# iiscleap/ICL-speech-text-LLM

Measured on AMD Instinct MI355X. Metric: ICL utterances/sec (whole node), SALMONN+Llama2-7B 5-shot VOXCELEB, higher is better.
Workload: dtype bf16

## Files before the change

### icl-speech-text-llm_amd/csrc/attn.hip

```cpp
#include "common.h"
#include <type_traits>

#ifndef ICL_ATTN_V
#define ICL_ATTN_V 1
#endif

namespace {

struct AttnParams {
  const unsigned short* Q;
  const unsigned short* K;
  const unsigned short* V;
  unsigned short* O;
  const int* cu;
  const int* kv_lens;
  const float* rel_bias;
  const float* rel_gate;
  int64_t ldq, ldk, ldv, ldo;
  int64_t kv_seq_stride, kv_head_stride;
  int n_heads, rel_span, n_qblocks;
  float scale_log2e;
};

constexpr float NEG_BIG = -1.0e30f;

__device__ __forceinline__ float max32(const f32x16& a, const f32x16& b) {
  float m = __builtin_fmaxf(a[0], a[1]);
#pragma unroll
  for (int r = 2; r < 16; ++r) m = __builtin_fmaxf(m, a[r]);
#pragma unroll
  for (int r = 0; r < 16; ++r) m = __builtin_fmaxf(m, b[r]);
  return m;
}
constexpr float LOG2E = 1.4426950408889634f;
typedef float f32x2 __attribute__((ext_vector_type(2)));

__device__ __forceinline__ float max_xhalf(float v) {
  const unsigned u = __builtin_bit_cast(unsigned, v);
  const auto r = __builtin_amdgcn_permlane32_swap(u, u, false, false);
  const unsigned lo = r[0], hi = r[1];
  return __builtin_fmaxf(__builtin_bit_cast(float, lo), __builtin_bit_cast(float, hi));
}

template <int D, bool CAUSAL, bool BIAS>
__global__ __launch_bounds__(256, (D == 64 && BIAS) ? 3 : 2) void attn_fwd_kernel(AttnParams p) {
  constexpr int QB = 1;
  constexpr bool P2 = (D == 128);
  constexpr int BQ = 128 * QB;
  constexpr int ROWB = D * 2;
  constexpr int KS = D / 16;
  constexpr int DB = D / 32;
  constexpr int CPR = D / 8;
  constexpr int NCH = 64 * CPR / 256;
  constexpr int RPI = 64 / CPR;
  constexpr int BUF = 2 * 64 * ROWB;
  constexpr int NBUF = D == 64 ? 3 : 2;
  constexpr int AHEAD = NBUF - 1;
  __shared__ __attribute__((aligned(16))) char lds[NBUF * BUF];
  __shared__ float bias_win[BIAS ? 4 * QB * 128 : 1];

  const int tid = threadIdx.x, lane = tid & 63, wave = tid >> 6;
  const int ql = lane & 31, hh = lane >> 5;
  const int n_blocks = gridDim.x;
  const int xcd = blockIdx.x & 7, q8 = n_blocks >> 3, r8 = n_blocks & 7;
  const int item = (xcd < r8 ? xcd * (q8 + 1) : r8 * (q8 + 1) + (xcd - r8) * q8) + (blockIdx.x >> 3);
  const int qblk = (CAUSAL && (ICL_ATTN_V & 2)) ? p.n_qblocks - 1 - item % p.n_qblocks : item % p.n_qblocks;
  const int head = (item / p.n_qblocks) % p.n_heads, seq = item / (p.n_qblocks * p.n_heads);
  const int row0 = p.cu[seq];
  const int len = p.cu[seq + 1] - row0;
  const int qb = qblk * BQ;
  if (qb >= len) return;
  int kvlen = len;
  if (p.kv_lens) kvlen = min(max(p.kv_lens[seq], 1), len);
  const int kv_end = CAUSAL ? min(kvlen, qb + BQ) : kvlen;
  const int n_tiles = (kv_end + 63) >> 6;

  int qw[QB], qpos[QB];
  bf16x8 qf[QB][KS];
  float gate[QB];
  const float* bias_row = nullptr;
#pragma unroll
  for (int qi = 0; qi < QB; ++qi) {
    qw[qi] = qb + (wave * QB + qi) * 32;
    qpos[qi] = qw[qi] + ql;
    const int qrow = min(qpos[qi], len - 1);
    const unsigned short* qp = p.Q + (int64_t)(row0 + qrow) * p.ldq + head * D + hh * 8;
#pragma unroll
    for (int ks = 0; ks < KS; ++ks) qf[qi][ks] = *(const bf16x8*)(qp + ks * 16);
    gate[qi] = 0.f;
    if (BIAS) gate[qi] = p.rel_gate[(int64_t)(row0 + qrow) * p.n_heads + head] * LOG2E;
  }
  if (BIAS) bias_row = p.rel_bias + (int64_t)head * (2 * p.rel_span - 1) + (p.rel_span - 1);

  auto f_k = [](int row) { return D == 64 ? (row >> 1) & 7 : row & 15; };
  auto f_v = [](int row) { return D == 64 ? ((row >> 1) & 1) << 2 : (row & 3) << 2; };
  const int64_t kv_off = p.kv_seq_stride ? (int64_t)seq * p.kv_seq_stride + (int64_t)head * p.kv_head_stride : -1;
  const unsigned short* kbase = kv_off >= 0 ? p.K + kv_off : p.K + (int64_t)row0 * p.ldk + head * D;
  const unsigned short* vbase = kv_off >= 0 ? p.V + kv_off : p.V + (int64_t)row0 * p.ldv + head * D;
  const unsigned short* kptr[NCH];
  const unsigned short* vptr[NCH];
  int srow[NCH], kch[NCH], vch[NCH];
#pragma unroll
  for (int i = 0; i < NCH; ++i) {
    const int j = wave * NCH + i;
    srow[i] = RPI * j + lane / CPR;
    kch[i] = (lane % CPR) ^ f_k(srow[i]);
    vch[i] = (lane % CPR) ^ f_v(srow[i]);
    kptr[i] = kbase + (int64_t)srow[i] * p.ldk + kch[i] * 8;
    vptr[i] = vbase + (int64_t)srow[i] * p.ldv + vch[i] * 8;
  }
  const int64_t kstep = 64 * p.ldk, vstep = 64 * p.ldv;
  typedef const __attribute__((address_space(1))) void* gptr_t;
  typedef __attribute__((address_space(3))) void* lptr_t;
  auto stage_tile = [&](int t, int buf) {
    const int k0 = t * 64;
    char* k_w = lds + buf * BUF + wave * NCH * 1024;
    char* v_w = k_w + 64 * ROWB;
    if (k0 + 64 <= len) {
#pragma unroll
      for (int i = 0; i < NCH; ++i) {
        __builtin_amdgcn_global_load_lds((gptr_t)(kptr[i] + (int64_t)t * kstep), (lptr_t)(k_w + i * 1024), 16, 0, 0);
        __builtin_amdgcn_global_load_lds((gptr_t)(vptr[i] + (int64_t)t * vstep), (lptr_t)(v_w + i * 1024), 16, 0, 0);
      }
    } else {
#pragma unroll
      for (int i = 0; i < NCH; ++i) {
        const int64_t grow = min(k0 + srow[i], len - 1);
        __builtin_amdgcn_global_load_lds((gptr_t)(kbase + grow * p.ldk + kch[i] * 8), (lptr_t)(k_w + i * 1024), 16, 0, 0);
        __builtin_amdgcn_global_load_lds((gptr_t)(vbase + grow * p.ldv + vch[i] * 8), (lptr_t)(v_w + i * 1024), 16, 0, 0);
      }
    }
  };

  f32x16 o_acc[QB][DB];
  float m_run[QB], l_run[QB];
#pragma unroll
  for (int qi = 0; qi < QB; ++qi) {
    m_run[qi] = NEG_BIG;
    l_run[qi] = 0.f;
#pragma unroll
    for (int d = 0; d < DB; ++d)
#pragma unroll
      for (int r = 0; r < 16; ++r) o_acc[qi][d][r] = 0.f;
  }

  int k_off[KS];
#pragma unroll
  for (int ks = 0; ks < KS; ++ks) k_off[ks] = ql * ROWB + (((2 * ks + hh) ^ f_k(ql)) << 4);
  int tr_off[DB];
  {
    const int q = (lane & 15) >> 2;
    const int c2 = ((lane >> 4) & 1) * 2 + ((lane & 3) >> 1);
#pragma unroll
    for (int d = 0; d < DB; ++d)
      tr_off[d] = (4 * hh + q) * ROWB + (((4 * d + c2) ^ f_v(q)) << 4) + (lane & 1) * 8;
  }

  auto wait_oldest_tile = [&]() {
    if constexpr (AHEAD == 1) asm volatile("s_waitcnt vmcnt(0)" ::: "memory");
    else if constexpr (NCH == 2) asm volatile("s_waitcnt vmcnt(4)" ::: "memory");
    else asm volatile("s_waitcnt vmcnt(8)" ::: "memory");
  };
#pragma unroll
  for (int a = 0; a < AHEAD; ++a) stage_tile(min(a, n_tiles - 1), a);
  wait_oldest_tile();
  __syncthreads();
  int cur = 0;

  auto tile = [&](const int t, auto maymask_c, auto last_c) {
    constexpr bool MAYMASK = decltype(maymask_c)::value;
    constexpr bool LAST = decltype(last_c)::value;
    int nxt = cur + AHEAD;
    if (nxt >= NBUF) nxt -= NBUF;
    if constexpr (!LAST) stage_tile(min(t + AHEAD, n_tiles - 1), nxt);
    const int k0 = t * 64;
    const char* k_lds = lds + cur * BUF;
    const char* v_lds = k_lds + 64 * ROWB;
    bool active[QB];
    bool any_active = false;
#pragma unroll
    for (int qi = 0; qi < QB; ++qi) {
      active[qi] = !MAYMASK || !CAUSAL || (k0 <= qw[qi] + 31);
      any_active |= active[qi];
    }
    if (any_active) {
      f32x16 s_acc[QB][2];
#pragma unroll
      for (int qi = 0; qi < QB; ++qi)
#pragma unroll
        for (int kb = 0; kb < 2; ++kb)
#pragma unroll
          for (int r = 0; r < 16; ++r) s_acc[qi][kb][r] = 0.f;
      {
        constexpr int LA = QB == 2 ? 1 : 2;
        bf16x8 kf[LA + 1][2];
        auto read_k = [&](int ks, int slot) {
#pragma unroll
          for (int kb = 0; kb < 2; ++kb) {
            const unsigned a = (unsigned)(uintptr_t)(k_lds + kb * 32 * ROWB + k_off[ks]);
            asm volatile("ds_read_b128 %0, %1" : "=v"(kf[slot][kb]) : "v"(a));
          }
        };
#pragma unroll
        for (int i = 0; i < LA; ++i) read_k(i, i);
#pragma unroll
        for (int ks = 0; ks < KS; ++ks) {
          const int slot = ks % (LA + 1);
          if (ks + LA < KS) read_k(ks + LA, (ks + LA) % (LA + 1));
          const int newer = 2 * (KS - 1 - ks < LA ? KS - 1 - ks : LA);
          if (newer == 4) asm volatile("s_waitcnt lgkmcnt(4)" : "+v"(kf[slot][0]), "+v"(kf[slot][1]));
          else if (newer == 2) asm volatile("s_waitcnt lgkmcnt(2)" : "+v"(kf[slot][0]), "+v"(kf[slot][1]));
          else asm volatile("s_waitcnt lgkmcnt(0)" : "+v"(kf[slot][0]), "+v"(kf[slot][1]));
#pragma unroll
          for (int kb = 0; kb < 2; ++kb)
#pragma unroll
            for (int qi = 0; qi < QB; ++qi)
              if (active[qi])
                s_acc[qi][kb] = __builtin_amdgcn_mfma_f32_32x32x16_bf16(kf[slot][kb], qf[qi][ks], s_acc[qi][kb], 0, 0, 0);
        }
      }
      bf16x8 pf[QB][2][2];
      bf16x8 pl[P2 ? QB : 1][2][2];
#pragma unroll
      for (int qi = 0; qi < QB; ++qi) {
        if (!active[qi]) {
#pragma unroll
          for (int kb = 0; kb < 2; ++kb)
#pragma unroll
            for (int h2 = 0; h2 < 2; ++h2)
#pragma unroll
              for (int e = 0; e < 8; ++e) {
                pf[qi][kb][h2][e] = (__bf16)0.f;
                if (P2) pl[qi][kb][h2][e] = (__bf16)0.f;
              }
          continue;
        }
        const bool need_mask =
            MAYMASK && __builtin_amdgcn_readfirstlane((int)((k0 + 64 > kvlen) || (CAUSAL && (k0 + 63 > qw[qi]))));
        float psum = 0.f, alpha;
        if (!BIAS && !need_mask) {
          float tmax = max32(s_acc[qi][0], s_acc[qi][1]);
          tmax = max_xhalf(tmax) * p.scale_log2e;
          const float m_new = __builtin_fmaxf(m_run[qi], tmax);
          alpha = __builtin_amdgcn_exp2f(m_run[qi] - m_new);
          m_run[qi] = m_new;
          const f32x2 sc2 = {p.scale_log2e, p.scale_log2e}, nm2 = {-m_new, -m_new};
          f32x2 ps2 = {0.f, 0.f};
#pragma unroll
          for (int kb = 0; kb < 2; ++kb)
#pragma unroll
            for (int r = 0; r < 16; r += 2) {
              const f32x2 x = f32x2{s_acc[qi][kb][r], s_acc[qi][kb][r + 1]} * sc2 + nm2;
              const f32x2 e = {__builtin_amdgcn_exp2f(x[0]), __builtin_amdgcn_exp2f(x[1])};
              ps2 += e;
#pragma unroll
              for (int h = 0; h < 2; ++h) {
                pf[qi][kb][r >> 3][(r & 7) + h] = (__bf16)e[h];
                if (P2) pl[qi][kb][r >> 3][(r & 7) + h] = (__bf16)(e[h] - (float)pf[qi][kb][r >> 3][(r & 7) + h]);
              }
            }
          psum = ps2[0] + ps2[1];
        } else {
          float tmax;
          const float* win = nullptr;
          if (BIAS) {
            float* w = bias_win + (wave * QB + qi) * 128;
            const int base_rel = k0 - qw[qi] - 31;
#pragma unroll
            for (int i = 0; i < 2; ++i) {
              const int rel = max(-(p.rel_span - 1), min(p.rel_span - 1, base_rel + lane + 64 * i));
              w[lane + 64 * i] = bias_row[rel];
            }
            __builtin_amdgcn_wave_barrier();
            win = w + (4 * hh - ql + 31);
          }
#pragma unroll
          for (int kb = 0; kb < 2; ++kb) {
#pragma unroll
            for (int r = 0; r < 16; ++r) {
              const int key = k0 + kb * 32 + (r & 3) + 8 * (r >> 2) + 4 * hh;
              float v = s_acc[qi][kb][r] * p.scale_log2e;
              if (BIAS) v = fmaf(gate[qi], win[kb * 32 + (r & 3) + 8 * (r >> 2)], v);
              if (need_mask) {
                const bool ok = (key < kvlen) && (!CAUSAL || key <= qpos[qi]);
                v = ok ? v : NEG_BIG;
              }
              s_acc[qi][kb][r] = v;
            }
          }
          tmax = max_xhalf(max32(s_acc[qi][0], s_acc[qi][1]));
          const float m_new = __builtin_fmaxf(m_run[qi], tmax);
          alpha = __builtin_amdgcn_exp2f(m_run[qi] - m_new);
          m_run[qi] = m_new;
#pragma unroll
          for (int kb = 0; kb < 2; ++kb) {
#pragma unroll
            for (int r = 0; r < 16; ++r) {
              float e = __builtin_amdgcn_exp2f(s_acc[qi][kb][r] - m_new);
              if (need_mask) e = (s_acc[qi][kb][r] <= NEG_BIG * 0.5f) ? 0.f : e;
              psum += e;
              pf[qi][kb][r >> 3][r & 7] = (__bf16)e;
              if (P2) pl[qi][kb][r >> 3][r & 7] = (__bf16)(e - (float)pf[qi][kb][r >> 3][r & 7]);
            }
          }
        }
        l_run[qi] = l_run[qi] * alpha + psum;
        if (__builtin_amdgcn_ballot_w64(alpha != 1.0f) != 0) {
#pragma unroll
          for (int d = 0; d < DB; ++d)
#pragma unroll
            for (int r = 0; r < 16; ++r) o_acc[qi][d][r] *= alpha;
        }
      }
      {
        typedef __attribute__((ext_vector_type(8))) short s16x8;
        s16x4 vr[2][2][2];
        auto read_unit = [&](int u, int slot) {
          const int d = u >> 1, kb = u & 1;
#pragma unroll
          for (int s = 0; s < 2; ++s) {
            const unsigned a = (unsigned)(uintptr_t)(v_lds + (kb * 32 + 16 * s) * ROWB + tr_off[d]);
            asm volatile("ds_read_b64_tr_b16 %0, %1" : "=v"(vr[slot][s][0]) : "v"(a));
            asm volatile("ds_read_b64_tr_b16 %0, %1 offset:%2" : "=v"(vr[slot][s][1]) : "v"(a), "n"(8 * ROWB));
          }
        };
        read_unit(0, 0);
#pragma unroll
        for (int u = 0; u < 2 * DB; ++u) {
          const int slot = u & 1, d = u >> 1, kb = u & 1;
          if (u + 1 < 2 * DB) {
            read_unit(u + 1, slot ^ 1);
            asm volatile("s_waitcnt lgkmcnt(4)" : "+v"(vr[slot][0][0]), "+v"(vr[slot][0][1]), "+v"(vr[slot][1][0]), "+v"(vr[slot][1][1]));
          } else {
            asm volatile("s_waitcnt lgkmcnt(0)" : "+v"(vr[slot][0][0]), "+v"(vr[slot][0][1]), "+v"(vr[slot][1][0]), "+v"(vr[slot][1][1]));
          }
#pragma unroll
          for (int s = 0; s < 2; ++s) {
            const s16x8 both = __builtin_shufflevector(vr[slot][s][0], vr[slot][s][1], 0, 1, 2, 3, 4, 5, 6, 7);
            const bf16x8 vf = __builtin_bit_cast(bf16x8, both);
#pragma unroll
            for (int qi = 0; qi < QB; ++qi)
              if (active[qi]) {
                o_acc[qi][d] = __builtin_amdgcn_mfma_f32_32x32x16_bf16(vf, pf[qi][kb][s], o_acc[qi][d], 0, 0, 0);
                if (P2) o_acc[qi][d] = __builtin_amdgcn_mfma_f32_32x32x16_bf16(vf, pl[qi][kb][s], o_acc[qi][d], 0, 0, 0);
              }
          }
        }
      }
    }
    if constexpr (LAST) asm volatile("s_waitcnt vmcnt(0)" ::: "memory");
    else wait_oldest_tile();
    __builtin_amdgcn_s_barrier();
    cur = cur + 1 == NBUF ? 0 : cur + 1;
  };
  int t = 0;
  if constexpr (ICL_ATTN_V & 1) {
    const int n_staged = max(n_tiles - AHEAD, 0);
    const int n_plain = min(n_staged, CAUSAL ? min(kvlen, qw[0] + 1) >> 6 : kvlen >> 6);
    for (; t < n_plain; ++t) tile(t, std::false_type{}, std::false_type{});
    for (; t < n_staged; ++t) tile(t, std::true_type{}, std::false_type{});
    for (; t < n_tiles; ++t) tile(t, std::true_type{}, std::true_type{});
  } else {
    const int n_plain = min(n_tiles, CAUSAL ? min(kvlen, qw[0] + 1) >> 6 : kvlen >> 6);
    for (; t < n_plain; ++t) tile(t, std::false_type{}, std::false_type{});
    for (; t < n_tiles; ++t) tile(t, std::true_type{}, std::false_type{});
  }
  asm volatile("s_waitcnt vmcnt(0)" ::: "memory");
  __syncthreads();

  float inv[QB];
#pragma unroll
  for (int qi = 0; qi < QB; ++qi) {
    const float l_tot = l_run[qi] + __shfl_xor(l_run[qi], 32, 64);
    inv[qi] = l_tot > 0.f ? 1.f / l_tot : 0.f;
  }
  const bool rows16 = (((uintptr_t)p.O | (uintptr_t)(p.ldo * 2)) & 15) == 0;
  if (rows16) {
    constexpr int PITCH = D * 2 + 16;
    constexpr int LPR = D * 2 / 16, RPI = 64 / LPR;
    char* stg = lds + wave * (QB * 32 * PITCH);
#pragma unroll
    for (int qi = 0; qi < QB; ++qi)
#pragma unroll
      for (int d = 0; d < DB; ++d)
#pragma unroll
        for (int g = 0; g < 4; ++g) {
          const int d0 = d * 32 + 8 * g + 4 * hh;
          *(u32x2*)(stg + (qi * 32 + ql) * PITCH + d0 * 2) =
              u32x2{pack_bf16x2(o_acc[qi][d][4 * g] * inv[qi], o_acc[qi][d][4 * g + 1] * inv[qi]),
                    pack_bf16x2(o_acc[qi][d][4 * g + 2] * inv[qi], o_acc[qi][d][4 * g + 3] * inv[qi])};
        }
    __builtin_amdgcn_wave_barrier();
#pragma unroll
    for (int it = 0; it < QB * 32 / RPI; ++it) {
      const int row = it * RPI + lane / LPR, cc = lane % LPR;
      const int q = qw[row >> 5] + (row & 31);
      const u32x4 v = *(const u32x4*)(stg + row * PITCH + cc * 16);
      if (q < len) *(u32x4*)(p.O + (int64_t)(row0 + q) * p.ldo + head * D + cc * 8) = v;
    }
    return;
  }
#pragma unroll
  for (int qi = 0; qi < QB; ++qi) {
    if (qpos[qi] < len) {
      unsigned short* op = p.O + (int64_t)(row0 + qpos[qi]) * p.ldo + head * D;
#pragma unroll
      for (int d = 0; d < DB; ++d) {
#pragma unroll
        for (int g = 0; g < 4; ++g) {
          const int d0 = d * 32 + 8 * g + 4 * hh;
          u32x2 pk = {pack_bf16x2(o_acc[qi][d][4 * g] * inv[qi], o_acc[qi][d][4 * g + 1] * inv[qi]),
                      pack_bf16x2(o_acc[qi][d][4 * g + 2] * inv[qi], o_acc[qi][d][4 * g + 3] * inv[qi])};
          *(u32x2*)(op + d0) = pk;
        }
      }
    }
  }
}


constexpr int IL64_NW = 4;
template <bool CAUSAL, int NW>
__global__ __launch_bounds__(64 * NW, CAUSAL ? 1 : 2) void attn_fwd_il64_kernel(AttnParams p) {
  constexpr int D = 64, QB = 2, BQ = 32 * NW * QB, ROWB = D * 2, KS = D / 16, DB = D / 32, CPR = D / 8;
  constexpr int NCH = 64 * CPR / (64 * NW), RPI = 64 / CPR, BUF = 2 * 64 * ROWB, NBUF = 3;
  constexpr int EPI = NW * QB * 32 * (D * 2 + 16);
  static_assert(NW == 4 && NCH == 2, "the counted waits below (vmcnt(4) = one tile of 2 K + 2 V LDS-DMA per wave in flight) are for 4 waves");
  static_assert(EPI <= NBUF * BUF, "the epilogue staging must fit inside the K / V ring it reuses");
  __shared__ __attribute__((aligned(16))) char lds[NBUF * BUF];

  const int tid = threadIdx.x, lane = tid & 63, wave = tid >> 6;
  const int ql = lane & 31, hh = lane >> 5;
  const int n_blocks = gridDim.x;
  const int xcd = blockIdx.x & 7, q8 = n_blocks >> 3, r8 = n_blocks & 7;
  const int item = (xcd < r8 ? xcd * (q8 + 1) : r8 * (q8 + 1) + (xcd - r8) * q8) + (blockIdx.x >> 3);
  const int qblk = item % p.n_qblocks;
  const int head = (item / p.n_qblocks) % p.n_heads, seq = item / (p.n_qblocks * p.n_heads);
  const int row0 = p.cu[seq];
  const int len = p.cu[seq + 1] - row0;
  const int qb = qblk * BQ;
  if (qb >= len) return;
  int kvlen = len;
  if (p.kv_lens) kvlen = min(max(p.kv_lens[seq], 1), len);
  const int kv_end = CAUSAL ? min(kvlen, qb + BQ) : kvlen;
  const int n_tiles = (kv_end + 63) >> 6;

  int qw[QB], qpos[QB];
  bf16x8 qf[QB][KS];
#pragma unroll
  for (int qi = 0; qi < QB; ++qi) {
    qw[qi] = qb + (wave * QB + qi) * 32;
    qpos[qi] = qw[qi] + ql;
    const int qrow = min(qpos[qi], len - 1);
    const unsigned short* qp = p.Q + (int64_t)(row0 + qrow) * p.ldq + head * D + hh * 8;
#pragma unroll
    for (int ks = 0; ks < KS; ++ks) qf[qi][ks] = *(const bf16x8*)(qp + ks * 16);
  }

  auto f_k = [](int row) { return (row >> 1) & 7; };
  auto f_v = [](int row) { return ((row >> 1) & 1) << 2; };
  const int64_t kv_off = p.kv_seq_stride ? (int64_t)seq * p.kv_seq_stride + (int64_t)head * p.kv_head_stride : -1;
  const unsigned short* kbase = kv_off >= 0 ? p.K + kv_off : p.K + (int64_t)row0 * p.ldk + head * D;
  const unsigned short* vbase = kv_off >= 0 ? p.V + kv_off : p.V + (int64_t)row0 * p.ldv + head * D;
  const unsigned short* kptr[NCH];
  const unsigned short* vptr[NCH];
  int srow[NCH], kch[NCH], vch[NCH];
#pragma unroll
  for (int i = 0; i < NCH; ++i) {
    const int j = wave * NCH + i;
    srow[i] = RPI * j + lane / CPR;
    kch[i] = (lane % CPR) ^ f_k(srow[i]);
    vch[i] = (lane % CPR) ^ f_v(srow[i]);
    kptr[i] = kbase + (int64_t)srow[i] * p.ldk + kch[i] * 8;
    vptr[i] = vbase + (int64_t)srow[i] * p.ldv + vch[i] * 8;
  }
  const int64_t kstep = 64 * p.ldk, vstep = 64 * p.ldv;
  typedef const __attribute__((address_space(1))) void* gptr_t;
  typedef __attribute__((address_space(3))) void* lptr_t;
  auto stage_tile = [&](int t, int buf) {
    const int k0 = t * 64;
    char* k_w = lds + buf * BUF + wave * NCH * 1024;
    char* v_w = k_w + 64 * ROWB;
    if (k0 + 64 <= len) {
#pragma unroll
      for (int i = 0; i < NCH; ++i) {
        __builtin_amdgcn_global_load_lds((gptr_t)(kptr[i] + (int64_t)t * kstep), (lptr_t)(k_w + i * 1024), 16, 0, 0);
        __builtin_amdgcn_global_load_lds((gptr_t)(vptr[i] + (int64_t)t * vstep), (lptr_t)(v_w + i * 1024), 16, 0, 0);
      }
    } else {
#pragma unroll
      for (int i = 0; i < NCH; ++i) {
        const int64_t grow = min(k0 + srow[i], len - 1);
        __builtin_amdgcn_global_load_lds((gptr_t)(kbase + grow * p.ldk + kch[i] * 8), (lptr_t)(k_w + i * 1024), 16, 0, 0);
        __builtin_amdgcn_global_load_lds((gptr_t)(vbase + grow * p.ldv + vch[i] * 8), (lptr_t)(v_w + i * 1024), 16, 0, 0);
      }
    }
  };

  f32x16 o_acc[QB][DB];
  float m_run[QB], l_run[QB];
#pragma unroll
  for (int qi = 0; qi < QB; ++qi) {
    m_run[qi] = NEG_BIG;
    l_run[qi] = 0.f;
#pragma unroll
    for (int d = 0; d < DB; ++d)
#pragma unroll
      for (int r = 0; r < 16; ++r) o_acc[qi][d][r] = 0.f;
  }
  int k_off[KS];
#pragma unroll
  for (int ks = 0; ks < KS; ++ks) k_off[ks] = ql * ROWB + (((2 * ks + hh) ^ f_k(ql)) << 4);
  int tr_off[DB];
  {
    const int q = (lane & 15) >> 2;
    const int c2 = ((lane >> 4) & 1) * 2 + ((lane & 3) >> 1);
#pragma unroll
    for (int d = 0; d < DB; ++d) tr_off[d] = (4 * hh + q) * ROWB + (((4 * d + c2) ^ f_v(q)) << 4) + (lane & 1) * 8;
  }

  auto sm_head = [&](const int qi, f32x16 (&s)[2], const int k0, auto maymask_c) -> bool {
    constexpr bool MAYMASK = decltype(maymask_c)::value;
    const bool need_mask =
        MAYMASK && __builtin_amdgcn_readfirstlane((int)((k0 + 64 > kvlen) || (CAUSAL && (k0 + 63 > qw[qi]))));
    float tmax;
    if (!need_mask) {
      tmax = max_xhalf(max32(s[0], s[1])) * p.scale_log2e;
    } else {
#pragma unroll
      for (int kb = 0; kb < 2; ++kb)
#pragma unroll
        for (int r = 0; r < 16; ++r) {
          const int key = k0 + kb * 32 + (r & 3) + 8 * (r >> 2) + 4 * hh;
          const bool ok = (key < kvlen) && (!CAUSAL || key <= qpos[qi]);
          s[kb][r] = ok ? s[kb][r] * p.scale_log2e : NEG_BIG;
        }
      tmax = max_xhalf(max32(s[0], s[1]));
    }
    const float m_new = __builtin_fmaxf(m_run[qi], tmax);
    const float alpha = __builtin_amdgcn_exp2f(m_run[qi] - m_new);
    m_run[qi] = m_new;
    l_run[qi] *= alpha;
    if (__builtin_amdgcn_ballot_w64(alpha != 1.0f) != 0) {
#pragma unroll
      for (int d = 0; d < DB; ++d)
#pragma unroll
        for (int r = 0; r < 16; ++r) o_acc[qi][d][r] *= alpha;
    }
    return need_mask;
  };
  auto sm_tail = [&](const int qi, f32x16 (&s)[2], const bool need_mask, bf16x8 (&pf)[2][2]) {
    float psum = 0.f;
    const float m = m_run[qi];
    if (!need_mask) {
#pragma unroll
      for (int kb = 0; kb < 2; ++kb)
#pragma unroll
        for (int r = 0; r < 16; ++r) {
          const float e = __builtin_amdgcn_exp2f(fmaf(s[kb][r], p.scale_log2e, -m));
          psum += e;
          pf[kb][r >> 3][r & 7] = (__bf16)e;
        }
    } else {
#pragma unroll
      for (int kb = 0; kb < 2; ++kb)
#pragma unroll
        for (int r = 0; r < 16; ++r) {
          float e = __builtin_amdgcn_exp2f(s[kb][r] - m);
          e = (s[kb][r] <= NEG_BIG * 0.5f) ? 0.f : e;
          psum += e;
          pf[kb][r >> 3][r & 7] = (__bf16)e;
        }
    }
    l_run[qi] += psum;
  };

  stage_tile(0, 0);
  stage_tile(min(1, n_tiles - 1), 1);
  asm volatile("s_waitcnt vmcnt(4)" ::: "memory");
  __syncthreads();
  int cur = 0;

  auto tile = [&](const int t, auto maymask_c) {
    int nxt = cur + 2;
    if (nxt >= NBUF) nxt -= NBUF;
    stage_tile(min(t + 2, n_tiles - 1), nxt);
    const int k0 = t * 64;
    const char* k_lds = lds + cur * BUF;
    const char* v_lds = k_lds + 64 * ROWB;
    bf16x8 kf[KS][2];
#pragma unroll
    for (int ks = 0; ks < KS; ++ks)
#pragma unroll
      for (int kb = 0; kb < 2; ++kb) {
        const unsigned a = (unsigned)(uintptr_t)(k_lds + kb * 32 * ROWB + k_off[ks]);
        asm volatile("ds_read_b128 %0, %1" : "=v"(kf[ks][kb]) : "v"(a));
      }
    f32x16 s0[2], s1[2];
#pragma unroll
    for (int kb = 0; kb < 2; ++kb)
#pragma unroll
      for (int r = 0; r < 16; ++r) s0[kb][r] = s1[kb][r] = 0.f;
#pragma unroll
    for (int ks = 0; ks < KS; ++ks) {
      if (ks == 0) asm volatile("s_waitcnt lgkmcnt(6)" : "+v"(kf[0][0]), "+v"(kf[0][1]));
      if (ks == 1) asm volatile("s_waitcnt lgkmcnt(4)" : "+v"(kf[1][0]), "+v"(kf[1][1]));
      if (ks == 2) asm volatile("s_waitcnt lgkmcnt(2)" : "+v"(kf[2][0]), "+v"(kf[2][1]));
      if (ks == 3) asm volatile("s_waitcnt lgkmcnt(0)" : "+v"(kf[3][0]), "+v"(kf[3][1]));
#pragma unroll
      for (int kb = 0; kb < 2; ++kb) s0[kb] = __builtin_amdgcn_mfma_f32_32x32x16_bf16(kf[ks][kb], qf[0][ks], s0[kb], 0, 0, 0);
    }
    const bool nm0 = sm_head(0, s0, k0, maymask_c);
#pragma unroll
    for (int ks = 0; ks < KS; ++ks)
#pragma unroll
      for (int kb = 0; kb < 2; ++kb) s1[kb] = __builtin_amdgcn_mfma_f32_32x32x16_bf16(kf[ks][kb], qf[1][ks], s1[kb], 0, 0, 0);
    bf16x8 pf0[2][2], pf1[2][2];
    sm_tail(0, s0, nm0, pf0);
    asm volatile("" : "+v"(pf0[0][0]), "+v"(pf0[0][1]), "+v"(pf0[1][0]), "+v"(pf0[1][1]));
    typedef __attribute__((ext_vector_type(8))) short s16x8;
    s16x4 vr[2][2][DB][2];
#pragma unroll
    for (int kb = 0; kb < 2; ++kb)
#pragma unroll
      for (int s = 0; s < 2; ++s)
#pragma unroll
        for (int d = 0; d < DB; ++d) {
          const unsigned a = (unsigned)(uintptr_t)(v_lds + (kb * 32 + 16 * s) * ROWB + tr_off[d]);
          asm volatile("ds_read_b64_tr_b16 %0, %1" : "=v"(vr[kb][s][d][0]) : "v"(a));
          asm volatile("ds_read_b64_tr_b16 %0, %1 offset:%2" : "=v"(vr[kb][s][d][1]) : "v"(a), "n"(8 * ROWB));
        }
    const bool nm1 = sm_head(1, s1, k0, maymask_c);
    bf16x8 vf[2][2][DB];
#pragma unroll
    for (int kb = 0; kb < 2; ++kb)
#pragma unroll
      for (int s = 0; s < 2; ++s) {
        if (kb == 0 && s == 0) asm volatile("s_waitcnt lgkmcnt(12)" : "+v"(vr[0][0][0][0]), "+v"(vr[0][0][0][1]), "+v"(vr[0][0][1][0]), "+v"(vr[0][0][1][1]));
        if (kb == 0 && s == 1) asm volatile("s_waitcnt lgkmcnt(8)" : "+v"(vr[0][1][0][0]), "+v"(vr[0][1][0][1]), "+v"(vr[0][1][1][0]), "+v"(vr[0][1][1][1]));
        if (kb == 1 && s == 0) asm volatile("s_waitcnt lgkmcnt(4)" : "+v"(vr[1][0][0][0]), "+v"(vr[1][0][0][1]), "+v"(vr[1][0][1][0]), "+v"(vr[1][0][1][1]));
        if (kb == 1 && s == 1) asm volatile("s_waitcnt lgkmcnt(0)" : "+v"(vr[1][1][0][0]), "+v"(vr[1][1][0][1]), "+v"(vr[1][1][1][0]), "+v"(vr[1][1][1][1]));
#pragma unroll
        for (int d = 0; d < DB; ++d) {
          const s16x8 both = __builtin_shufflevector(vr[kb][s][d][0], vr[kb][s][d][1], 0, 1, 2, 3, 4, 5, 6, 7);
          vf[kb][s][d] = __builtin_bit_cast(bf16x8, both);
          o_acc[0][d] = __builtin_amdgcn_mfma_f32_32x32x16_bf16(vf[kb][s][d], pf0[kb][s], o_acc[0][d], 0, 0, 0);
        }
      }
    sm_tail(1, s1, nm1, pf1);
#pragma unroll
    for (int kb = 0; kb < 2; ++kb)
#pragma unroll
      for (int s = 0; s < 2; ++s)
#pragma unroll
        for (int d = 0; d < DB; ++d)
          o_acc[1][d] = __builtin_amdgcn_mfma_f32_32x32x16_bf16(vf[kb][s][d], pf1[kb][s], o_acc[1][d], 0, 0, 0);
    asm volatile("s_waitcnt vmcnt(4)" ::: "memory");
    __builtin_amdgcn_s_barrier();
    cur = cur + 1 == NBUF ? 0 : cur + 1;
  };
  int t = 0;
  {
    const int n_plain = min(n_tiles, CAUSAL ? min(kvlen, qw[0] + 1) >> 6 : kvlen >> 6);
    for (; t < n_plain; ++t) tile(t, std::false_type{});
  }
  for (; t < n_tiles; ++t) tile(t, std::true_type{});
  asm volatile("s_waitcnt vmcnt(0)" ::: "memory");
  __syncthreads();

  float inv[QB];
#pragma unroll
  for (int qi = 0; qi < QB; ++qi) {
    const float l_tot = l_run[qi] + __shfl_xor(l_run[qi], 32, 64);
    inv[qi] = l_tot > 0.f ? 1.f / l_tot : 0.f;
  }
  const bool rows16 = (((uintptr_t)p.O | (uintptr_t)(p.ldo * 2)) & 15) == 0;
  if (rows16) {
    constexpr int PITCH = D * 2 + 16;
    constexpr int LPR = D * 2 / 16, RPS = 64 / LPR;
    char* stg = lds + wave * (QB * 32 * PITCH);
#pragma unroll
    for (int qi = 0; qi < QB; ++qi)
#pragma unroll
      for (int d = 0; d < DB; ++d)
#pragma unroll
        for (int g = 0; g < 4; ++g) {
          const int d0 = d * 32 + 8 * g + 4 * hh;
          *(u32x2*)(stg + (qi * 32 + ql) * PITCH + d0 * 2) =
              u32x2{pack_bf16x2(o_acc[qi][d][4 * g] * inv[qi], o_acc[qi][d][4 * g + 1] * inv[qi]),
                    pack_bf16x2(o_acc[qi][d][4 * g + 2] * inv[qi], o_acc[qi][d][4 * g + 3] * inv[qi])};
        }
    __builtin_amdgcn_wave_barrier();
#pragma unroll
    for (int it = 0; it < QB * 32 / RPS; ++it) {
      const int row = it * RPS + lane / LPR, cc = lane % LPR;
      const int q = qw[row >> 5] + (row & 31);
      const u32x4 v = *(const u32x4*)(stg + row * PITCH + cc * 16);
      if (q < len) *(u32x4*)(p.O + (int64_t)(row0 + q) * p.ldo + head * D + cc * 8) = v;
    }
    return;
  }
#pragma unroll
  for (int qi = 0; qi < QB; ++qi) {
    if (qpos[qi] < len) {
      unsigned short* op = p.O + (int64_t)(row0 + qpos[qi]) * p.ldo + head * D;
#pragma unroll
      for (int d = 0; d < DB; ++d)
#pragma unroll
        for (int g = 0; g < 4; ++g) {
          const int d0 = d * 32 + 8 * g + 4 * hh;
          *(u32x2*)(op + d0) = u32x2{pack_bf16x2(o_acc[qi][d][4 * g] * inv[qi], o_acc[qi][d][4 * g + 1] * inv[qi]),
                                     pack_bf16x2(o_acc[qi][d][4 * g + 2] * inv[qi], o_acc[qi][d][4 * g + 3] * inv[qi])};
        }
    }
  }
}

template <int D>
int launch_attn(const AttnParams& p, const icl_attn_args* a, hipStream_t stream) {
  const int bq = (D == 64 && !a->rel_bias) ? IL64_NW * 64 : 128;
  dim3 grid(((a->max_seqlen + bq - 1) / bq) * a->n_heads * a->n_seqs, 1, 1);
  const bool bias = a->rel_bias != nullptr;
  if (D == 64 && !bias) {
    if (a->causal) hipLaunchKernelGGL((attn_fwd_il64_kernel<true, IL64_NW>), grid, dim3(64 * IL64_NW), 0, stream, p);
    else hipLaunchKernelGGL((attn_fwd_il64_kernel<false, IL64_NW>), grid, dim3(64 * IL64_NW), 0, stream, p);
    ICL_CHECK_LAUNCH("icl_attn_fwd_bf16");
    return ICL_OK;
  }
  if (a->causal) {
    if (bias)
      hipLaunchKernelGGL((attn_fwd_kernel<D, true, true>), grid, dim3(256), 0, stream, p);
    else
      hipLaunchKernelGGL((attn_fwd_kernel<D, true, false>), grid, dim3(256), 0, stream, p);
  } else {
    if (bias)
      hipLaunchKernelGGL((attn_fwd_kernel<D, false, true>), grid, dim3(256), 0, stream, p);
    else
      hipLaunchKernelGGL((attn_fwd_kernel<D, false, false>), grid, dim3(256), 0, stream, p);
  }
  ICL_CHECK_LAUNCH("icl_attn_fwd_bf16");
  return ICL_OK;
}

}

extern "C" int icl_attn_fwd_bf16(const icl_attn_args* a, void* stream) {
  ICL_CHECK_ARG(a != nullptr, "icl_attn_fwd_bf16: args is NULL");
  ICL_CHECK_ARG(a->Q && a->K && a->V && a->O && a->cu_seqlens, "icl_attn_fwd_bf16: NULL pointer");
  ICL_CHECK_ARG(a->head_dim == 64 || a->head_dim == 128, "icl_attn_fwd_bf16: head_dim=%d (only 64 and 128)", a->head_dim);
  ICL_CHECK_ARG(a->n_seqs > 0 && a->n_seqs <= 65535 && a->n_heads > 0 && a->n_heads <= 65535 && a->max_seqlen > 0,
                "icl_attn_fwd_bf16: bad n_seqs/n_heads/max_seqlen");
  ICL_CHECK_ARG(a->ldq % 8 == 0 && a->ldk % 8 == 0 && a->ldv % 8 == 0 && a->ldo % 4 == 0,
                "icl_attn_fwd_bf16: leading dimensions must be multiples of 8 (ldo: 4)");
  ICL_CHECK_ARG(((uintptr_t)a->Q & 15) == 0 && ((uintptr_t)a->K & 15) == 0 && ((uintptr_t)a->V & 15) == 0 &&
                    ((uintptr_t)a->O & 7) == 0,
                "icl_attn_fwd_bf16: Q/K/V must be 16-byte and O 8-byte aligned");
  ICL_CHECK_ARG((a->rel_bias == nullptr) == (a->rel_gate == nullptr), "icl_attn_fwd_bf16: rel_bias and rel_gate go together");
  if (a->rel_bias) ICL_CHECK_ARG(a->rel_span >= 1, "icl_attn_fwd_bf16: rel_span must be >= 1");
  AttnParams p;
  p.Q = (const unsigned short*)a->Q;
  p.K = (const unsigned short*)a->K;
  p.V = (const unsigned short*)a->V;
  p.O = (unsigned short*)a->O;
  p.cu = a->cu_seqlens;
  p.kv_lens = a->kv_lens;
  p.rel_bias = a->rel_bias;
  p.rel_gate = a->rel_gate;
  p.ldq = a->ldq; p.ldk = a->ldk; p.ldv = a->ldv; p.ldo = a->ldo;
  ICL_CHECK_ARG((a->kv_seq_stride == 0) == (a->kv_head_stride == 0) && a->kv_seq_stride >= 0 && a->kv_head_stride >= 0 &&
                    a->kv_seq_stride % 8 == 0 && a->kv_head_stride % 8 == 0,
                "icl_attn_fwd_bf16: kv_seq_stride / kv_head_stride must both be 0 or both positive multiples of 8");
  p.kv_seq_stride = a->kv_seq_stride; p.kv_head_stride = a->kv_head_stride;
  p.n_heads = a->n_heads;
  p.rel_span = a->rel_span;
  const int bq = (a->head_dim == 64 && !a->rel_bias) ? IL64_NW * 64 : 128;
  p.n_qblocks = (a->max_seqlen + bq - 1) / bq;
  p.scale_log2e = a->scale * LOG2E;
  return a->head_dim == 64 ? launch_attn<64>(p, a, (hipStream_t)stream) : launch_attn<128>(p, a, (hipStream_t)stream);
}
```

### icl-speech-text-llm_amd/csrc/beats.hip

```cpp
#include "common.h"

namespace {

__device__ __forceinline__ int audio_of(const int* cu, int n_audio, int row, int pad) {
  int lo = 0, hi = n_audio - 1;
  while (lo < hi) {
    const int mid = (lo + hi + 1) >> 1;
    if (cu[mid] + pad * mid <= row) lo = mid;
    else hi = mid - 1;
  }
  return lo;
}

__global__ __launch_bounds__(256) void beats_patchify_kernel(const float* fbank, int max_frames, const int* cu,
                                                              int n_audio, int total_rows, unsigned short* out) {
  const int row0 = blockIdx.x * 8;
  const int row = row0 + (threadIdx.x >> 5);
  if (row >= total_rows) return;
  int a = audio_of(cu, n_audio, row0, 0);
  while (a + 1 < n_audio && cu[a + 1] <= row) ++a;
  const int local = row - cu[a];
  const int tp = local >> 3, fp = local & 7;
  const int l = threadIdx.x & 31, i = l >> 1, j0 = (l & 1) * 8;
  const float* src = fbank + ((int64_t)a * max_frames + tp * 16 + i) * 128 + fp * 16 + j0;
  const f32x4 v0 = *(const f32x4*)src, v1 = *(const f32x4*)(src + 4);
  *(u32x4*)(out + (int64_t)row * 256 + l * 8) =
      u32x4{pack_bf16x2(v0[0], v0[1]), pack_bf16x2(v0[2], v0[3]), pack_bf16x2(v1[0], v1[1]), pack_bf16x2(v1[2], v1[3])};
}

__global__ __launch_bounds__(256) void beats_posconv_pack_kernel(float* x, const int* cu, const int* valid,
                                                                  int n_audio, int C, int G, unsigned short* xg) {
  const int lanes_per_row = C >> 3, rows_per_block = 256 / lanes_per_row;
  const int sub = threadIdx.x / lanes_per_row;
  if (sub >= rows_per_block) return;
  const int total = cu[n_audio] + 128 * n_audio;
  const int prow0 = blockIdx.x * rows_per_block, prow = prow0 + sub;
  if (prow >= total) return;
  int a = audio_of(cu, n_audio, prow0, 128);
  while (a + 1 < n_audio && cu[a + 1] + 128 * (a + 1) <= prow) ++a;
  const int r = prow - (cu[a] + 128 * a);
  const int T = cu[a + 1] - cu[a];
  const int t = r - 64;
  const bool in_range = (t >= 0) && (t < T);
  const bool live = in_range && (t < valid[a]);
  const int cpg = C / G;
  const int c = (threadIdx.x - sub * lanes_per_row) * 8;
  f32x4 v0 = {0.f, 0.f, 0.f, 0.f}, v1 = v0;
  if (in_range) {
    float* px = x + ((int64_t)cu[a] + t) * C + c;
    if (live) {
      v0 = *(const f32x4*)px;
      v1 = *(const f32x4*)(px + 4);
    } else {
      *(f32x4*)px = v0;
      *(f32x4*)(px + 4) = v0;
    }
  }
  const int g = c / cpg, ci = c - g * cpg;
  const int64_t base = ((int64_t)cu[a] + 128 * (int64_t)a) * C;
  *(u32x4*)(xg + base + ((int64_t)g * (T + 128) + r) * cpg + ci) =
      u32x4{pack_bf16x2(v0[0], v0[1]), pack_bf16x2(v0[2], v0[3]), pack_bf16x2(v1[0], v1[1]), pack_bf16x2(v1[2], v1[3])};
}

__global__ __launch_bounds__(256) void gather_rows_kernel(const float* src, int64_t lds_, const int* idx, float* out,
                                                           int64_t ldo, int N) {
  const int64_t r = blockIdx.x;
  const float* s = src + (int64_t)idx[r] * lds_;
  float* d = out + r * ldo;
  for (int c = threadIdx.x * 4; c < N; c += blockDim.x * 4) *(f32x4*)(d + c) = *(const f32x4*)(s + c);
}

}

extern "C" int icl_beats_patchify(const float* fbank, int32_t max_frames, const int32_t* cu_rows, int32_t n_audio,
                                  int32_t total_rows, void* out, void* stream) {
  ICL_CHECK_ARG(fbank && cu_rows && out && n_audio > 0 && total_rows > 0, "icl_beats_patchify: bad arguments");
  ICL_CHECK_ARG(((uintptr_t)fbank & 15) == 0 && ((uintptr_t)out & 15) == 0, "icl_beats_patchify: misaligned pointer");
  hipLaunchKernelGGL(beats_patchify_kernel, dim3((total_rows + 7) / 8), dim3(256), 0, (hipStream_t)stream, fbank, max_frames,
                     cu_rows, n_audio, total_rows, (unsigned short*)out);
  ICL_CHECK_LAUNCH("icl_beats_patchify");
  return ICL_OK;
}

extern "C" int icl_beats_posconv_pack(float* x, const int32_t* cu_rows, const int32_t* valid_rows, int32_t n_audio,
                                      int32_t total_rows, int32_t channels, int32_t groups, void* xg, void* stream) {
  ICL_CHECK_ARG(x && cu_rows && valid_rows && xg && n_audio > 0 && total_rows > 0, "icl_beats_posconv_pack: bad arguments");
  ICL_CHECK_ARG(groups > 0 && channels % groups == 0 && (channels / groups) % 8 == 0,
                "icl_beats_posconv_pack: channels/groups must be a multiple of 8 (got %d/%d)", channels, groups);
  ICL_CHECK_ARG(channels % 8 == 0 && channels <= 2048 && ((uintptr_t)x & 15) == 0 && ((uintptr_t)xg & 15) == 0,
                "icl_beats_posconv_pack: channels must be a multiple of 8 (<= 2048), pointers 16-byte aligned");
  const int rows_per_block = 256 / (channels / 8);
  hipLaunchKernelGGL(beats_posconv_pack_kernel, dim3((total_rows + 128 * n_audio + rows_per_block - 1) / rows_per_block), dim3(256),
                     0, (hipStream_t)stream, x, cu_rows, valid_rows, n_audio, channels, groups, (unsigned short*)xg);
  ICL_CHECK_LAUNCH("icl_beats_posconv_pack");
  return ICL_OK;
}

extern "C" int icl_gather_rows_f32(const float* src, int64_t ld_src, const int32_t* idx, float* out, int64_t ld_out,
                                   int32_t rows, int32_t N, void* stream) {
  ICL_CHECK_ARG(src && idx && out && rows > 0 && N > 0 && N % 4 == 0 && ld_src % 4 == 0 && ld_out % 4 == 0,
                "icl_gather_rows_f32: bad arguments");
  ICL_CHECK_ARG(((uintptr_t)src & 15) == 0 && ((uintptr_t)out & 15) == 0, "icl_gather_rows_f32: misaligned");
  hipLaunchKernelGGL(gather_rows_kernel, dim3(rows), dim3(256), 0, (hipStream_t)stream, src, ld_src, idx, out, ld_out, N);
  ICL_CHECK_LAUNCH("icl_gather_rows_f32");
  return ICL_OK;
}
```

### icl-speech-text-llm_amd/csrc/gemm.hip

```cpp
#include "gemm_common.h"
#include <vector>

using namespace iclg;

namespace {


#define TILE_STAGES_DEEP(BM_, BN_) (((BM_) + (BN_)) <= 128 ? 4 : 3)

template <int WAVES_M, int WAVES_N, int MI, int NI, int NST>
__global__ __launch_bounds__(256) void gemm_bf16_kernel(GemmParams p) {
  constexpr int BM = WAVES_M * MI * 16, BN = WAVES_N * NI * 16;
  constexpr int A_BYTES = BM * 128, W_BYTES = BN * 128, BUF = A_BYTES + W_BYTES;
  constexpr int A_INSTR = BM / 32, W_INSTR = BN / 32;
  constexpr int G_STAGE = A_INSTR + W_INSTR;
  static_assert(WAVES_M * WAVES_N == 4, "4 waves per block");
  extern __shared__ __attribute__((aligned(16))) char smem[];

  const int tid = threadIdx.x, lane = tid & 63;
  const int wave = __builtin_amdgcn_readfirstlane(tid >> 6);
  const int wm = wave / WAVES_N, wn = wave % WAVES_N;

  int tm, tn;
  block_to_tile(p, blockIdx.x, tm, tn);
// ... 664 lines not shown
    for (int u = 0; u < U; ++u) {
      if (j + u >= j1) break;
      const int s = 2 * (j + u);
#pragma unroll
      for (int h = 0; h < 2; ++h) {
        if (h == 0 ? s < s0 : s + 1 >= s1) continue;
#pragma unroll
        for (int t = 0; t < NT; ++t) {
          const bf16x8 wf = fp8x8_scaled_bf16(wq[u][t][2 * h], wq[u][t][2 * h + 1], sc[t]);
#pragma unroll
          for (int b = 0; b < MB; ++b) acc[t][b] = __builtin_amdgcn_mfma_f32_16x16x32_bf16(wf, af[u][h][b], acc[t][b], 0, 0, 0);
        }
      }
    }
  }
#pragma unroll
  for (int t = 0; t < NT; ++t)
#pragma unroll
    for (int b = 0; b < MB; ++b) *(f32x4*)&red[wave][t][b][lane * 4] = acc[t][b];
  __syncthreads();
  for (int f = wave; f < NT * MB; f += 8) {
    const int t = f / MB, b = f - t * MB;
    f32x4 v = *(const f32x4*)&red[0][t][b][lane * 4];
#pragma unroll
    for (int w = 1; w < 8; ++w) v = v + *(const f32x4*)&red[w][t][b][lane * 4];
    if (!(p.epi & ICL_EPI_SWIGLU)) epi_store4(p, 0, b * 16 + fr, n0 + t * 16 + fq * 4, v);
    else *(f32x4*)&red[0][t][b][lane * 4] = v;
  }
  if (p.epi & ICL_EPI_SWIGLU) {
    if constexpr (NT == 2) {
      __syncthreads();
      for (int b = wave; b < MB; b += 8) {
        const f32x4 g = *(const f32x4*)&red[0][0][b][lane * 4], u = *(const f32x4*)&red[0][1][b][lane * 4];
        epi_store_swiglu(p, 0, b * 16 + fr, n0, fq * 4, g, u);
      }
    }
  }
}

template <int MB, int NT, int U>
int launch_skinny_fp8w(GemmParams& p, const float* wscale, hipStream_t stream) {
  const int blocks = (p.N + 16 * NT - 1) / (16 * NT);
  hipLaunchKernelGGL((gemm_skinny_fp8w_kernel<MB, NT, U>), dim3(blocks), dim3(512), 0, stream, p, wscale);
  ICL_CHECK_LAUNCH("icl_gemm_fp8w");
  return ICL_OK;
}


template <int DEPTH, int MT>
int launch_m128(GemmParams& p, hipStream_t stream) {
  constexpr int BN = 128, SMEM = (DEPTH + 1) * MT * 16 * 128;
  auto kern = gemm_m128_kernel<DEPTH, MT>;
  static bool attr_set = false;
  if (!attr_set) {
    hipError_t e = hipFuncSetAttribute((const void*)kern, hipFuncAttributeMaxDynamicSharedMemorySize, SMEM);
    if (e != hipSuccess) {
      icl_set_error("icl_gemm_bf16: hipFuncSetAttribute(%d) failed: %s", SMEM, hipGetErrorString(e));
      return ICL_ELAUNCH;
    }
    attr_set = true;
  }
  hipLaunchKernelGGL(kern, dim3((p.N + BN - 1) / BN, 1, p.split_k), dim3(512), SMEM, stream, p);
  ICL_CHECK_LAUNCH("icl_gemm_bf16(m128)");
  return ICL_OK;
}

template <int WAVES_M, int WAVES_N, int MI, int NI, int NST>
int launch_tile_n(GemmParams& p, dim3 grid, hipStream_t stream) {
  constexpr int BM = WAVES_M * MI * 16, BN = WAVES_N * NI * 16;
  constexpr int SMEM = (BM + BN) * 128 * NST;
  auto kern = gemm_bf16_kernel<WAVES_M, WAVES_N, MI, NI, NST>;
  static bool attr_set = false;
  if (!attr_set) {
    hipError_t e = hipFuncSetAttribute((const void*)kern, hipFuncAttributeMaxDynamicSharedMemorySize, SMEM);
    if (e != hipSuccess) {
      icl_set_error("icl_gemm_bf16: hipFuncSetAttribute(%d) failed: %s", SMEM, hipGetErrorString(e));
      return ICL_ELAUNCH;
    }
    attr_set = true;
  }
  hipLaunchKernelGGL(kern, grid, dim3(256), SMEM, stream, p);
  ICL_CHECK_LAUNCH("icl_gemm_bf16");
  return ICL_OK;
}

template <int WAVES_M, int WAVES_N, int MI, int NI>
int launch_tile(GemmParams& p, int batch, hipStream_t stream) {
  constexpr int BM = WAVES_M * MI * 16, BN = WAVES_N * NI * 16;
  constexpr int DEEP = TILE_STAGES_DEEP(BM, BN);
  p.tiles_m = (p.M + BM - 1) / BM;
  p.tiles_n = (p.N + BN - 1) / BN;
  dim3 grid(p.tiles_m * p.tiles_n, 1, p.split_k > 1 ? p.split_k : batch);
  static int n_cu = 0;
  if (n_cu <= 0) {
    n_cu = icl_device_cu_count();
    if (n_cu <= 0) n_cu = 256;
  }
  const int64_t blocks = (int64_t)grid.x * grid.z;
  const int per_cu = (160 * 1024) / ((BM + BN) * 128 * DEEP);
  if (blocks <= (int64_t)n_cu * per_cu) return launch_tile_n<WAVES_M, WAVES_N, MI, NI, DEEP>(p, grid, stream);
  return launch_tile_n<WAVES_M, WAVES_N, MI, NI, 2>(p, grid, stream);
}

}


extern "C" int icl_gemm_select_tile(int32_t M, int32_t N, int32_t K, int32_t batch, int32_t split_k) {
  const int64_t t128 = (int64_t)((M + 127) / 128) * ((N + 127) / 128) * batch;
  if (split_k > 1 || M <= 64 || t128 < 256) return 2;
  if (N <= 64) return 2;
  if (N <= 128) return 1;
  static int ncu = 0;
  if (ncu <= 0) {
    ncu = icl_device_cu_count();
    if (ncu <= 0) ncu = 256;
  }
  const int64_t t256 = (int64_t)((M + 255) / 256) * ((N + 255) / 256) * batch;
  const int64_t rounds = (t256 + ncu - 1) / ncu;
  const double eff = (double)t256 / (double)(rounds * ncu);
  if (K >= 768 && eff >= 0.6) return 3;
  return 1;
}

struct NormFuse {
  const float* gamma;
  float eps;
  unsigned short* xn;
  int64_t ldx;
};

static int gemm_impl(const icl_gemm_args* a, void* stream_, const RopeFuse* rope, const NormFuse* norm = nullptr,
                     const float* wscale = nullptr) {
  hipStream_t stream = (hipStream_t)stream_;
  ICL_CHECK_ARG(a != nullptr, "icl_gemm_bf16: args is NULL");
  ICL_CHECK_ARG(a->A && a->W && a->C, "icl_gemm_bf16: A/W/C must be non-NULL");
  ICL_CHECK_ARG(a->M > 0 && a->N > 0 && a->K > 0, "icl_gemm_bf16: M,N,K must be > 0 (got %d,%d,%d)",
                a->M, a->N, a->K);
  ICL_CHECK_ARG(a->K % 64 == 0, "icl_gemm_bf16: K=%d must be a multiple of 64", a->K);
  ICL_CHECK_ARG(a->lda % 8 == 0 && a->ldw % 8 == 0,
                "icl_gemm_bf16: lda=%lld / ldw=%lld must be multiples of 8", (long long)a->lda,
                (long long)a->ldw);
  ICL_CHECK_ARG(((uintptr_t)a->A & 15) == 0 && ((uintptr_t)a->W & 15) == 0,
                "icl_gemm_bf16: A and W must be 16-byte aligned");
  ICL_CHECK_ARG(a->ldw >= a->K, "icl_gemm_bf16: ldw=%lld < K=%d", (long long)a->ldw, a->K);
  ICL_CHECK_ARG(a->batch >= 1 && a->batch <= 65535, "icl_gemm_bf16: batch=%d out of range", a->batch);
  ICL_CHECK_ARG(a->split_k >= 1 && a->split_k <= 64, "icl_gemm_bf16: split_k=%d out of range", a->split_k);
  ICL_CHECK_ARG(a->out_dtype == ICL_BF16 || a->out_dtype == ICL_F32, "icl_gemm_bf16: bad out_dtype %d",
                a->out_dtype);
  ICL_CHECK_ARG(a->res_dtype == ICL_BF16 || a->res_dtype == ICL_F32, "icl_gemm_bf16: bad res_dtype %d",
                a->res_dtype);
  ICL_CHECK_ARG((a->epilogue & ~15) == 0, "icl_gemm_bf16: unknown epilogue bits 0x%x", a->epilogue);
  const bool swiglu = a->epilogue & ICL_EPI_SWIGLU;
  if (swiglu) {
    ICL_CHECK_ARG(a->N % 32 == 0, "icl_gemm_bf16: SWIGLU needs N %% 32 == 0 (N=%d)", a->N);
    ICL_CHECK_ARG((a->epilogue & (ICL_EPI_GELU | ICL_EPI_RESIDUAL)) == 0,
                  "icl_gemm_bf16: SWIGLU cannot be combined with GELU/RESIDUAL");
    ICL_CHECK_ARG(a->ldc % 4 == 0, "icl_gemm_bf16: SWIGLU needs ldc %% 4 == 0");
  }
  if (a->epilogue & ICL_EPI_BIAS) ICL_CHECK_ARG(a->bias, "icl_gemm_bf16: EPI_BIAS without bias");
  if (a->epilogue & ICL_EPI_RESIDUAL) ICL_CHECK_ARG(a->R, "icl_gemm_bf16: EPI_RESIDUAL without R");
  const int nout = swiglu ? a->N / 2 : a->N;
  ICL_CHECK_ARG(a->ldc >= nout, "icl_gemm_bf16: ldc=%lld < %d output columns", (long long)a->ldc, nout);
  if (a->split_k > 1) {
    ICL_CHECK_ARG(a->batch == 1, "icl_gemm_bf16: split_k > 1 requires batch == 1");
    ICL_CHECK_ARG(a->workspace, "icl_gemm_bf16: split_k > 1 requires a workspace");
    ICL_CHECK_ARG(a->split_k <= a->K / 64, "icl_gemm_bf16: split_k=%d > K/64=%d", a->split_k, a->K / 64);
  }
  const int cal = a->out_dtype == ICL_BF16 ? 8 : 16;
  ICL_CHECK_ARG(((uintptr_t)a->C % cal) == 0, "icl_gemm_bf16: C must be %d-byte aligned", cal);
  if (a->R) {
    const int ral = a->res_dtype == ICL_BF16 ? 8 : 16;
    ICL_CHECK_ARG(((uintptr_t)a->R % ral) == 0, "icl_gemm_bf16: R must be %d-byte aligned", ral);
  }

  GemmParams p;
  p.A = (const __bf16*)a->A;
  p.W = (const __bf16*)a->W;
  p.C = a->C;
  p.bias = a->bias;
  p.R = a->R;
  p.ws = a->workspace;
  p.lda = a->lda; p.ldw = a->ldw; p.ldc = a->ldc; p.ldr = a->ldr;
  p.sA = a->strideA; p.sC = a->strideC; p.sR = a->strideR;
  p.M = a->M; p.N = a->N; p.K = a->K;
  p.epi = a->epilogue; p.out_dtype = a->out_dtype; p.res_dtype = a->res_dtype;
  p.split_k = a->split_k;
  p.tiles_m = p.tiles_n = 0;
  p.group_m = p.xcd_sync = 0;

  if (wscale) {
    ICL_CHECK_ARG(a->M <= 64 && a->batch == 1 && !rope, "icl_gemm_fp8w: needs M <= 64 and batch == 1 (M=%d batch=%d)", a->M, a->batch);
    p.split_k = 1;
    const bool sw = a->epilogue & ICL_EPI_SWIGLU;
    const int mb = (a->M + 15) / 16;
    if (sw) return mb <= 1 ? launch_skinny_fp8w<1, 2, 4>(p, wscale, stream) : mb == 2 ? launch_skinny_fp8w<2, 2, 2>(p, wscale, stream)
                           : launch_skinny_fp8w<4, 2, 1>(p, wscale, stream);
    return mb <= 1 ? launch_skinny_fp8w<1, 1, 8>(p, wscale, stream) : mb == 2 ? launch_skinny_fp8w<2, 1, 4>(p, wscale, stream)
                   : launch_skinny_fp8w<4, 1, 2>(p, wscale, stream);
  }
  int tile = a->tile;
  if (tile == 0) tile = icl_gemm_select_tile(a->M, a->N, a->K, a->batch, a->split_k);
  if (tile == 3 && a->K < 128) tile = 1;
  if (rope) {
    ICL_CHECK_ARG(tile == 3, "icl_gemm_rope_kv_bf16: only the 256x256 tile fuses RoPE (this problem resolves to tile %d; "
                             "use icl_gemm_bf16 + icl_rope_kv_bf16)", tile);
    ICL_CHECK_ARG(a->split_k == 1, "icl_gemm_rope_kv_bf16: split_k must be 1");
    return launch_tile256(p, 1, stream, rope);
  }
  int rc;
  if (tile == 1)
    rc = launch_tile<2, 2, 4, 4>(p, a->batch, stream);
  else if (tile == 2)
    rc = launch_tile<2, 2, 2, 2>(p, a->batch, stream);
  else if (tile == 3) {
    ICL_CHECK_ARG(a->split_k == 1 || (a->split_k <= a->K / 128 && a->N % 4 == 0),
                  "icl_gemm_bf16: split_k=%d on the 256x256 tile needs K / split_k >= 128 and N %% 4 == 0 (K=%d N=%d)", a->split_k, a->K, a->N);
    rc = launch_tile256(p, a->batch, stream);
  } else if (tile == 4 || tile == 6) {
    ICL_CHECK_ARG(a->M <= 64 && a->batch == 1, "icl_gemm_bf16: the skinny kernel needs M <= 64 and batch == 1");
    p.split_k = 1;
    const bool sw = a->epilogue & ICL_EPI_SWIGLU, pk = tile == 6;
    const int mb = (a->M + 15) / 16;
    if (sw) rc = mb <= 1 ? launch_skinny<1, 2, 4>(p, stream, pk) : mb == 2 ? launch_skinny<2, 2, 2>(p, stream, pk) : launch_skinny<4, 2, 2>(p, stream, pk);
    else    rc = mb <= 1 ? launch_skinny<1, 1, 8>(p, stream, pk) : mb == 2 ? launch_skinny<2, 1, 4>(p, stream, pk) : launch_skinny<4, 1, 2>(p, stream, pk);
    return rc;
  } else if (tile == 5) {
    ICL_CHECK_ARG(a->M <= 256 && a->batch == 1, "icl_gemm_bf16: the decode tile needs M <= 256 and batch == 1");
    rc = a->M <= 64 ? launch_m128<3, 4>(p, stream) : a->M <= 128 ? launch_m128<3, 8>(p, stream) : launch_m128<3, 16>(p, stream);
  } else {
    icl_set_error("icl_gemm_bf16: unsupported tile id %d", tile);
    return ICL_EINVAL;
  }
  if (rc != ICL_OK) return rc;
  if (a->split_k > 1 && norm) {
    if (a->N <= 4096) hipLaunchKernelGGL(splitk_reduce_rmsnorm_kernel<4>, dim3(a->M), dim3(256), 0, stream, p, norm->gamma, norm->eps, norm->xn, norm->ldx);
    else              hipLaunchKernelGGL(splitk_reduce_rmsnorm_kernel<8>, dim3(a->M), dim3(256), 0, stream, p, norm->gamma, norm->eps, norm->xn, norm->ldx);
    ICL_CHECK_LAUNCH("icl_gemm_rmsnorm_bf16(split-K reduce + RMSNorm)");
  } else if (a->split_k > 1) {
    const int64_t total = (int64_t)a->M * nout;
    int blocks = (int)((total + 255) / 256);
    if (blocks > 2048) blocks = 2048;
    hipLaunchKernelGGL(gemm_splitk_reduce_kernel, dim3(blocks), dim3(256), 0, stream, p);
    ICL_CHECK_LAUNCH("icl_gemm_bf16(split-K reduce)");
  }
  return ICL_OK;
}

extern "C" int icl_rmsnorm(const void* x, int64_t ldx, const float* gamma, void* y, int64_t ldy, int32_t M, int32_t N, float eps,
                           int32_t in_dtype, int32_t out_dtype, void* stream);

static int gemm_rmsnorm_impl(const icl_gemm_args* a, const float* wscale, const float* gamma, float eps, void* xn, int64_t ld_xn,
                             void* stream) {
  ICL_CHECK_ARG(a != nullptr && gamma && xn, "icl_gemm_rmsnorm_bf16: NULL pointer");
  ICL_CHECK_ARG(a->batch == 1 && a->out_dtype == ICL_F32 && (a->epilogue & ~ICL_EPI_RESIDUAL) == 0 &&
                    (!(a->epilogue & ICL_EPI_RESIDUAL) || a->res_dtype == ICL_F32),
                "icl_gemm_rmsnorm_bf16: batch 1, f32 output, residual-only epilogue with an f32 residual");
  ICL_CHECK_ARG(a->N % 4 == 0 && a->N <= 8192 && a->ldc % 4 == 0 && a->ldr % 4 == 0 && ld_xn % 4 == 0 && ld_xn >= a->N,
                "icl_gemm_rmsnorm_bf16: N=%d must be a multiple of 4 and <= 8192, leading dimensions multiples of 4", a->N);
  ICL_CHECK_ARG(((uintptr_t)gamma & 15) == 0 && ((uintptr_t)xn & 7) == 0 && ((uintptr_t)a->C & 15) == 0 &&
                    (!a->R || ((uintptr_t)a->R & 15) == 0), "icl_gemm_rmsnorm_bf16: misaligned pointer");
  if (a->split_k > 1 && a->tile != 4 && a->tile != 6 && !wscale) {
    const NormFuse nf{gamma, eps, (unsigned short*)xn, ld_xn};
    return gemm_impl(a, stream, nullptr, &nf);
  }
  const int rc = gemm_impl(a, stream, nullptr, nullptr, wscale);
  if (rc != ICL_OK) return rc;
#ifndef ICL_SMALL_M_BLOCKNORM
#define ICL_SMALL_M_BLOCKNORM 1
#endif
  if (ICL_SMALL_M_BLOCKNORM && a->M <= 64 && a->ldc == a->N) {
    GemmParams q{};
    q.ws = (float*)a->C; q.C = a->C; q.R = nullptr; q.ldc = a->ldc; q.ldr = 0; q.M = a->M; q.N = a->N; q.split_k = 1; q.epi = 0;
    if (a->N <= 4096) hipLaunchKernelGGL(splitk_reduce_rmsnorm_kernel<4>, dim3(a->M), dim3(256), 0, (hipStream_t)stream, q, gamma, eps, (unsigned short*)xn, ld_xn);
    else              hipLaunchKernelGGL(splitk_reduce_rmsnorm_kernel<8>, dim3(a->M), dim3(256), 0, (hipStream_t)stream, q, gamma, eps, (unsigned short*)xn, ld_xn);
    ICL_CHECK_LAUNCH("icl_gemm_rmsnorm_bf16(row-per-block RMSNorm)");
    return ICL_OK;
  }
  return icl_rmsnorm(a->C, a->ldc, gamma, xn, ld_xn, a->M, a->N, eps, ICL_F32, ICL_BF16, stream);
}

extern "C" int icl_gemm_rmsnorm_bf16(const icl_gemm_args* a, const float* gamma, float eps, void* xn, int64_t ld_xn, void* stream) {
  return gemm_rmsnorm_impl(a, nullptr, gamma, eps, xn, ld_xn, stream);
}

extern "C" int icl_gemm_bf16(const icl_gemm_args* a, void* stream) { return gemm_impl(a, stream, nullptr); }

extern "C" int icl_gemm_fp8w(const icl_gemm_args* a, const float* w_scale, void* stream) {
  ICL_CHECK_ARG(w_scale, "icl_gemm_fp8w: w_scale is NULL");
  return gemm_impl(a, stream, nullptr, nullptr, w_scale);
}

extern "C" int icl_gemm_rmsnorm_fp8w(const icl_gemm_args* a, const float* w_scale, const float* gamma, float eps, void* xn,
                                     int64_t ld_xn, void* stream) {
  ICL_CHECK_ARG(w_scale, "icl_gemm_rmsnorm_fp8w: w_scale is NULL");
  return gemm_rmsnorm_impl(a, w_scale, gamma, eps, xn, ld_xn, stream);
}

extern "C" int icl_gemm_rope_kv_bf16(const icl_gemm_args* a, int64_t k_off, int64_t v_off, const float* cosT,
                                     const float* sinT, const int32_t* pos, const int32_t* seq_ids, void* kcache,
                                     void* vcache, int32_t n_heads, int32_t head_dim, int32_t max_len, int32_t kv_rows_to_c,
                                     void* stream) {
  ICL_CHECK_ARG(a != nullptr && cosT && sinT && pos, "icl_gemm_rope_kv_bf16: NULL pointer");
  ICL_CHECK_ARG(head_dim == 128, "icl_gemm_rope_kv_bf16: head_dim=%d (the fused epilogue is built for 128)", head_dim);
  ICL_CHECK_ARG(n_heads > 0 && k_off == (int64_t)n_heads * 128 && v_off == 2 * k_off && a->N == 3 * k_off && k_off % 256 == 0,
                "icl_gemm_rope_kv_bf16: need q|k|v blocks of n_heads*128 columns each, a multiple of 256 (N=%d k_off=%lld v_off=%lld)",
                a->N, (long long)k_off, (long long)v_off);
  ICL_CHECK_ARG(a->batch == 1 && a->out_dtype == ICL_BF16 && (a->epilogue & ~ICL_EPI_BIAS) == 0,
                "icl_gemm_rope_kv_bf16: batch 1, bf16 output, bias-only epilogue");
  ICL_CHECK_ARG(a->C && ((uintptr_t)a->C & 15) == 0 && a->ldc % 8 == 0, "icl_gemm_rope_kv_bf16: C must be 16-byte aligned, ldc %% 8 == 0");
  ICL_CHECK_ARG(!a->bias || ((uintptr_t)a->bias & 15) == 0, "icl_gemm_rope_kv_bf16: bias must be 16-byte aligned");
  ICL_CHECK_ARG(((uintptr_t)cosT & 15) == 0 && ((uintptr_t)sinT & 15) == 0, "icl_gemm_rope_kv_bf16: cos/sin misaligned");
  ICL_CHECK_ARG((kcache == nullptr) == (vcache == nullptr), "icl_gemm_rope_kv_bf16: kcache and vcache must both be set or both NULL");
  if (kcache) {
    ICL_CHECK_ARG(seq_ids && max_len > 0, "icl_gemm_rope_kv_bf16: cache append needs seq_ids and max_len");
    ICL_CHECK_ARG(((uintptr_t)kcache & 15) == 0 && ((uintptr_t)vcache & 15) == 0, "icl_gemm_rope_kv_bf16: cache misaligned");
  }
  ICL_CHECK_ARG(kv_rows_to_c || kcache, "icl_gemm_rope_kv_bf16: kv_rows_to_c = 0 needs a cache to hold k / v");
  RopeFuse rf;
  rf.kv_rows_to_c = kv_rows_to_c;
  rf.cosT = cosT; rf.sinT = sinT; rf.pos = pos; rf.seq_ids = seq_ids;
  rf.kc = (unsigned short*)kcache; rf.vc = (unsigned short*)vcache;
  rf.k_off = (int)k_off; rf.v_off = (int)v_off; rf.H = n_heads; rf.max_len = max_len;
  return gemm_impl(a, stream, &rf);
}

extern "C" int icl_pack_decode_weights(const void* W, int64_t ldw, int32_t N, int32_t K, void* out, void* stream) {
  ICL_CHECK_ARG(W && out && N > 0 && K > 0, "icl_pack_decode_weights: bad arguments");
  ICL_CHECK_ARG(K % 64 == 0 && ldw % 8 == 0 && ldw >= K, "icl_pack_decode_weights: K=%d must be a multiple of 64, ldw=%lld a multiple of 8", K, (long long)ldw);
  ICL_CHECK_ARG(((uintptr_t)W & 15) == 0 && ((uintptr_t)out & 15) == 0, "icl_pack_decode_weights: misaligned pointer");
  const int64_t pieces = (int64_t)((N + 15) >> 4) * (K >> 5) * 64;
  const int blocks = (int)std::min<int64_t>((pieces + 255) / 256, 65535);
  hipLaunchKernelGGL(pack_decode_w_kernel, dim3(blocks), dim3(256), 0, (hipStream_t)stream, (const unsigned short*)W, ldw, N, K, (u32x4*)out);
  ICL_CHECK_LAUNCH("icl_pack_decode_weights");
  return ICL_OK;
}

extern "C" int icl_pack_fp8_weights(const void* W, int64_t ldw, int32_t N, int32_t K, void* q, float* scales, void* w_deq,
                                    int64_t ld_deq, void* stream) {
  ICL_CHECK_ARG(W && q && scales && w_deq && N > 0 && K > 0, "icl_pack_fp8_weights: bad arguments");
  ICL_CHECK_ARG(K % 64 == 0 && ldw % 8 == 0 && ldw >= K && ld_deq % 8 == 0 && ld_deq >= K,
                "icl_pack_fp8_weights: K=%d must be a multiple of 64, ldw=%lld / ld_deq=%lld multiples of 8 and >= K", K, (long long)ldw,
                (long long)ld_deq);
  ICL_CHECK_ARG((((uintptr_t)W | (uintptr_t)q | (uintptr_t)w_deq) & 15) == 0, "icl_pack_fp8_weights: misaligned pointer");
  ICL_CHECK_ARG(w_deq == W ? ld_deq == ldw : true, "icl_pack_fp8_weights: in place needs ld_deq == ldw");
  const int tiles = (N + 15) >> 4;
  hipStream_t s = (hipStream_t)stream;
  hipLaunchKernelGGL(pack_fp8_w_kernel, dim3(tiles), dim3(256), 0, s, (const unsigned short*)W, ldw, N, K, (u32x4*)q, scales,
                     (unsigned short*)w_deq, ld_deq);
  ICL_CHECK_LAUNCH("icl_pack_fp8_weights");
  std::vector<float> sc_host(N);
  hipError_t e = hipMemcpyAsync(sc_host.data(), scales, sizeof(float) * (size_t)N, hipMemcpyDeviceToHost, s);
  if (e == hipSuccess) e = hipStreamSynchronize(s);
  if (e != hipSuccess) {
    icl_set_error("icl_pack_fp8_weights: %s", hipGetErrorString(e));
    return ICL_ELAUNCH;
  }
  for (int n = 0; n < N; ++n)
    ICL_CHECK_ARG(sc_host[n] == sc_host[n], "icl_pack_fp8_weights: row %d holds a non-finite value", n);
  return ICL_OK;
}
```

### icl-speech-text-llm_amd/runtime/binding.py

```python
from __future__ import annotations

import ctypes
import os
from ctypes import POINTER, Structure, c_char_p, c_float, c_int, c_int32, c_int64, c_void_p

import torch

_HERE = os.path.dirname(os.path.abspath(__file__))
LIB_PATH = os.path.normpath(os.path.join(_HERE, "..", "lib", "libicl_hip.so"))

ICL_BF16, ICL_F32 = 0, 1
EPI_BIAS, EPI_GELU, EPI_RESIDUAL, EPI_SWIGLU = 1, 2, 4, 8
ABI_VERSION = 6
SAMPLE_TOP_K_MAX = 1024


GEMM_PROFILE = None


class IclError(RuntimeError):
    """Raised when a libicl_hip entry point returns a negative code."""


class GemmArgs(Structure):
    _fields_ = [
        ("A", c_void_p), ("W", c_void_p), ("C", c_void_p), ("bias", c_void_p), ("R", c_void_p),
        ("workspace", c_void_p),
        ("lda", c_int64), ("ldw", c_int64), ("ldc", c_int64), ("ldr", c_int64),
        ("strideA", c_int64), ("strideC", c_int64), ("strideR", c_int64),
        ("M", c_int32), ("N", c_int32), ("K", c_int32), ("batch", c_int32), ("epilogue", c_int32),
        ("out_dtype", c_int32), ("res_dtype", c_int32), ("split_k", c_int32), ("tile", c_int32),
    ]


class AttnArgs(Structure):
    _fields_ = [
        ("Q", c_void_p), ("K", c_void_p), ("V", c_void_p), ("O", c_void_p),
        ("cu_seqlens", c_void_p), ("kv_lens", c_void_p), ("rel_bias", c_void_p), ("rel_gate", c_void_p),
        ("ldq", c_int64), ("ldk", c_int64), ("ldv", c_int64), ("ldo", c_int64),
        ("n_seqs", c_int32), ("max_seqlen", c_int32), ("n_heads", c_int32), ("head_dim", c_int32),
        ("causal", c_int32), ("rel_span", c_int32), ("scale", c_float), ("reserved", c_int32),
        ("kv_seq_stride", c_int64), ("kv_head_stride", c_int64),
    ]


_SIGNATURES = {
    "icl_abi_version": (c_int, []),
    "icl_last_error": (c_char_p, []),
    "icl_device_cu_count": (c_int, []),
    "icl_gemm_bf16": (c_int, [POINTER(GemmArgs), c_void_p]),
    "icl_gemm_rmsnorm_bf16": (c_int, [POINTER(GemmArgs), c_void_p, c_float, c_void_p, c_int64, c_void_p]),
    "icl_gemm_select_tile": (c_int, [c_int32, c_int32, c_int32, c_int32, c_int32]),
    "icl_attn_fwd_bf16": (c_int, [POINTER(AttnArgs), c_void_p]),
    "icl_attn_decode_bf16": (c_int, [c_void_p, c_int64, c_void_p, c_void_p, c_void_p, c_int64, c_void_p,
                                     c_int32, c_int32, c_int32, c_int32, c_float, c_void_p]),
    "icl_attn_decode_rope_bf16": (c_int, [c_void_p, c_int64, c_int64, c_int64, c_void_p, c_void_p, c_void_p, c_void_p, c_void_p,
                                          c_void_p, c_void_p, c_int64, c_void_p, c_int32, c_int32, c_int32, c_int32, c_float,
                                          c_void_p]),
    "icl_layernorm": (c_int, [c_void_p, c_int64, c_void_p, c_float, c_void_p, c_void_p, c_void_p, c_int64,
                              c_void_p, c_int64, c_int32, c_int32, c_float, c_int32, c_int32, c_void_p]),
    "icl_rmsnorm": (c_int, [c_void_p, c_int64, c_void_p, c_void_p, c_int64, c_int32, c_int32, c_float,
                            c_int32, c_int32, c_void_p]),
    "icl_rope_kv_bf16": (c_int, [c_void_p, c_int64, c_int64, c_int64, c_void_p, c_void_p, c_void_p, c_void_p,
                                 c_void_p, c_void_p, c_int32, c_int32, c_int32, c_int32, c_void_p]),
    "icl_gemm_rope_kv_bf16": (c_int, [POINTER(GemmArgs), c_int64, c_int64, c_void_p, c_void_p, c_void_p, c_void_p,
                                      c_void_p, c_void_p, c_int32, c_int32, c_int32, c_int32, c_void_p]),
    "icl_pack_decode_weights": (c_int, [c_void_p, c_int64, c_int32, c_int32, c_void_p, c_void_p]),
    "icl_pack_fp8_weights": (c_int, [c_void_p, c_int64, c_int32, c_int32, c_void_p, c_void_p, c_void_p, c_int64, c_void_p]),
    "icl_gemm_fp8w": (c_int, [POINTER(GemmArgs), c_void_p, c_void_p]),
    "icl_gemm_rmsnorm_fp8w": (c_int, [POINTER(GemmArgs), c_void_p, c_void_p, c_float, c_void_p, c_int64, c_void_p]),
    "icl_embed_gather_interleave": (c_int, [c_void_p, c_void_p, c_void_p, c_void_p, c_int32, c_int32,
                                            c_int32, c_int32, c_void_p]),
    "icl_argmax_eos": (c_int, [c_void_p, c_int64, c_int32, c_int32, c_int32, c_int32, c_int32, c_void_p, c_void_p,
                               c_int32, c_int32, c_void_p, c_void_p]),
    "icl_argmax_fsm": (c_int, [c_void_p, c_int64, c_int32, c_int32, c_void_p, c_void_p, c_void_p, c_void_p, c_int32, c_int32,
                               c_void_p, c_int32, c_int32, c_int32, c_int32, c_void_p, c_void_p, c_int32, c_int32, c_void_p,
                               c_void_p, c_void_p]),
    "icl_sample_eos": (c_int, [c_void_p, c_int64, c_int32, c_int32, c_void_p, c_int64, c_void_p, c_int32, c_int32,
                               c_float, c_float, c_int32, c_float, c_void_p, c_int32, c_int32, c_int32, c_void_p, c_void_p,
                               c_int32, c_int32, c_void_p, c_void_p, c_void_p, c_void_p, c_int32, c_void_p]),
    "icl_beam_step": (c_int, [c_void_p, c_int64, c_int32, c_int32, c_int32, c_int32, c_int32, c_int32, c_int32, c_int32, c_float, c_float,
                              c_void_p, c_void_p, c_void_p, c_void_p, c_void_p, c_void_p, c_void_p, c_void_p, c_void_p, c_void_p]),
    "icl_kv_copy_spans_bf16": (c_int, [c_void_p, c_void_p, c_int64, c_int64, c_int64, c_int64, c_int64, c_int64, c_void_p,
                                       c_void_p, c_void_p, c_void_p, c_void_p, c_int32, c_int32, c_int32, c_int32, c_int32,
                                       c_int32, c_int32, c_int32, c_int32, c_void_p]),
    "icl_kv_copy_spans_fp8": (c_int, [c_void_p, c_void_p, c_void_p, c_void_p] + [c_int64] * 12 +
                              [c_void_p, c_void_p, c_void_p, c_void_p, c_void_p] + [c_int32] * 9 + [c_void_p]),
    "icl_kv_append_fp8": (c_int, [c_void_p, c_int64, c_int64, c_int64, c_void_p, c_void_p, c_void_p, c_void_p, c_void_p,
                                  c_void_p, c_int32, c_int32, c_int32, c_int32, c_void_p]),
    "icl_rope_kv_fp8": (c_int, [c_void_p, c_int64, c_int64, c_int64, c_void_p, c_void_p, c_void_p, c_void_p, c_void_p,
                                c_void_p, c_void_p, c_void_p, c_int32, c_int32, c_int32, c_int32, c_void_p]),
    "icl_attn_decode_bf16_epl16": (c_int, [c_void_p, c_int64, c_void_p, c_void_p, c_void_p, c_int64, c_void_p,
                                           c_int32, c_int32, c_int32, c_int32, c_float, c_void_p]),
    "icl_attn_decode_fp8": (c_int, [c_void_p, c_int64, c_void_p, c_void_p, c_void_p, c_void_p, c_void_p, c_int64, c_void_p,
                                    c_int32, c_int32, c_int32, c_int32, c_float, c_void_p]),
    "icl_attn_decode_rope_fp8": (c_int, [c_void_p, c_int64, c_int64, c_int64, c_void_p, c_void_p, c_void_p, c_void_p, c_void_p,
                                         c_void_p, c_void_p, c_void_p, c_void_p, c_int64, c_void_p, c_int32, c_int32, c_int32,
                                         c_int32, c_float, c_void_p]),
    "icl_logmel_whisper": (c_int, [c_void_p, c_int64, c_void_p, c_void_p, c_int32, c_int32, c_void_p,
                                   c_void_p, c_int64, c_void_p, c_void_p]),
    "icl_spec_to_xt": (c_int, [c_void_p, c_int32, c_int32, c_void_p, c_int64, c_void_p]),
    "icl_fbank_kaldi": (c_int, [c_void_p, c_int64, c_void_p, c_void_p, c_int32, c_int32, c_float, c_float,
                                c_void_p, c_void_p]),
    "icl_qformer_window_xattn": (c_int, [c_void_p, c_int64, c_void_p, c_int64, c_int64, c_void_p, c_int64,
                                         c_int32, c_int32, c_int32, c_int32, c_int32, c_float, c_void_p]),
    "icl_beats_gate": (c_int, [c_void_p, c_int64, c_void_p, c_void_p, c_void_p, c_void_p, c_int32, c_int32,
                               c_void_p]),
    "icl_axpby_cast": (c_int, [c_void_p, c_int64, c_int32, c_void_p, c_int64, c_int32, c_float, c_void_p,
                               c_int64, c_int32, c_int32, c_int32, c_void_p]),
    "icl_lora_down_bf16": (c_int, [c_void_p, c_int64, c_int32, c_void_p, c_int64, c_int32, c_float, c_int32,
                                   c_void_p]),
    "icl_beats_patchify": (c_int, [c_void_p, c_int32, c_void_p, c_int32, c_int32, c_void_p, c_void_p]),
    "icl_beats_posconv_pack": (c_int, [c_void_p, c_void_p, c_void_p, c_int32, c_int32, c_int32, c_int32, c_void_p,
                                       c_void_p]),
    "icl_gather_rows_f32": (c_int, [c_void_p, c_int64, c_void_p, c_void_p, c_int64, c_int32, c_int32, c_void_p]),
    "icl_cross_entropy": (c_int, [c_void_p, c_int64, c_void_p, c_int32, c_int32, c_void_p, c_void_p, c_void_p]),
}

EXPORTED_SYMBOLS = tuple(_SIGNATURES)

_lib = None


def load_library() -> ctypes.CDLL:
    global _lib
    if _lib is not None:
        return _lib
    path = os.environ.get("ICL_LIB_PATH") or LIB_PATH
    if not os.path.exists(path):
        raise ImportError(
            f"{path} not found: build it with `python -c 'import __graft_entry__ as g; g.build()'` "
            "(or `make -C icl-speech-text-llm_amd/csrc`). There is no CPU fallback for the HIP path.")
    lib = ctypes.CDLL(path)
    for name, (res, args) in _SIGNATURES.items():
        fn = getattr(lib, name)
        fn.restype = res
        fn.argtypes = args
    ver = lib.icl_abi_version()
    if ver != ABI_VERSION:
        raise ImportError(f"libicl_hip ABI version {ver} != binding version {ABI_VERSION}")
    _lib = lib
    return lib


def _check(rc: int, what: str) -> None:
    if rc != 0:
        msg = load_library().icl_last_error()
        raise IclError(f"{what} failed (code {rc}): {msg.decode() if msg else '?'}")


def _eos_pair(eos_id):
    if isinstance(eos_id, (tuple, list)):
        ids = [int(e) for e in eos_id]
        if not 1 <= len(ids) <= 2:
            raise ValueError(f"one or two EOS ids are supported, not {ids}")
        return ids[0], (ids[1] if len(ids) == 2 and ids[1] != ids[0] else -1)
    return int(eos_id), -1


def _stream() -> int:
    return torch.cuda.current_stream().cuda_stream


def _ptr(t):
    return 0 if t is None else t.data_ptr()


def _dt(t: torch.Tensor) -> int:
    if t.dtype == torch.bfloat16:
        return ICL_BF16
    if t.dtype == torch.float32:
        return ICL_F32
    raise TypeError(f"unsupported dtype {t.dtype}")


def _require_gpu(*tensors):
    for t in tensors:
        if t is not None and not t.is_cuda:
            raise IclError("libicl_hip operands must live on the GPU (no CPU fallback in the product path)")


def gemm(a: torch.Tensor, w: torch.Tensor, out: torch.Tensor, *, bias=None, residual=None, gelu=False,
         swiglu=False, split_k: int = 1, workspace=None, tile: int = 0, M=None, K=None, lda=None,
         batch: int = 1, stride_a: int = 0, stride_c: int = 0, stride_r: int = 0, rope=None, N=None, w_scale=None) -> torch.Tensor:
    _require_gpu(a, w, out, bias, residual, workspace)
    lib = load_library()
    g = GemmArgs()
    _require_gpu(w_scale)
    N = w.shape[0] if N is None else N
    g.A, g.W, g.C = a.data_ptr(), w.data_ptr(), out.data_ptr()
    g.bias, g.R, g.workspace = _ptr(bias), _ptr(residual), _ptr(workspace)
    g.lda = a.stride(-2) if lda is None else lda
    g.ldw = w.stride(0) if w_scale is None else w.shape[1]
    g.ldc = out.stride(-2)
    g.ldr = residual.stride(-2) if residual is not None else 0
    g.strideA, g.strideC, g.strideR = stride_a, stride_c, stride_r
    g.M = a.shape[-2] if M is None else M
    g.N = N
    g.K = w.shape[1] if K is None else K
    g.batch = batch
    epi = 0
    if bias is not None:
        assert bias.dtype == torch.float32
        epi |= EPI_BIAS
    if gelu:
        epi |= EPI_GELU
    if residual is not None:
        epi |= EPI_RESIDUAL
    if swiglu:
        epi |= EPI_SWIGLU
    g.epilogue = epi
    g.out_dtype = _dt(out)
    g.res_dtype = _dt(residual) if residual is not None else ICL_F32
    g.split_k = split_k
    if w_scale is not None:
        assert w.dtype == torch.uint8 and w_scale.dtype == torch.float32 and rope is None
        tile = "fp8w"
    elif tile == 0:
        tile = lib.icl_gemm_select_tile(g.M, N, g.K, batch, split_k)
    g.tile = tile if w_scale is None else 0
    if split_k > 1 and workspace is not None:
        assert workspace.dtype == torch.float32 and workspace.numel() >= split_k * g.M * N
    if rope is not None:
        k_off, v_off, cos, sin, pos, seq_ids, kcache, vcache, n_heads, head_dim, max_len = rope[:11]
        kv_rows_to_c = int(rope[11]) if len(rope) > 11 else 1
        _require_gpu(cos, sin, pos, seq_ids, kcache, vcache)

        def launch():
            _check(lib.icl_gemm_rope_kv_bf16(ctypes.byref(g), k_off, v_off, cos.data_ptr(), sin.data_ptr(), pos.data_ptr(),
                                             _ptr(seq_ids), _ptr(kcache), _ptr(vcache), n_heads, head_dim, max_len,
                                             kv_rows_to_c, _stream()), "icl_gemm_rope_kv_bf16")
    elif w_scale is not None:
        def launch():
            _check(lib.icl_gemm_fp8w(ctypes.byref(g), w_scale.data_ptr(), _stream()), "icl_gemm_fp8w")
    else:
        def launch():
            _check(lib.icl_gemm_bf16(ctypes.byref(g), _stream()), "icl_gemm_bf16")
    if GEMM_PROFILE is not None:
        e0, e1 = torch.cuda.Event(enable_timing=True), torch.cuda.Event(enable_timing=True)
        e0.record()
        launch()
        e1.record()
        GEMM_PROFILE.append((tile, split_k, 2.0 * g.M * N * g.K * batch, e0, e1, (g.M, N, g.K, batch)))
        return out
    launch()
    return out


def gemm_rmsnorm(a: torch.Tensor, w: torch.Tensor, out: torch.Tensor, gamma: torch.Tensor, eps: float, xn: torch.Tensor, *,
                 residual=None, split_k: int = 1, workspace=None, tile: int = 0, N=None, K=None, w_scale=None) -> torch.Tensor:
    _require_gpu(a, w, out, gamma, xn, residual, workspace, w_scale)
    lib = load_library()
    g = GemmArgs()
    N = w.shape[0] if N is None else N
    g.A, g.W, g.C = a.data_ptr(), w.data_ptr(), out.data_ptr()
    g.bias, g.R, g.workspace = 0, _ptr(residual), _ptr(workspace)
    g.lda, g.ldw, g.ldc = a.stride(-2), (w.stride(0) if w_scale is None else w.shape[1]), out.stride(-2)
    g.ldr = residual.stride(-2) if residual is not None else 0
    g.strideA = g.strideC = g.strideR = 0
    g.M, g.N, g.K, g.batch = a.shape[-2], N, (w.shape[1] if K is None else K), 1
    g.epilogue = EPI_RESIDUAL if residual is not None else 0
    g.out_dtype, g.res_dtype, g.split_k = _dt(out), ICL_F32, split_k
    assert out.dtype == torch.float32 and xn.dtype == torch.bfloat16 and gamma.dtype == torch.float32
    if w_scale is not None:
        assert w.dtype == torch.uint8 and w_scale.dtype == torch.float32
        g.tile = 0
        _check(lib.icl_gemm_rmsnorm_fp8w(ctypes.byref(g), w_scale.data_ptr(), gamma.data_ptr(), eps, xn.data_ptr(), xn.stride(0),
                                         _stream()), "icl_gemm_rmsnorm_fp8w")
        return out
    g.tile = tile if tile else lib.icl_gemm_select_tile(g.M, N, g.K, 1, split_k)
    if split_k > 1 and workspace is not None:
        assert workspace.dtype == torch.float32 and workspace.numel() >= split_k * g.M * N
    _check(lib.icl_gemm_rmsnorm_bf16(ctypes.byref(g), gamma.data_ptr(), eps, xn.data_ptr(), xn.stride(0), _stream()),
           "icl_gemm_rmsnorm_bf16")
    return out


def pack_decode_weights(w: torch.Tensor, K=None) -> torch.Tensor:
    _require_gpu(w)
    assert w.dtype == torch.bfloat16 and w.dim() == 2
    N, K = w.shape[0], (w.shape[1] if K is None else K)
    out = torch.empty((N + 15) // 16 * 16, K, dtype=torch.bfloat16, device=w.device)
    _check(load_library().icl_pack_decode_weights(w.data_ptr(), w.stride(0), N, K, out.data_ptr(), _stream()),
           "icl_pack_decode_weights")
    return out


def pack_fp8_weights(w: torch.Tensor, K=None, out=None):
    _require_gpu(w, out)
    assert w.dtype == torch.bfloat16 and w.dim() == 2
    N, K = w.shape[0], (w.shape[1] if K is None else K)
    q = torch.empty((N + 15) // 16 * 16, K, dtype=torch.uint8, device=w.device)
    scales = torch.empty(N, dtype=torch.float32, device=w.device)
    if out is None:
        out = torch.empty(N, K, dtype=torch.bfloat16, device=w.device)
    assert out.dtype == torch.bfloat16 and out.shape[0] == N and out.shape[1] >= K and out.stride(1) == 1
    _check(load_library().icl_pack_fp8_weights(w.data_ptr(), w.stride(0), N, K, q.data_ptr(), scales.data_ptr(), out.data_ptr(),
                                               out.stride(0), _stream()), "icl_pack_fp8_weights")
    return q, scales, out


def rope_fusable(M: int, n_heads: int, head_dim: int, K: int) -> bool:
    hd = n_heads * head_dim
    return (head_dim == 128 and hd % 256 == 0 and K >= 128 and
            load_library().icl_gemm_select_tile(M, 3 * hd, K, 1, 1) == 3)


def attn_fwd(q, k, v, out, cu_seqlens, max_seqlen: int, n_heads: int, head_dim: int, scale: float, *,
             causal=False, kv_lens=None, rel_bias=None, rel_gate=None, rel_span: int = 0, kv_cache_max_len: int = 0):
    _require_gpu(q, k, v, out, cu_seqlens, kv_lens, rel_bias, rel_gate)
    lib = load_library()
    a = AttnArgs()
    a.Q, a.K, a.V, a.O = q.data_ptr(), k.data_ptr(), v.data_ptr(), out.data_ptr()
    a.cu_seqlens, a.kv_lens = cu_seqlens.data_ptr(), _ptr(kv_lens)
    a.rel_bias, a.rel_gate = _ptr(rel_bias), _ptr(rel_gate)
    a.ldq, a.ldk, a.ldv, a.ldo = q.stride(0), k.stride(0), v.stride(0), out.stride(0)
    a.reserved = 0
    if kv_cache_max_len > 0:
        a.ldk = a.ldv = head_dim
        a.kv_seq_stride, a.kv_head_stride = n_heads * kv_cache_max_len * head_dim, kv_cache_max_len * head_dim
    else:
        a.kv_seq_stride = a.kv_head_stride = 0
    a.n_seqs = cu_seqlens.numel() - 1
    a.max_seqlen, a.n_heads, a.head_dim = max_seqlen, n_heads, head_dim
    a.causal, a.rel_span, a.scale = int(causal), rel_span, scale
    assert cu_seqlens.dtype == torch.int32
    _check(lib.icl_attn_fwd_bf16(ctypes.byref(a), _stream()), "icl_attn_fwd_bf16")
    return out


def attn_decode(q, kcache, vcache, out, lens, n_heads: int, head_dim: int, max_len: int, scale: float):
    _require_gpu(q, kcache, vcache, out, lens)
    assert lens.dtype == torch.int32
    _check(load_library().icl_attn_decode_bf16(q.data_ptr(), q.stride(0), kcache.data_ptr(), vcache.data_ptr(),
                                               out.data_ptr(), out.stride(0), lens.data_ptr(), q.shape[0],
                                               n_heads, head_dim, max_len, scale, _stream()),
           "icl_attn_decode_bf16")
    return out


def attn_decode_rope(qkv, k_off: int, v_off: int, cos, sin, pos, seq_ids, kcache, vcache, out, lens, n_heads: int,
                     head_dim: int, max_len: int, scale: float):
    _require_gpu(qkv, cos, sin, pos, seq_ids, kcache, vcache, out, lens)
    assert lens.dtype == torch.int32 and pos.dtype == torch.int32 and qkv.dtype == torch.bfloat16
    _check(load_library().icl_attn_decode_rope_bf16(qkv.data_ptr(), qkv.stride(0), k_off, v_off, cos.data_ptr(), sin.data_ptr(),
                                                    pos.data_ptr(), _ptr(seq_ids), kcache.data_ptr(), vcache.data_ptr(),
                                                    out.data_ptr(), out.stride(0), lens.data_ptr(), qkv.shape[0], n_heads,
                                                    head_dim, max_len, scale, _stream()), "icl_attn_decode_rope_bf16")
    return out


def _fp8_cache(kq, vq, ks, vs):
    assert kq.dtype == torch.uint8 and vq.dtype == torch.uint8 and ks.dtype == torch.float32 and vs.dtype == torch.float32


def attn_decode_bf16_epl16(q, kcache, vcache, out, lens, n_heads: int, head_dim: int, max_len: int, scale: float):
    _require_gpu(q, kcache, vcache, out, lens)
    assert lens.dtype == torch.int32
    _check(load_library().icl_attn_decode_bf16_epl16(q.data_ptr(), q.stride(0), kcache.data_ptr(), vcache.data_ptr(),
                                                     out.data_ptr(), out.stride(0), lens.data_ptr(), q.shape[0], n_heads, head_dim,
                                                     max_len, scale, _stream()), "icl_attn_decode_bf16_epl16")
    return out


def attn_decode_fp8(q, kq, vq, ks, vs, out, lens, n_heads: int, head_dim: int, max_len: int, scale: float):
    _require_gpu(q, kq, vq, ks, vs, out, lens)
    _fp8_cache(kq, vq, ks, vs)
    assert lens.dtype == torch.int32
    _check(load_library().icl_attn_decode_fp8(q.data_ptr(), q.stride(0), kq.data_ptr(), vq.data_ptr(), ks.data_ptr(), vs.data_ptr(),
                                              out.data_ptr(), out.stride(0), lens.data_ptr(), q.shape[0], n_heads, head_dim,
                                              max_len, scale, _stream()), "icl_attn_decode_fp8")
    return out


def attn_decode_rope_fp8(qkv, k_off: int, v_off: int, cos, sin, pos, seq_ids, kq, vq, ks, vs, out, lens, n_heads: int,
                         head_dim: int, max_len: int, scale: float):
    _require_gpu(qkv, cos, sin, pos, seq_ids, kq, vq, ks, vs, out, lens)
    _fp8_cache(kq, vq, ks, vs)
    assert lens.dtype == torch.int32 and pos.dtype == torch.int32 and qkv.dtype == torch.bfloat16
    _check(load_library().icl_attn_decode_rope_fp8(qkv.data_ptr(), qkv.stride(0), k_off, v_off, cos.data_ptr(), sin.data_ptr(),
                                                   pos.data_ptr(), _ptr(seq_ids), kq.data_ptr(), vq.data_ptr(), ks.data_ptr(),
                                                   vs.data_ptr(), out.data_ptr(), out.stride(0), lens.data_ptr(), qkv.shape[0],
                                                   n_heads, head_dim, max_len, scale, _stream()), "icl_attn_decode_rope_fp8")
    return out


def rope_kv_fp8(qkv, k_off: int, v_off: int, cos, sin, pos, seq_ids, kq, vq, ks, vs, n_heads: int, head_dim: int,
                max_len: int, M=None):
    _require_gpu(qkv, cos, sin, pos, seq_ids, kq, vq, ks, vs)
    _fp8_cache(kq, vq, ks, vs)
    M = qkv.shape[0] if M is None else M
    _check(load_library().icl_rope_kv_fp8(qkv.data_ptr(), qkv.stride(0), k_off, v_off, cos.data_ptr(), sin.data_ptr(),
                                          pos.data_ptr(), seq_ids.data_ptr(), kq.data_ptr(), vq.data_ptr(), ks.data_ptr(),
                                          vs.data_ptr(), M, n_heads, head_dim, max_len, _stream()), "icl_rope_kv_fp8")


def kv_append_fp8(qkv, k_off: int, v_off: int, pos, seq_ids, kq, vq, ks, vs, n_heads: int, head_dim: int, max_len: int, M=None):
    _require_gpu(qkv, pos, seq_ids, kq, vq, ks, vs)
    _fp8_cache(kq, vq, ks, vs)
    M = qkv.shape[0] if M is None else M
    _check(load_library().icl_kv_append_fp8(qkv.data_ptr(), qkv.stride(0), k_off, v_off, pos.data_ptr(), seq_ids.data_ptr(),
                                            kq.data_ptr(), vq.data_ptr(), ks.data_ptr(), vs.data_ptr(), M, n_heads, head_dim,
                                            max_len, _stream()), "icl_kv_append_fp8")


def layernorm(x, gamma, beta, out, eps: float, *, res=None, alpha: float = 1.0, out2=None, M=None, N=None):
    _require_gpu(x, gamma, beta, out, res, out2)
    M = x.shape[0] if M is None else M
    N = x.shape[1] if N is None else N
    if res is not None:
        assert res.dtype == x.dtype and res.stride(0) == x.stride(0)
    _check(load_library().icl_layernorm(x.data_ptr(), x.stride(0), _ptr(res), alpha, gamma.data_ptr(),
                                        beta.data_ptr(), out.data_ptr(), out.stride(0), _ptr(out2),
                                        out2.stride(0) if out2 is not None else 0, M, N, eps, _dt(x), _dt(out),
                                        _stream()), "icl_layernorm")
    return out


def rmsnorm(x, gamma, out, eps: float, *, M=None, N=None):
    _require_gpu(x, gamma, out)
    M = x.shape[0] if M is None else M
    N = x.shape[1] if N is None else N
    _check(load_library().icl_rmsnorm(x.data_ptr(), x.stride(0), gamma.data_ptr(), out.data_ptr(), out.stride(0),
                                      M, N, eps, _dt(x), _dt(out), _stream()), "icl_rmsnorm")
    return out


def rope_kv(qkv, k_off: int, v_off: int, cos, sin, pos, seq_ids, kcache, vcache, n_heads: int, head_dim: int,
            max_len: int, M=None):
    _require_gpu(qkv, cos, sin, pos, seq_ids, kcache, vcache)
    M = qkv.shape[0] if M is None else M
    _check(load_library().icl_rope_kv_bf16(qkv.data_ptr(), qkv.stride(0), k_off, v_off, cos.data_ptr(),
                                           sin.data_ptr(), pos.data_ptr(), _ptr(seq_ids), _ptr(kcache),
                                           _ptr(vcache), M, n_heads, head_dim, max_len, _stream()),
           "icl_rope_kv_bf16")


def embed_gather_interleave(src_idx, table, speech, out):
    _require_gpu(src_idx, table, speech, out)
    assert src_idx.dtype == torch.int32 and table.dtype == torch.bfloat16 and out.dtype == torch.float32
    _check(load_library().icl_embed_gather_interleave(src_idx.data_ptr(), table.data_ptr(), _ptr(speech),
                                                      out.data_ptr(), src_idx.numel(), table.shape[1],
                                                      table.shape[0], 0 if speech is None else speech.shape[0],
                                                      _stream()), "icl_embed_gather_interleave")
    return out


def argmax_eos(logits, eos_id, pad_id: int, finished, out_tokens, step: int, next_ids, V=None):
    _require_gpu(logits, finished, out_tokens, next_ids)
    e1, e2 = _eos_pair(eos_id)
    _check(load_library().icl_argmax_eos(logits.data_ptr(), logits.stride(0), logits.shape[0],
                                         logits.shape[1] if V is None else V, e1, e2, pad_id, finished.data_ptr(),
                                         out_tokens.data_ptr(), out_tokens.stride(0), step, next_ids.data_ptr(),
                                         _stream()), "icl_argmax_eos")


def argmax_fsm(logits, tables, state, steps_left: int, eos_id, pad_id: int, finished, out_tokens, step: int, next_ids,
               out_logprob=None, V=None):
    _require_gpu(logits, tables.state_off, tables.edge_tok, tables.edge_next, tables.state_dist, state, finished, out_tokens,
                 next_ids, out_logprob)
    V = logits.shape[1] if V is None else V
    if tables.vocab > V:
        raise ValueError(f"automaton built for a vocabulary of {tables.vocab} ids used on logits of {V}")
    assert logits.dtype == torch.float32 and state.dtype == torch.int32 and state.numel() == logits.shape[0]
    assert out_logprob is None or (out_logprob.dtype == torch.float32 and out_logprob.stride(0) == out_tokens.stride(0))
    e1, e2 = _eos_pair(eos_id)
    _check(load_library().icl_argmax_fsm(logits.data_ptr(), logits.stride(0), logits.shape[0], V, tables.state_off.data_ptr(),
                                         tables.edge_tok.data_ptr(), tables.edge_next.data_ptr(), tables.state_dist.data_ptr(),
                                         tables.n_states, tables.n_edges, state.data_ptr(), steps_left, e1, e2, pad_id,
                                         finished.data_ptr(), out_tokens.data_ptr(), out_tokens.stride(0), step,
                                         next_ids.data_ptr(), _ptr(out_logprob), _stream()), "icl_argmax_fsm")


def sample_eos(logits, work, uniforms, eos_id, pad_id: int, finished, out_tokens, step: int, next_ids, *,
               temperature: float = 1.0, top_k: int = 50, top_p: float = 1.0, repetition_penalty: float = 1.0, V=None,
               debug=None):
    _require_gpu(logits, work, uniforms, finished, out_tokens, next_ids)
    assert logits.dtype == torch.float32 and work.dtype == torch.float32 and uniforms.dtype == torch.float32
    V = logits.shape[1] if V is None else V
    e1, e2 = _eos_pair(eos_id)
    dbg = (None, None, None, 0)
    if debug is not None:
        _require_gpu(*debug)
        dbg = (debug[0].data_ptr(), debug[1].data_ptr(), debug[2].data_ptr(), debug[0].shape[1])
    _check(load_library().icl_sample_eos(logits.data_ptr(), logits.stride(0), logits.shape[0], V, work.data_ptr(),
                                         work.stride(0), out_tokens.data_ptr(), out_tokens.stride(0), step,
                                         repetition_penalty, temperature, top_k, top_p, uniforms.data_ptr(), e1, e2, pad_id,
                                         finished.data_ptr(), out_tokens.data_ptr(), out_tokens.stride(0), step,
                                         next_ids.data_ptr(), dbg[0], dbg[1], dbg[2], dbg[3], _stream()), "icl_sample_eos")


class BeamState:

    def __init__(self, get, B: int, K: int, T: int, pad_id: int):
        f32, i32 = torch.float32, torch.int32
        self.B, self.K, self.T = B, K, T
        self.run_score, self.fin_score = get("gen_beam_run_score", (B, K), f32), get("gen_beam_fin_score", (B, K), f32)
        self.run_seq, self.fin_seq = get("gen_beam_run_seq", (B, K, T), i32), get("gen_beam_fin_seq", (B, K, T), i32)
        self.fin_len, self.fin_flag = get("gen_beam_fin_len", (B, K), i32), get("gen_beam_fin_flag", (B, K), i32)
        self.unsat = get("gen_beam_unsat", (B,), i32)
        self.next_ids, self.parent = get("gen_beam_next", (B * K,), i32), get("gen_beam_parent", (B * K,), i32)
        self.run_score.fill_(-1.0e9)
        self.run_score[:, 0] = 0.0
        self.fin_score.fill_(-1.0e9)
        self.run_seq.fill_(pad_id)
        self.fin_seq.fill_(pad_id)
        self.fin_len.zero_()
        self.fin_flag.zero_()
        self.unsat.fill_(1)


def beam_step(logits, state: BeamState, step: int, eos_id, length_penalty: float, V=None, repetition_penalty: float = 1.0):
    _require_gpu(logits, state.run_score)
    assert logits.dtype == torch.float32 and logits.stride(1) == 1
    rows = logits.shape[0] // state.B
    assert rows * state.B == logits.shape[0] and rows in (1, state.K)
    e1, e2 = _eos_pair(eos_id)
    _check(load_library().icl_beam_step(logits.data_ptr(), logits.stride(0), rows, state.B,
                                        logits.shape[1] if V is None else V, state.K, state.T, step, e1, e2,
                                        float(length_penalty), float(repetition_penalty), state.run_score.data_ptr(),
                                        state.run_seq.data_ptr(),
                                        state.fin_score.data_ptr(), state.fin_seq.data_ptr(), state.fin_len.data_ptr(),
                                        state.fin_flag.data_ptr(), state.unsat.data_ptr(), state.next_ids.data_ptr(),
                                        state.parent.data_ptr(), _stream()), "icl_beam_step")


def kv_copy_spans(src, dst, n_rows: int, *, src_seq=None, src_t0=None, dst_seq=None, dst_t0=None, n_t=None, n_fixed: int = 0,
                  src_scale=None, dst_scale=None):
    _require_gpu(src, dst, src_seq, src_t0, dst_seq, dst_t0, n_t, src_scale, dst_scale)
    fp8 = src.dtype == torch.uint8
    assert src.dtype == dst.dtype and src.dtype in (torch.bfloat16, torch.uint8) and src.dim() == 5 and dst.dim() == 5
    assert src.stride(4) == 1 and dst.stride(4) == 1 and src.stride(3) == src.shape[4] and dst.stride(3) == dst.shape[4]
    assert src.shape[0] == dst.shape[0] and src.shape[2] == dst.shape[2] and src.shape[4] == dst.shape[4]
    for t in (src_seq, src_t0, dst_seq, dst_t0, n_t):
        assert t is None or (t.dtype == torch.int32 and t.numel() >= n_rows)
    ids = (_ptr(src_seq), _ptr(src_t0), _ptr(dst_seq), _ptr(dst_t0), _ptr(n_t), n_fixed, n_rows, src.shape[0], src.shape[2],
           src.shape[4], src.shape[1], dst.shape[1], src.shape[3], dst.shape[3], _stream())
    if fp8:
        assert src_scale is not None and dst_scale is not None and src_scale.dtype == torch.float32 and dst_scale.dtype == torch.float32
        assert tuple(src_scale.shape) == tuple(src.shape[:4]) and tuple(dst_scale.shape) == tuple(dst.shape[:4])
        assert src_scale.stride(3) == 1 and dst_scale.stride(3) == 1
        _check(load_library().icl_kv_copy_spans_fp8(src.data_ptr(), src_scale.data_ptr(), dst.data_ptr(), dst_scale.data_ptr(),
                                                    src.stride(0), src.stride(1), src.stride(2), dst.stride(0), dst.stride(1),
                                                    dst.stride(2), src_scale.stride(0), src_scale.stride(1), src_scale.stride(2),
                                                    dst_scale.stride(0), dst_scale.stride(1), dst_scale.stride(2), *ids),
               "icl_kv_copy_spans_fp8")
        return
    assert src_scale is None and dst_scale is None
    _check(load_library().icl_kv_copy_spans_bf16(src.data_ptr(), dst.data_ptr(), src.stride(0), src.stride(1), src.stride(2),
                                                 dst.stride(0), dst.stride(1), dst.stride(2), *ids), "icl_kv_copy_spans_bf16")


def logmel_whisper(wav, wav_lens, mel_filters, n_mel: int, spec, xt, workspace):
    _require_gpu(wav, wav_lens, mel_filters, spec, xt, workspace)
    assert wav.dtype == torch.float32 and mel_filters.dtype == torch.float64 and wav_lens.dtype == torch.int32
    _check(load_library().icl_logmel_whisper(wav.data_ptr(), wav.stride(0), wav_lens.data_ptr(),
                                             mel_filters.data_ptr(), n_mel, wav.shape[0], _ptr(spec), _ptr(xt),
                                             xt.stride(-2) if xt is not None else 0, workspace.data_ptr(),
                                             _stream()), "icl_logmel_whisper")


def spec_to_xt(spec, xt):
    _require_gpu(spec, xt)
    assert spec.dtype == torch.float32 and spec.is_contiguous()
    _check(load_library().icl_spec_to_xt(spec.data_ptr(), spec.shape[1], spec.shape[0], xt.data_ptr(),
                                         xt.stride(-2), _stream()), "icl_spec_to_xt")


def fbank_kaldi(wav, wav_lens, mel_banks, max_frames: int, mean: float, std: float, out):
    _require_gpu(wav, wav_lens, mel_banks, out)
    assert wav.dtype == torch.float32 and mel_banks.dtype == torch.float64 and wav_lens.dtype == torch.int32
    _check(load_library().icl_fbank_kaldi(wav.data_ptr(), wav.stride(0), wav_lens.data_ptr(), mel_banks.data_ptr(),
                                          wav.shape[0], max_frames, mean, std, out.data_ptr(), _stream()),
           "icl_fbank_kaldi")


def qformer_window_xattn(q, kv, v_off: int, out, n_audio: int, win_per_audio: int, win: int, rows_per_audio: int,
                         n_heads: int, scale: float):
    _require_gpu(q, kv, out)
    _check(load_library().icl_qformer_window_xattn(q.data_ptr(), q.stride(0), kv.data_ptr(), kv.stride(0), v_off,
                                                   out.data_ptr(), out.stride(0), n_audio, win_per_audio, win,
                                                   rows_per_audio, n_heads, scale, _stream()),
           "icl_qformer_window_xattn")


def beats_gate(qkv, grep_w, grep_b, grep_a, gate, n_heads: int, M=None):
    _require_gpu(qkv, grep_w, grep_b, grep_a, gate)
    M = qkv.shape[0] if M is None else M
    _check(load_library().icl_beats_gate(qkv.data_ptr(), qkv.stride(0), grep_w.data_ptr(), grep_b.data_ptr(),
                                         grep_a.data_ptr(), gate.data_ptr(), M, n_heads, _stream()),
           "icl_beats_gate")


def axpby_cast(x, out, alpha: float = 1.0, add=None):
    _require_gpu(x, out, add)
    M, N = x.shape
    _check(load_library().icl_axpby_cast(x.data_ptr(), x.stride(0), _dt(x), _ptr(add),
                                         add.stride(0) if add is not None else 0,
                                         _dt(add) if add is not None else ICL_F32, alpha, out.data_ptr(),
                                         out.stride(0), _dt(out), M, N, _stream()), "icl_axpby_cast")
    return out


def lora_down(x, K0: int, a, r_total: int, scale: float, M=None):
    _require_gpu(x, a)
    M = x.shape[0] if M is None else M
    _check(load_library().icl_lora_down_bf16(x.data_ptr(), x.stride(0), K0, a.data_ptr(), a.stride(0), r_total,
                                             scale, M, _stream()), "icl_lora_down_bf16")


def device_cu_count() -> int:
    return load_library().icl_device_cu_count()


def beats_patchify(fbank, cu_rows, total_rows: int, out):
    _require_gpu(fbank, cu_rows, out)
    _check(load_library().icl_beats_patchify(fbank.data_ptr(), fbank.shape[1], cu_rows.data_ptr(), fbank.shape[0],
                                             total_rows, out.data_ptr(), _stream()), "icl_beats_patchify")


def beats_posconv_pack(x, cu_rows, valid_rows, n_audio: int, total_rows: int, groups: int, xg):
    _require_gpu(x, cu_rows, valid_rows, xg)
    _check(load_library().icl_beats_posconv_pack(x.data_ptr(), cu_rows.data_ptr(), valid_rows.data_ptr(), n_audio,
                                                 total_rows, x.shape[1], groups, xg.data_ptr(), _stream()),
           "icl_beats_posconv_pack")


def gather_rows(src, idx, out, N=None):
    _require_gpu(src, idx, out)
    assert src.dtype == torch.float32 and out.dtype == torch.float32 and idx.dtype == torch.int32
    _check(load_library().icl_gather_rows_f32(src.data_ptr(), src.stride(0), idx.data_ptr(), out.data_ptr(),
                                              out.stride(0), idx.numel(), src.shape[1] if N is None else N,
                                              _stream()), "icl_gather_rows_f32")
    return out


def cross_entropy(logits, labels, row_loss, mean_loss, V=None):
    _require_gpu(logits, labels, row_loss, mean_loss)
    assert logits.dtype == torch.float32 and labels.dtype == torch.int32
    _check(load_library().icl_cross_entropy(logits.data_ptr(), logits.stride(0), labels.data_ptr(), labels.numel(),
                                            logits.shape[1] if V is None else V, row_loss.data_ptr(),
                                            mean_loss.data_ptr(), _stream()), "icl_cross_entropy")
    return mean_loss
```

### icl-speech-text-llm_amd/runtime/engines.py

```python
from __future__ import annotations

import os
from dataclasses import dataclass

from typing import Dict, List, Optional, Sequence, Tuple

import torch

from . import binding as B
from .packing import PackedBeats, PackedLlama, PackedQFormer, PackedWhisper

BF16, F32, I32 = torch.bfloat16, torch.float32, torch.int32


class Workspace:

    GRAPH_VISIBLE = ("dc_", "gen_", "kv_")

    def __init__(self, device):
        self.device = torch.device(device)
        self._bufs: Dict[tuple, list] = {}
        self.generation = 0

    def get(self, name: str, shape: Sequence[int], dtype, zero: bool = False) -> torch.Tensor:
# ... 65 lines not shown
        w, c = self.w, self.w.cfg
        n, d, T = xt.shape[0], c.d_model, c.n_ctx
        M = n * T
        x2 = ws.get("wh_x2", (n, 3002, d), BF16, zero=True)
        h = ws.get("wh_h", (M, d), F32)
        xn = ws.get("wh_xn", (M, d), BF16)
        qkv = ws.get("wh_qkv", (M, 3 * d), BF16)
        att = ws.get("wh_att", (M, d), BF16)
        ff = ws.get("wh_ff", (M, c.ffn), BF16)
        out = ws.get("wh_out", (M, d), F32)
        cu = ws.get("wh_cu", (n + 1,), I32)
        cu.copy_(torch.arange(0, M + 1, T, dtype=I32), non_blocking=True)
        B.gemm(xt, w.conv1_w, x2[:, 1:], bias=w.conv1_b, gelu=True, M=3000, K=384, lda=128, batch=n,
               stride_a=3002 * 128, stride_c=3002 * d)
        B.gemm(x2, w.conv2_w, h, bias=w.conv2_b, gelu=True, residual=w.pos, M=T, K=3 * d, lda=2 * d, batch=n,
               stride_a=3002 * d, stride_c=T * d, stride_r=0)
        D = d // c.n_heads
        for L in w.layers:
            B.layernorm(h, L.ln1_g, L.ln1_b, xn, 1e-5)
            B.gemm(xn, L.wqkv, qkv, bias=L.bqkv)
            B.attn_fwd(qkv[:, :d], qkv[:, d:2 * d], qkv[:, 2 * d:], att, cu, T, c.n_heads, D, D ** -0.5, kv_lens=kv_lens)
            B.gemm(att, L.wo, h, bias=L.bo, residual=h)
            B.layernorm(h, L.ln2_g, L.ln2_b, xn, 1e-5)
            B.gemm(xn, L.w1, ff, bias=L.b1, gelu=True)
            B.gemm(ff, L.w2, h, bias=L.b2, residual=h)
        if not final_ln:
            return h
        B.layernorm(h, w.lnf_g, w.lnf_b, out, 1e-5)
        return out


class QwenAudioTowerHIP:

    def __init__(self, enc: WhisperEncoderHIP, proj_w: torch.Tensor, proj_b: torch.Tensor, llm_hidden: int):
        self.enc, self.proj_w, self.proj_b, self.llm_hidden = enc, proj_w, proj_b, llm_hidden

    @staticmethod
    def output_lengths(mel_len: int):
        feat = (mel_len - 1) // 2 + 1
        return feat, (feat - 2) // 2 + 1

    def forward(self, ws: Workspace, xt: torch.Tensor, mel_lens: List[int]) -> Tuple[torch.Tensor, List[int]]:
        w, c = self.enc.w, self.enc.w.cfg
        n, d, T = xt.shape[0], c.d_model, c.n_ctx
        lens = [self.output_lengths(int(m)) for m in mel_lens]
        kv = _i32([max(1, f) for f, _ in lens], xt.device)
        h = self.enc.forward(ws, xt, kv_lens=kv, final_ln=False)
        P = n * (T // 2)
        pooled = ws.get("qa_pool", (P, d), F32)
        even, odd = h.view(P, 2 * d)[:, :d], h.view(P, 2 * d)[:, d:]
        B.axpby_cast(odd, pooled, alpha=0.5)
        B.axpby_cast(even, pooled, alpha=0.5, add=pooled)
        pb = ws.get("qa_pool_bf", (P, d), BF16)
        B.layernorm(pooled, w.lnf_g, w.lnf_b, pb, 1e-5)
        out = ws.get("qa_out", (P, self.llm_hidden), F32)
        B.gemm(pb, self.proj_w, out, bias=self.proj_b)
        return out, [o for _, o in lens]


class BeatsHIP:
    def __init__(self, w: PackedBeats, device):
        from .audio_tables import kaldi_mel_banks
        self.w = w
        self.banks = torch.from_numpy(kaldi_mel_banks()).to(device)

    @staticmethod
    def frames(n_samples: int) -> int:
        return 0 if n_samples < 400 else 1 + (n_samples - 400) // 160

    @classmethod
    def tokens(cls, n_samples: int) -> int:
        return (cls.frames(n_samples) // 16) * 8

    def forward(self, ws: Workspace, wav: torch.Tensor, padded_lens: List[int], valid_lens: List[int]):
        w, c = self.w, self.w.cfg
        dev = wav.device
        n, d = wav.shape[0], c.d_model
        nf = [self.frames(L) for L in padded_lens]
        T = [(f // 16) * 8 for f in nf]
        assert min(T) > 0, "audio shorter than one BEATs patch (16 frames)"
        assert max(T) <= w.rel_span or w.rel_span > c.max_distance, "audio longer than the packed relative-position span"
        cu_h = [0]
        for t in T:
            cu_h.append(cu_h[-1] + t)
        M = cu_h[-1]
        valid_T = []
        for a in range(n):
            vf = self._valid_units(valid_lens[a], padded_lens[a], nf[a])
            valid_T.append(max(1, self._valid_units(vf, nf[a], T[a])))
        max_frames = max(nf)
        fb = ws.get("be_fbank", (n, max_frames, 128), F32)
        B.fbank_kaldi(wav, _i32(padded_lens, dev), self.banks, max_frames, c.fbank_mean, c.fbank_std, fb)
        cu = _i32(cu_h, dev)
        valid = _i32(valid_T, dev)
        patches = ws.get("be_patches", (M, 256), BF16)
        B.beats_patchify(fb, cu, M, patches)
        e = ws.get("be_e", (M, c.embed), F32)
        eb = ws.get("be_eb", (M, c.embed), BF16)
        B.gemm(patches, w.patch_w, e)
        B.layernorm(e, w.ln0_g, w.ln0_b, eb, 1e-5)
        x = ws.get("be_x", (M, d), F32)
        B.gemm(eb, w.proj_w, x, bias=w.proj_b)
        G, cpg = c.conv_groups, d // c.conv_groups
        xg = ws.get("be_xg", ((M + 128 * n) * d,), BF16)
        B.beats_posconv_pack(x, cu, valid, n, M, G, xg)
        y = ws.get("be_y", (M, d), F32)
        uniform = all(t == T[0] for t in T)
        for g in range(G):
            wg, bg = w.posconv_w[g], w.posconv_b[g * cpg:(g + 1) * cpg]
            if uniform:
                a_view = xg[g * (T[0] + 128) * cpg:]
                B.gemm(a_view, wg, y[:, g * cpg:], bias=bg, gelu=True, residual=x[:, g * cpg:], M=T[0], K=128 * cpg,
                       lda=cpg, batch=n, stride_a=(T[0] + 128) * d, stride_c=T[0] * d, stride_r=T[0] * d)
            else:
                for a in range(n):
                    base = (cu_h[a] + 128 * a) * d + g * (T[a] + 128) * cpg
                    B.gemm(xg[base:], wg, y[cu_h[a]:cu_h[a + 1], g * cpg:], bias=bg, gelu=True,
                           residual=x[cu_h[a]:cu_h[a + 1], g * cpg:], M=T[a], K=128 * cpg, lda=cpg)
        xb = ws.get("be_xb", (M, d), BF16)
        B.layernorm(y, w.enc_ln_g, w.enc_ln_b, x, 1e-5, out2=xb)
        qkv = ws.get("be_qkv", (M, 3 * d), BF16)
        att = ws.get("be_att", (M, d), BF16)
        o = ws.get("be_o", (M, d), F32)
        ff = ws.get("be_ff", (M, c.ffn), BF16)
        gate = ws.get("be_gate", (M, c.n_heads), F32)
        alpha = c.deep_norm_alpha
        for L in w.layers:
            B.gemm(xb, L.wqkv, qkv, bias=L.bqkv)
            B.beats_gate(qkv, L.extra["grep_w"], L.extra["grep_b"], L.extra["grep_a"], gate, c.n_heads)
            B.attn_fwd(qkv[:, :d], qkv[:, d:2 * d], qkv[:, 2 * d:], att, cu, max(T), c.n_heads, 64, 0.125,
                       kv_lens=valid, rel_bias=w.rel_table, rel_gate=gate, rel_span=w.rel_span)
            B.gemm(att, L.wo, o, bias=L.bo)
            B.layernorm(o, L.ln1_g, L.ln1_b, x, 1e-5, res=x, alpha=alpha, out2=xb)
            B.gemm(xb, L.w1, ff, bias=L.b1, gelu=True)
            B.gemm(ff, L.w2, o, bias=L.b2)
            B.layernorm(o, L.ln2_g, L.ln2_b, x, 1e-5, res=x, alpha=alpha, out2=xb)
        return x, cu_h, T

    @staticmethod
    def _valid_units(valid_in: int, total_in: int, n_units: int) -> int:
        if n_units == 0:
            return 0
        per = total_in // n_units
        if per == 0:
            return n_units
        return min(n_units, -(-valid_in // per)) if valid_in > 0 else 0


class SpeechQFormerHIP:
    def __init__(self, w: PackedQFormer, whisper_d: int, beats_d: int, llm_hidden: int):
        self.w, self.whisper_d, self.beats_d, self.llm_hidden = w, whisper_d, beats_d, llm_hidden
        c = w.cfg
        self.win = round(1500 * c.second_per_window / 30.0)
        self.stride = round(1500 * c.second_stride / 30.0)
        assert self.win == self.stride, "HIP path implements non-overlapping windows (kernel == stride, SURVEY.md A8)"

    def n_windows(self, T: int = 1500) -> int:
        return (T - self.win) // self.stride + 1

    def forward(self, ws: Workspace, speech: torch.Tensor, n: int, audio: Optional[torch.Tensor] = None,
                audio_cu: Optional[List[int]] = None) -> torch.Tensor:
        T0 = 1500
        frames = [T0] * n if audio is None else [max(T0, audio_cu[a + 1] - audio_cu[a]) for a in range(n)]
        self.last_windows = [self.n_windows(f) for f in frames]
        if all(f == T0 for f in frames):
            return self._run(ws, speech, n, audio, audio_cu, T0)
        Wmax = max(self.last_windows)
        full = ws.get("qf_out_ragged", (n, Wmax, self.llm_hidden), F32)
        full.zero_()
        a0 = 0
        while a0 < n:
            a1 = a0 + 1
            while a1 < n and frames[a1] == frames[a0]:
                a1 += 1
            cu = [x - audio_cu[a0] for x in audio_cu[a0:a1 + 1]]
            out = self._run(ws, speech[a0 * T0:a1 * T0], a1 - a0, audio[audio_cu[a0]:audio_cu[a1]], cu, frames[a0])
            nw = self.n_windows(frames[a0])
            full[a0:a1, :nw].copy_(out.view(a1 - a0, nw, self.llm_hidden))
            a0 = a1
        return full.view(n * Wmax, self.llm_hidden)

    def _run(self, ws: Workspace, speech: torch.Tensor, n: int, audio: Optional[torch.Tensor], audio_cu: Optional[List[int]],
             T: int) -> torch.Tensor:
        w, c = self.w, self.w.cfg
        dw, db, hq = self.whisper_d, self.beats_d, c.hidden
        C = dw + (db if audio is not None else 0)
        assert C == c.enc_width, f"Q-Former encoder width {c.enc_width} != {C}"
        cat = ws.get("qf_cat", (n * T, C), BF16)
        if T == 1500:
            B.layernorm(speech, w.ln_speech_g, w.ln_speech_b, cat, 1e-5, N=dw)
        else:
            cat.zero_()
            for a in range(n):
                B.layernorm(speech[a * 1500:(a + 1) * 1500], w.ln_speech_g, w.ln_speech_b, cat[a * T:a * T + 1500], 1e-5, N=dw)
        if audio is not None:
            if T == 1500:
                cat[:, dw:].zero_()
            for a in range(n):
                ta = audio_cu[a + 1] - audio_cu[a]
                assert ta <= T
                B.layernorm(audio[audio_cu[a]:audio_cu[a] + ta], w.ln_audio_g, w.ln_audio_b,
                            cat[a * T:a * T + ta, dw:], 1e-5, N=db)
        nw = self.n_windows(T)
        W = n * nw
        h = ws.get("qf_h", (W, hq), F32)
        hb = ws.get("qf_hb", (W, hq), BF16)
        t32 = ws.get("qf_t32", (W, hq), F32)
        tb = ws.get("qf_tb", (W, hq), BF16)
        q = ws.get("qf_q", (W, hq), BF16)
        kv = ws.get("qf_kv", (n * T, 2 * hq), BF16)
        ff = ws.get("qf_ff", (W, c.ffn), BF16)
        q0 = ws.get("qf_q0", (1, hq), F32)
        B.layernorm(w.query, w.emb_ln_g, w.emb_ln_b, q0, c.ln_eps)
        B.axpby_cast(q0.expand(W, hq), h)
        B.axpby_cast(q0.expand(W, hq), hb)
        for L in w.layers:
            B.gemm(hb, L.sa_wv, tb, bias=L.sa_bv)
            B.gemm(tb, L.sa_wo, t32, bias=L.sa_bo, residual=h)
            B.layernorm(t32, L.sa_ln_g, L.sa_ln_b, h, c.ln_eps, out2=hb)
            B.gemm(hb, L.ca_wq, q, bias=L.ca_bq)
            B.gemm(cat, L.ca_wkv, kv, bias=L.ca_bkv)
            B.qformer_window_xattn(q, kv, hq, tb, n, nw, self.win, T, c.n_heads, 0.125)
            B.gemm(tb, L.ca_wo, t32, bias=L.ca_bo, residual=h)
            B.layernorm(t32, L.ca_ln_g, L.ca_ln_b, h, c.ln_eps, out2=hb)
            B.gemm(hb, L.w1, ff, bias=L.b1, gelu=True)
            B.gemm(ff, L.w2, t32, bias=L.b2, residual=h)
            B.layernorm(t32, L.ff_ln_g, L.ff_ln_b, h, c.ln_eps, out2=hb)
        out = ws.get("qf_out", (W, self.llm_hidden), F32)
        B.gemm(hb, w.proj_w, out, bias=w.proj_b)
        return out


DECODE_SITES = ("qkv", "o", "gu", "down")


@dataclass(frozen=True)
class GemmLaunch:
    tile: object
    split_k: int
    weight: str
    N: int
    K: int
    fused_norm: bool = False


@dataclass(frozen=True)
class DecodePlan:
    Bn: int
    sites: Dict[str, GemmLaunch]
    workspace: int


def lm_head_tile(R: int) -> int:
    return 4 if R <= 8 else 0


def t256_split(N: int, K: int, n_cu: int) -> int:
    tiles = (N + 255) // 256
    split = min(K // 512, int(0.8 * n_cu) // tiles)
    return split if split >= 2 and tiles * split >= 0.45 * n_cu else 0


def decode_plan(Bn: int, cfg, k_aug: int, n_cu: int, weight_dtype: str = "bf16", decode_packed: bool = True,
                decode_t256: Sequence[str] = DECODE_SITES, fuse_norms: bool = True) -> DecodePlan:
    hd, I = cfg.hidden, cfg.ffn
    shapes = dict(qkv=(3 * hd, k_aug), o=(hd, hd), gu=(2 * I, hd), down=(hd, I))

    def sk(N, K):
        tiles = ((N + 63) // 64) * ((Bn + 63) // 64)
        s = max(1, min(K // 512, (2 * n_cu + tiles - 1) // tiles))
        return min(s, 16)

    def sk5(N, K):
        return max(1, min(n_cu // ((N + 127) // 128), K // 512))
    plan = {}
    for name, (N, K) in shapes.items():
        if Bn <= 8 and weight_dtype == "fp8":
            tile, split, weight = "fp8w", 1, "fp8"
        elif Bn <= 256 and decode_packed:
            if Bn <= 8:
                tile, split, weight = 6, 1, "packed"
            else:
                tile, split, weight = 5, sk5(N, K), "packed"
                s256 = t256_split(N, K, n_cu) if Bn > 128 and name in decode_t256 else 0
                if s256:
                    tile, split, weight = 3, s256, "row"
        elif Bn <= 8:
            tile, split, weight = 4, 1, "row"
        else:
            tile, split, weight = 2, sk(N, K), "row"
        plan[name] = GemmLaunch(tile, split, weight, N, K, fused_norm=fuse_norms and name in ("o", "down"))
    plan["lm_head"] = GemmLaunch(lm_head_tile(Bn), 1, "row", cfg.vocab, hd)
    nsplit = max(p.split_k for p in plan.values())
    return DecodePlan(Bn, plan, nsplit * Bn * max(3 * hd, 2 * I) if nsplit > 1 else 0)


class LlamaHIP:
    decode_packed_weights = True
    fuse_decode_norms = True
    fuse_decode_rope = os.environ.get("ICL_FUSE_DECODE_ROPE", "1") != "0"

    decode_t256 = tuple(x for x in os.environ.get("ICL_DECODE_T256", "qkv,o,gu,down").split(",") if x)

    def _t256_split(self, N: int, K: int) -> int:
        return t256_split(N, K, self.n_cu)

    def decode_plan(self, Bn: int) -> DecodePlan:
        return decode_plan(Bn, self.w.cfg, self.w.k_aug, self.n_cu, self.weight_dtype, self.decode_packed_weights,
                           self.decode_t256, self.fuse_decode_norms)

    def __init__(self, w: PackedLlama, device, decode_packed: Optional[bool] = None, pack_now: bool = True,
                 weight_dtype: str = "bf16"):
        if weight_dtype not in ("bf16", "fp8"):
            raise ValueError(f"weight_dtype must be 'bf16' or 'fp8', not {weight_dtype!r}")
        self.w = w
        self.device = torch.device(device)
        self.n_cu = max(B.device_cu_count(), 1)
        self.weight_dtype = weight_dtype
        if decode_packed is not None:
            self.decode_packed_weights = bool(decode_packed)
        if weight_dtype == "fp8":
            self._quantize_fp8()
        elif self.decode_packed_weights and pack_now:
            self.ensure_decode_packed()

    def _quantize_fp8(self):
        c = self.w.cfg
        for L in self.w.layers:
            packs = []
            for name, K in (("wqkv", self.w.k_aug), ("wo", c.hidden), ("wgu", c.hidden), ("wdown", c.ffn)):
                q, s, wd = B.pack_fp8_weights(getattr(L, name), K=K)
                setattr(L, name, wd)
                packs.append((q, s))
            L.fp8 = tuple(packs)
            L.decode_packed = None

    def ensure_decode_packed(self):
        c = self.w.cfg
        for L in self.w.layers:
            if getattr(L, "decode_packed", None) is None:
                L.decode_packed = (B.pack_decode_weights(L.wqkv, K=self.w.k_aug), B.pack_decode_weights(L.wo, K=c.hidden),
                                   B.pack_decode_weights(L.wgu, K=c.hidden), B.pack_decode_weights(L.wdown, K=c.ffn))

    def embed(self, ws: Workspace, src_idx: torch.Tensor, speech: Optional[torch.Tensor], name: str = "ll_h") -> torch.Tensor:
        h = ws.get(name, (src_idx.numel(), self.w.cfg.hidden), F32)
        B.embed_gather_interleave(src_idx, self.w.embed, speech, h)
        return h

    def _layer(self, ws: Workspace, L, h, M: int, tag: str, attn_fn, pos, seq_ids, kc, vc, max_len: int,
               split: Optional[DecodePlan] = None, kv_rows_to_c: bool = True, xn_ready: bool = False, next_norm=None,
               attn_does_rope: bool = False, rope_fn=None):
        c, w = self.w.cfg, self.w
        hd, I, D, H = c.hidden, c.ffn, c.head_dim, c.n_heads
        xn = ws.get(tag + "xn", (M, w.k_aug), BF16, zero=True)
        qkv = ws.get(tag + "qkv", (M, 3 * hd), BF16)
        att = ws.get(tag + "att", (M, hd), BF16)
        act = ws.get(tag + "act", (M, I), BF16)
        site = split.sites if split is not None else {}
        ps = {k: site[k] if k in site else GemmLaunch(0, 1, "row", 0, 0) for k in DECODE_SITES}

        def tile_of(name):
            return ps[name].tile

        def weight_of(name, idx, row_major):
            if ps[name].weight == "fp8":
                return L.fp8[idx][0]
            return L.decode_packed[idx] if ps[name].weight == "packed" else row_major

        def scale_of(name, idx):
            return L.fp8[idx][1] if ps[name].weight == "fp8" else None
        sk = {k: p.split_k for k, p in ps.items()}
        wsk = ws.get(tag + "splitk", (split.workspace,), F32) if split is not None and split.workspace else None
        if not xn_ready:
            B.rmsnorm(h, L.rms1, xn, c.rms_eps, N=hd)
        if L.lora_a is not None:
            r2 = L.lora_a.shape[0]
            if split is not None and M > 64:
                B.lora_down(xn, hd, L.lora_a, r2, 1.0, M=M)
            else:
                B.gemm(xn, L.lora_a, xn[:, hd:hd + r2], K=hd, tile=4 if split is not None else 2)
        if split is None and B.rope_fusable(M, H, D, L.wqkv.shape[1]):
            B.gemm(xn, L.wqkv, qkv, bias=L.bqkv, tile=3,
                   rope=(hd, 2 * hd, w.rope_cos, w.rope_sin, pos, seq_ids, kc, vc, H, D, max_len, kv_rows_to_c))
        else:
            B.gemm(xn, weight_of("qkv", 0, L.wqkv), qkv, bias=L.bqkv, split_k=sk.get("qkv", 1),
                   workspace=wsk, tile=tile_of("qkv"), N=3 * hd, K=w.k_aug, w_scale=scale_of("qkv", 0))
            if rope_fn is not None:
                rope_fn(qkv)
            elif not attn_does_rope:
                B.rope_kv(qkv, hd, 2 * hd, w.rope_cos, w.rope_sin, pos, seq_ids, kc, vc, H, D, max_len, M=M)
        attn_fn(qkv, att)
        if ps["o"].fused_norm:
            B.gemm_rmsnorm(att, weight_of("o", 1, L.wo), h, L.rms2, c.rms_eps, xn, residual=h, split_k=sk.get("o", 1),
                           workspace=wsk, tile=tile_of("o"), N=hd, K=hd, w_scale=scale_of("o", 1))
        else:
            B.gemm(att, weight_of("o", 1, L.wo), h, residual=h, split_k=sk.get("o", 1), workspace=wsk, tile=tile_of("o"),
                   N=hd, K=hd, w_scale=scale_of("o", 1))
            B.rmsnorm(h, L.rms2, xn, c.rms_eps, N=hd)
        B.gemm(xn, weight_of("gu", 2, L.wgu), act, swiglu=True, K=hd, split_k=sk.get("gu", 1), workspace=wsk,
               tile=tile_of("gu"), N=2 * I, w_scale=scale_of("gu", 2))
        if ps["down"].fused_norm and next_norm is not None:
            B.gemm_rmsnorm(act, weight_of("down", 3, L.wdown), h, next_norm[0], c.rms_eps, next_norm[1], residual=h,
                           split_k=sk.get("down", 1), workspace=wsk, tile=tile_of("down"), N=hd, K=I, w_scale=scale_of("down", 3))
            return True
        B.gemm(act, weight_of("down", 3, L.wdown), h, residual=h, split_k=sk.get("down", 1), workspace=wsk,
               tile=tile_of("down"), N=hd, K=I, w_scale=scale_of("down", 3))
        return False

    def prefill(self, ws: Workspace, h: torch.Tensor, seq_lens: List[int], cache: Optional["KVCache"] = None) -> torch.Tensor:
        c = self.w.cfg
        dev = h.device
        M = sum(seq_lens)
        cu_h = [0]
        for s in seq_lens:
            cu_h.append(cu_h[-1] + s)
        assert max(seq_lens) <= c.max_pos
        pos = _i32([p for s in seq_lens for p in range(s)], dev)
        sid = _i32([b for b, s in enumerate(seq_lens) for _ in range(s)], dev)
        cu = _i32(cu_h, dev)
        maxS = max(seq_lens)
        H, D, hd = c.n_heads, c.head_dim, c.hidden

        fp8 = cache is not None and cache.dtype == "fp8"
        kv_from_cache = cache is not None and not fp8 and B.rope_fusable(M, H, D, self.w.k_aug)

        def attn(qkv, att):
            B.attn_fwd(qkv[:, :hd], qkv[:, hd:2 * hd], qkv[:, 2 * hd:], att, cu, maxS, H, D, D ** -0.5, causal=True)

        for i, L in enumerate(self.w.layers):
            kc = cache.k[i] if cache is not None else None
            vc = cache.v[i] if cache is not None else None
            fn = attn
            if fp8:
                def fn(qkv, att, i=i):
                    B.kv_append_fp8(qkv, hd, 2 * hd, pos, sid, cache.k[i], cache.v[i], cache.ks[i], cache.vs[i], H, D, cache.max_len,
                                    M=M)
                    attn(qkv, att)
                self._layer(ws, L, h, M, "pf_", fn, pos, sid, None, None, 0)
                continue
            if kv_from_cache:
                def fn(qkv, att, kc=kc, vc=vc):
                    B.attn_fwd(qkv[:, :hd], kc, vc, att, cu, maxS, H, D, D ** -0.5, causal=True, kv_cache_max_len=cache.max_len)
            self._layer(ws, L, h, M, "pf_", fn, pos, sid, kc, vc, cache.max_len if cache is not None else 0,
                        kv_rows_to_c=not kv_from_cache)
        return h

    def logits(self, ws: Workspace, h_rows: torch.Tensor, name: str = "ll_logits", xn_ready: bool = False) -> torch.Tensor:
        c = self.w.cfg
        R = h_rows.shape[0]
        xn = ws.get(name + "_xn", (R, c.hidden), BF16)
        out = ws.get(name, (R, c.vocab), F32)
        if not xn_ready:
            B.rmsnorm(h_rows, self.w.norm, xn, c.rms_eps)
        B.gemm(xn, self.w.lm_head, out, tile=lm_head_tile(R))
        return out

    def decode_step(self, ws: Workspace, cache: "KVCache", next_ids: torch.Tensor, pos: torch.Tensor,
                    lens: torch.Tensor, sid: torch.Tensor) -> torch.Tensor:
        c = self.w.cfg
        Bn = next_ids.numel()
        h = self.embed(ws, next_ids, None, name="dc_h")
        H, D = c.n_heads, c.head_dim
        split = self.decode_plan(Bn)
        if any(p.weight == "packed" for p in split.sites.values()):
            self.ensure_decode_packed()

        layers = self.w.layers
        xn_next = ws.get("dc_xn", (Bn, self.w.k_aug), BF16, zero=True)
        xn_final = ws.get("dc_logits_xn", (Bn, c.hidden), BF16)
        ready = False
        fp8 = cache.dtype == "fp8"
        for i, L in enumerate(layers):
            kc, vc = cache.k[i], cache.v[i]
            ks, vs = (cache.ks[i], cache.vs[i]) if fp8 else (None, None)

            fuse_rope = self.fuse_decode_rope and Bn > 8
            rope_fn = None
            if fp8 and fuse_rope:
                def attn(qkv, att, kc=kc, vc=vc, ks=ks, vs=vs):
                    B.attn_decode_rope_fp8(qkv, c.hidden, 2 * c.hidden, self.w.rope_cos, self.w.rope_sin, pos, sid, kc, vc, ks, vs,
                                           att, lens, H, D, cache.max_len, D ** -0.5)
            elif fp8:
                def rope_fn(qkv, ks=ks, vs=vs, kc=kc, vc=vc):
                    B.rope_kv_fp8(qkv, c.hidden, 2 * c.hidden, self.w.rope_cos, self.w.rope_sin, pos, sid, kc, vc, ks, vs, H, D,
                                  cache.max_len, M=Bn)

                def attn(qkv, att, kc=kc, vc=vc, ks=ks, vs=vs):
                    B.attn_decode_fp8(qkv[:, :c.hidden], kc, vc, ks, vs, att, lens, H, D, cache.max_len, D ** -0.5)
            elif fuse_rope:
                def attn(qkv, att, kc=kc, vc=vc):
                    B.attn_decode_rope(qkv, c.hidden, 2 * c.hidden, self.w.rope_cos, self.w.rope_sin, pos, sid, kc, vc, att, lens,
                                       H, D, cache.max_len, D ** -0.5)
            else:
                def attn(qkv, att, kc=kc, vc=vc):
                    B.attn_decode(qkv[:, :c.hidden], kc, vc, att, lens, H, D, cache.max_len, D ** -0.5)

            nxt = (layers[i + 1].rms1, xn_next) if i + 1 < len(layers) else (self.w.norm, xn_final)
            ready = self._layer(ws, L, h, Bn, "dc_", attn, pos, sid, kc, vc, cache.max_len, split=split, xn_ready=ready,
                                next_norm=nxt, attn_does_rope=fuse_rope, rope_fn=rope_fn)
        return self.logits(ws, h, name="dc_logits", xn_ready=ready)


KV_DTYPES = ("bf16", "fp8")


def check_kv_dtype(value: str) -> str:
    if value not in KV_DTYPES:
        raise ValueError(f"llm_kv_dtype must be one of {KV_DTYPES}, not {value!r}")
    return value


class KVCache:

    def __init__(self, cfg, n_seqs: int, max_len: int, ws: Workspace, dtype: str = "bf16"):
        self.n_seqs, self.max_len, self.dtype = n_seqs, max_len, check_kv_dtype(dtype)
        shape = (cfg.n_layers, n_seqs, cfg.n_heads, max_len, cfg.head_dim)
        if dtype == "fp8":
            self.k = ws.get("kv_k8", shape, torch.uint8)
            self.v = ws.get("kv_v8", shape, torch.uint8)
            self.ks = ws.get("kv_ks", shape[:4], F32)
            self.vs = ws.get("kv_vs", shape[:4], F32)
        else:
            self.k = ws.get("kv_k", shape, BF16)
            self.v = ws.get("kv_v", shape, BF16)
            self.ks = self.vs = None

    def planes(self):
        return ((self.k, self.ks), (self.v, self.vs))

    def rows(self, b0: int, b1: int) -> "KVCache":
        sub = object.__new__(KVCache)
        sub.n_seqs, sub.max_len, sub.dtype = b1 - b0, self.max_len, self.dtype
        sub.k, sub.v = self.k[:, b0:b1], self.v[:, b0:b1]
        sub.ks, sub.vs = (self.ks[:, b0:b1], self.vs[:, b0:b1]) if self.ks is not None else (None, None)
        return sub
```

### icl-speech-text-llm_amd/runtime/salmonn.py

```python
from __future__ import annotations

import os

from dataclasses import dataclass
from typing import Dict, List, Optional, Sequence, Tuple, Union

import torch

from . import binding as B
from .config import SalmonnCfg
from .engines import (BF16, F32, I32, BeatsHIP, KVCache, LlamaHIP, LogMel, SpeechQFormerHIP, WhisperEncoderHIP, Workspace, _i32,
                      check_kv_dtype)
from .packing import normalize_keys, pack_beats, pack_llama, pack_qformer, pack_whisper

Segment = Union[Sequence[int], Tuple[str, int, int]]


def speech_segment(first_row: int, n_rows: int) -> Tuple[str, int, int]:
    return ("speech", first_row, n_rows)


@dataclass
class GenerateResult:
    tokens: torch.Tensor
    first_logits: Optional[torch.Tensor] = None
    step_logits: Optional[torch.Tensor] = None
    dropped: Tuple[int, ...] = ()
    token_logprobs: Optional[torch.Tensor] = None


class CausalLMRuntimeMixin:

    use_graphs = True
    kv_dtype = "bf16"

    def _gather_indices(self, prompts: Sequence[Sequence[Segment]], n_speech_rows: int) -> Tuple[List[int], List[int]]:
        V = self.lm_cfg.vocab
        flat: List[int] = []
        lens: List[int] = []
        for segs in prompts:
            before = len(flat)
            for seg in segs:
                if isinstance(seg, tuple) and len(seg) == 3 and seg[0] == "speech":
                    _, first, cnt = seg
                    if first < 0 or first + cnt > n_speech_rows:
                        raise ValueError(f"speech segment [{first},{first + cnt}) outside {n_speech_rows} speech rows")
                    flat.extend(-(r + 1) for r in range(first, first + cnt))
                else:
                    for t in seg:
                        t = int(t)
                        if not 0 <= t < V:
                            raise ValueError(f"token id {t} outside the vocabulary [0,{V})")
                        flat.append(t)
            if len(flat) == before:
                raise ValueError("empty prompt")
            lens.append(len(flat) - before)
        return flat, lens

    @staticmethod
    def _prompt_lengths(prompts: Sequence[Sequence[Segment]]) -> List[int]:
        return [sum(seg[2] if (isinstance(seg, tuple) and len(seg) == 3 and seg[0] == "speech") else len(seg) for seg in segs)
                for segs in prompts]

    def embed_prompts(self, prompts, speech: Optional[torch.Tensor], name: str = "ll_h"):
        rows = 0 if speech is None else speech.shape[0] * (speech.shape[1] if speech.dim() == 3 else 1)
        sp2 = None if speech is None else speech.reshape(rows, self.lm_cfg.hidden).contiguous()
        flat, lens = self._gather_indices(prompts, rows)
        h = self.llama.embed(self.ws, _i32(flat, self.device), sp2, name=name)
        return h, lens

    def forward_logits(self, prompts, speech: Optional[torch.Tensor]) -> Tuple[torch.Tensor, List[int]]:
        h, lens = self.embed_prompts(prompts, speech, name="fw_h")
        self.llama.prefill(self.ws, h, lens, cache=None)
        return self.llama.logits(self.ws, h, name="fw_logits"), lens

    def cross_entropy(self, logits: torch.Tensor, shifted_labels: torch.Tensor) -> torch.Tensor:
        M = logits.shape[0]
        rows = self.ws.get("ce_rows", (M,), F32)
        mean = self.ws.get("ce_mean", (1,), F32)
        B.cross_entropy(logits, shifted_labels.to(device=self.device, dtype=I32), rows, mean)
        return mean

    MAX_GRAPHS = 16

    def _cache(self, n_seqs: int, max_len: int) -> KVCache:
        return KVCache(self.lm_cfg, n_seqs, max_len, self.ws, dtype=self.kv_dtype)

    prefill_chunk = int(os.environ.get("ICL_PREFILL_CHUNK", "128"))

    def _graph_lookup(self, gkey):
        gen = self.ws.generation
        if self._graph_gen != gen:
            self._graphs.clear()
            self._graph_warm.clear()
            self._graph_gen = gen
        return self._graphs.get(gkey), gkey in self._graph_warm

    def generate(self, prompts, speech: Optional[torch.Tensor], max_new_tokens: int = 10, eos_id: Optional[int] = None,
                 pad_id: Optional[int] = None, suppress_eos: bool = False, want_first_logits: bool = False,
                 cache_len_multiple: int = 64, do_sample: bool = False, temperature: float = 1.0, top_p: float = 1.0,
                 top_k: int = 50, repetition_penalty: float = 1.0, generator: Optional[torch.Generator] = None,
                 sample_debug=None, want_step_logits: bool = False, overlong: str = "raise", num_beams: int = 1,
                 length_penalty: float = 1.0, beam_debug: Optional[dict] = None, constraint=None) -> GenerateResult:
        c, ws, dev = self.lm_cfg, self.ws, self.device
        if overlong not in ("raise", "drop"):
            raise ValueError(f"overlong must be 'raise' or 'drop', not {overlong!r}")
        if constraint is not None:
            constraint = self._check_constraint(constraint, len(prompts), max_new_tokens, eos_id, do_sample, repetition_penalty,
                                                num_beams, suppress_eos)
        limit = c.max_pos // cache_len_multiple * cache_len_multiple
        plens = self._prompt_lengths(prompts)
        bad = [b for b, n in enumerate(plens) if n + max_new_tokens > limit]
        if bad and (overlong == "raise" or len(bad) == len(plens)):
            raise ValueError(f"prompt + new tokens of row(s) {bad} ({[plens[b] + max_new_tokens for b in bad]} positions) "
                             f"exceed max_pos {c.max_pos}")
        if bad:
            keep = [b for b in range(len(plens)) if b not in set(bad)]
            sub = self.generate([prompts[b] for b in keep], speech, max_new_tokens=max_new_tokens, eos_id=eos_id, pad_id=pad_id,
                                suppress_eos=suppress_eos, want_first_logits=want_first_logits,
                                cache_len_multiple=cache_len_multiple, do_sample=do_sample, temperature=temperature, top_p=top_p,
                                top_k=top_k, repetition_penalty=repetition_penalty, generator=generator,
                                sample_debug=sample_debug, want_step_logits=want_step_logits, num_beams=num_beams,
                                length_penalty=length_penalty,
                                constraint=None if constraint is None else (constraint[0], [constraint[1][b] for b in keep]))
            n, kidx = len(plens), torch.tensor(keep)
            toks = torch.full((n, sub.tokens.shape[1]), c.pad_id if pad_id is None else pad_id, dtype=torch.int64)
            toks[kidx] = sub.tokens
            first = steps = None
            if sub.first_logits is not None:
                first = torch.full((n, sub.first_logits.shape[1]), float("nan"), dtype=F32, device=dev)
                first[kidx.to(dev)] = sub.first_logits
            if sub.step_logits is not None:
                steps = torch.full((sub.step_logits.shape[0], n, sub.step_logits.shape[2]), float("nan"), dtype=F32, device=dev)
                steps[:, kidx.to(dev)] = sub.step_logits
            lps = None
            if sub.token_logprobs is not None:
                lps = torch.full((n, sub.token_logprobs.shape[1]), float("nan"), dtype=F32)
                lps[kidx] = sub.token_logprobs
            return GenerateResult(tokens=toks, first_logits=first, step_logits=steps, dropped=tuple(bad), token_logprobs=lps)
        eos = c.eos_id if eos_id is None else eos_id
        eos = tuple(int(e) for e in eos) if isinstance(eos, (tuple, list)) else int(eos)
        pad = c.pad_id if pad_id is None else pad_id
        if suppress_eos:
            eos = -1
        assert max_new_tokens >= 1
        if num_beams != 1:
            if num_beams < 1:
                raise ValueError(f"num_beams must be >= 1, not {num_beams}")
            if do_sample or want_step_logits:
                raise NotImplementedError("beam search runs without sampling (HF's beam-sample mode) and without a per-step logits trace")
            if num_beams > 8 or max_new_tokens > 64:
                raise ValueError(f"beam search supports num_beams <= 8 and max_new_tokens <= 64 (got {num_beams}, {max_new_tokens})")
            return self._generate_beam(prompts, speech, max_new_tokens, eos, pad, num_beams, float(length_penalty),
                                       want_first_logits, cache_len_multiple, debug=beam_debug,
                                       repetition_penalty=float(repetition_penalty))
        h, lens = self.embed_prompts(prompts, speech)
        Bn = len(lens)
        need = max(lens) + max_new_tokens
        max_len = -(-need // cache_len_multiple) * cache_len_multiple
        assert max_len <= c.max_pos, f"prompt + new tokens ({need}) exceeds max_pos {c.max_pos}"
        cache = self._cache(Bn, max_len)
        marks = getattr(self, "phase_marks", None)
        if marks is not None:
            marks["prefill_start"].record()
        if Bn <= self.prefill_chunk:
            self.llama.prefill(ws, h, lens, cache)
        else:
            r0 = 0
            for b0 in range(0, Bn, self.prefill_chunk):
                b1 = min(Bn, b0 + self.prefill_chunk)
                r1 = r0 + sum(lens[b0:b1])
                self.llama.prefill(ws, h[r0:r1], lens[b0:b1], cache.rows(b0, b1))
                r0 = r1
        cu_last = []
        acc = 0
        for s in lens:
            acc += s
            cu_last.append(acc - 1)
        last = ws.get("gen_last", (Bn, c.hidden), F32)
        B.gather_rows(h, _i32(cu_last, dev), last)
        logits = self.llama.logits(ws, last, name="gen_logits")
        first = logits.clone() if want_first_logits else None
        trace = ws.get("gen_logits_trace", (max_new_tokens, Bn, c.vocab), F32) if want_step_logits else None
        if trace is not None:
            trace[0].copy_(logits)
        if marks is not None:
            marks["prefill_end"].record()
        finished = ws.get("gen_finished", (Bn,), I32)
        finished.zero_()
        toks = ws.get("gen_tokens", (Bn, max_new_tokens), I32)
        nxt = ws.get("gen_next", (Bn,), I32)
        sampled = do_sample or repetition_penalty != 1.0
        lps = None
        if constraint is not None:
            tables = constraint[0].upload(dev)
            fsm_state = ws.get("gen_fsm_state", (Bn,), I32)
            fsm_state.copy_(torch.tensor(constraint[1], dtype=I32), non_blocking=True)
            lps = ws.get("gen_token_logprobs", (Bn, max_new_tokens), F32)
            knobs = ("fsm", tables.uid)

            def tail(lg, step):
                B.argmax_fsm(lg, tables, fsm_state, max_new_tokens - step, eos, pad, finished, toks, step, nxt, out_logprob=lps,
                             V=c.vocab)
        elif sampled:
            top_k = c.vocab if not top_k else min(int(top_k), c.vocab)
            if top_k < 1 or B.SAMPLE_TOP_K_MAX < top_k < c.vocab:
                raise ValueError(f"top_k={top_k}: the sampling kernel supports 1..{B.SAMPLE_TOP_K_MAX}, or 0 / None / >= vocabulary "
                                 f"({c.vocab}) for no top-k filter")
            if (do_sample and not (0.0 < float(top_p) <= 1.0 and float(temperature) > 0.0)) or not float(repetition_penalty) > 0.0:
                raise ValueError(f"sampling knobs out of range: temperature={temperature} (> 0), top_p={top_p} (0 < p <= 1), "
                                 f"repetition_penalty={repetition_penalty} (> 0)")
            knobs = ((float(temperature), top_k, float(top_p)) if do_sample else (1.0, 1, 1.0)) + (float(repetition_penalty),)
            uni = ws.get("gen_uniform", (max_new_tokens, Bn), F32)
            if do_sample and generator is not None and generator.device.type != uni.device.type:
                uni.copy_(torch.rand(uni.shape, generator=generator))
            elif do_sample:
                uni.uniform_(0.0, 1.0, generator=generator)
            else:
                uni.zero_()
            work = ws.get("gen_sample_work", (Bn, logits.shape[1]), F32)

            def tail(lg, step):
                B.sample_eos(lg, work, uni[step], eos, pad, finished, toks, step, nxt, temperature=knobs[0], top_k=knobs[1],
                             top_p=knobs[2], repetition_penalty=knobs[3], V=c.vocab,
                             debug=sample_debug if step == 0 else None)
        else:
            knobs = None

            def tail(lg, step):
                B.argmax_eos(lg, eos, pad, finished, toks, step, nxt, V=c.vocab)
        tail(logits, 0)
        if max_new_tokens > 1:
            steps = max_new_tokens - 1
            pos_all = ws.get("gen_pos", (steps, Bn), I32)
            len_all = ws.get("gen_len", (steps, Bn), I32)
            sid = ws.get("gen_sid", (Bn,), I32)
            pos_all.copy_(torch.tensor([[s + t for s in lens] for t in range(steps)], dtype=I32), non_blocking=True)
            len_all.copy_(torch.tensor([[s + t + 1 for s in lens] for t in range(steps)], dtype=I32), non_blocking=True)
            sid.copy_(torch.arange(Bn, dtype=I32), non_blocking=True)

            def decode_loop():
                for t in range(steps):
                    lg = self.llama.decode_step(ws, cache, nxt, pos_all[t], len_all[t], sid)
                    if trace is not None:
                        trace[t + 1].copy_(lg)
                    tail(lg, t + 1)

            gkey = (Bn, max_len, steps, eos, pad, knobs, trace is not None, self.kv_dtype)
            graph, warm = self._graph_lookup(gkey) if self.use_graphs else (None, False)
            if graph is not None:
                graph.replay()
            elif warm:
                g = torch.cuda.CUDAGraph()
                torch.cuda.synchronize()
                prof, B.GEMM_PROFILE = B.GEMM_PROFILE, None
                try:
                    with torch.cuda.graph(g):
                        decode_loop()
                finally:
                    B.GEMM_PROFILE = prof
                while len(self._graphs) >= self.MAX_GRAPHS:
                    self._graphs.pop(next(iter(self._graphs)))
                self._graphs[gkey] = g
                g.replay()
            else:
                decode_loop()
                if self.use_graphs:
                    self._graph_lookup(gkey)
                    self._graph_warm.add(gkey)
        if marks is not None:
            marks["decode_end"].record()
        out = toks.cpu().to(torch.int64)
        width = max_new_tokens
        if B._eos_pair(eos)[0] >= 0:
            is_eos = torch.isin(out, torch.tensor([e for e in B._eos_pair(eos) if e >= 0]))
            first_eos = torch.where(is_eos.any(1), is_eos.float().argmax(1) + 1, torch.full((Bn,), max_new_tokens))
            width = int(first_eos.max())
        return GenerateResult(tokens=out[:, :width].contiguous(), first_logits=first,
                              step_logits=trace.clone() if trace is not None else None,
                              token_logprobs=lps.cpu()[:, :width].contiguous() if lps is not None else None)

    def _check_constraint(self, constraint, n_rows: int, max_new_tokens: int, eos_id, do_sample: bool, repetition_penalty: float,
                          num_beams: int, suppress_eos: bool):
        try:
            automaton, starts = constraint
            starts = [int(x) for x in starts]
        except (TypeError, ValueError):
            raise ValueError("constraint must be (LabelAutomaton, one start state per prompt)") from None
        c = self.lm_cfg
        if do_sample or float(repetition_penalty) != 1.0 or num_beams != 1 or suppress_eos:
            raise ValueError("constrained decoding is greedy: do_sample, repetition_penalty != 1, num_beams > 1 and suppress_eos "
                             "cannot be combined with a constraint")
        if len(starts) != n_rows:
            raise ValueError(f"{len(starts)} start states for {n_rows} prompts")
        if any(not -1 <= x < automaton.n_states for x in starts):
            raise ValueError(f"start state outside [-1,{automaton.n_states})")
        if automaton.vocab > c.vocab:
            raise ValueError(f"automaton built for a vocabulary of {automaton.vocab} ids, the model has {c.vocab}")
        eos = c.eos_id if eos_id is None else eos_id
        if automaton.eos_id not in B._eos_pair(tuple(eos) if isinstance(eos, (tuple, list)) else eos):
            raise ValueError(f"automaton built for EOS id {automaton.eos_id}, generate() stops on {eos}")
        short = [b for b, x in enumerate(starts) if automaton.min_tokens(x) > max_new_tokens]
        if short:
            raise ValueError(f"max_new_tokens={max_new_tokens} is below the shortest answer of row(s) {short[:8]} "
                             f"({[automaton.min_tokens(starts[b]) for b in short[:8]]} tokens): no complete label fits")
        return automaton, starts


    beam_rows = 256

    def _generate_beam(self, prompts, speech, max_new_tokens: int, eos: int, pad: int, K: int, length_penalty: float,
                       want_first_logits: bool, cache_len_multiple: int, debug: Optional[dict] = None,
                       repetition_penalty: float = 1.0) -> GenerateResult:
        c, ws, dev = self.lm_cfg, self.ws, self.device
        n_rows = len(prompts)
        per_pass = max(1, self.beam_rows // K)
        if n_rows > per_pass:
            assert debug is None
            parts = [self._generate_beam(prompts[i:i + per_pass], speech, max_new_tokens, eos, pad, K, length_penalty,
                                         want_first_logits, cache_len_multiple, repetition_penalty=repetition_penalty)
                     for i in range(0, n_rows, per_pass)]
            width = max(p.tokens.shape[1] for p in parts)
            toks = torch.full((n_rows, width), pad, dtype=torch.int64)
            r = 0
            for p in parts:
                toks[r:r + p.tokens.shape[0], :p.tokens.shape[1]] = p.tokens
                r += p.tokens.shape[0]
            first = torch.cat([p.first_logits for p in parts]) if want_first_logits else None
            return GenerateResult(tokens=toks, first_logits=first)
        h, lens = self.embed_prompts(prompts, speech)
        Bn, T = len(lens), max_new_tokens
        BK = Bn * K
        need = max(lens) + T
        max_len = -(-need // cache_len_multiple) * cache_len_multiple
        assert max_len <= c.max_pos, f"prompt + new tokens ({need}) exceeds max_pos {c.max_pos}"
        whole = self._cache(BK + Bn, max_len)
        cache, pre = whole.rows(0, BK), whole.rows(BK, BK + Bn)
        r0 = 0
        for b0 in range(0, Bn, self.prefill_chunk):
            b1 = min(Bn, b0 + self.prefill_chunk)
            r1 = r0 + sum(lens[b0:b1])
            self.llama.prefill(ws, h[r0:r1], lens[b0:b1], pre.rows(b0, b1))
            r0 = r1
        cu_last, acc = [], 0
        for s in lens:
            acc += s
            cu_last.append(acc - 1)
        last = ws.get("gen_last", (Bn, c.hidden), F32)
        B.gather_rows(h, _i32(cu_last, dev), last)
        logits = self.llama.logits(ws, last, name="gen_logits")
        first = logits.clone() if want_first_logits else None
        st = B.BeamState(ws.get, Bn, K, T, pad)

        def score(lg, step):
            B.beam_step(lg, st, step, eos, length_penalty, V=c.vocab, repetition_penalty=repetition_penalty)
            if debug is not None:
                for key, val in (("logits", lg), ("run_seq", st.run_seq), ("parent", st.parent), ("next", st.next_ids),
                                 ("fin_seq", st.fin_seq), ("fin_score", st.fin_score), ("fin_len", st.fin_len)):
                    debug.setdefault(key, []).append(val.clone())
        score(logits, 0)
        lens_rep = [s for s in lens for _ in range(K)]
        plen = ws.get("gen_beam_plen", (BK,), I32)
        plen.copy_(torch.tensor(lens_rep, dtype=I32), non_blocking=True)
        if T > 1:
            src = ws.get("gen_beam_src", (BK,), I32)
            src.copy_(torch.tensor([BK + b for b in range(Bn) for _ in range(K)], dtype=I32), non_blocking=True)
            for kv, sc in whole.planes():
                B.kv_copy_spans(kv, kv, BK, src_seq=src, n_t=plen, src_scale=sc, dst_scale=sc)
            steps = T - 1
            pos_all = ws.get("gen_pos", (steps, BK), I32)
            len_all = ws.get("gen_len", (steps, BK), I32)
            sid = ws.get("gen_sid", (BK,), I32)
            pos_all.copy_(torch.tensor([[s + t for s in lens_rep] for t in range(steps)], dtype=I32), non_blocking=True)
            len_all.copy_(torch.tensor([[s + t + 1 for s in lens_rep] for t in range(steps)], dtype=I32), non_blocking=True)
            sid.copy_(torch.arange(BK, dtype=I32), non_blocking=True)
            tmp_k = ws.get("beam_tmp_k", (c.n_layers, BK, c.n_heads, steps, c.head_dim), cache.k.dtype)
            tmp_v = ws.get("beam_tmp_v", tuple(tmp_k.shape), cache.k.dtype)
            tmp_ks = tmp_vs = None
            if cache.dtype == "fp8":
                tmp_ks = ws.get("beam_tmp_ks", tuple(tmp_k.shape[:4]), F32)
                tmp_vs = ws.get("beam_tmp_vs", tuple(tmp_k.shape[:4]), F32)
            for t in range(steps):
                if t:
                    for (kv, sc), tmp, tsc in zip(cache.planes(), (tmp_k, tmp_v), (tmp_ks, tmp_vs)):
                        B.kv_copy_spans(kv, tmp, BK, src_seq=st.parent, src_t0=plen, n_fixed=t, src_scale=sc, dst_scale=tsc)
                        B.kv_copy_spans(tmp, kv, BK, dst_t0=plen, n_fixed=t, src_scale=tsc, dst_scale=sc)
                lg = self.llama.decode_step(ws, cache, st.next_ids, pos_all[t], len_all[t], sid)
                score(lg, t + 1)
        best = st.fin_seq[:, 0].cpu().to(torch.int64)
        blen = st.fin_len[:, 0].cpu()
        ws.release("beam_tmp_k", "beam_tmp_v", "beam_tmp_ks", "beam_tmp_vs")
        width = max(1, int(blen.max()))
        return GenerateResult(tokens=best[:, :width].contiguous(), first_logits=first)


class SalmonnRuntime(CausalLMRuntimeMixin):
    def __init__(self, cfg: SalmonnCfg, state_dict: Dict[str, torch.Tensor], device="cuda", consume: bool = False,
                 parts: Sequence[str] = ("whisper", "beats", "qformer", "llama"), llm_weight_dtype: str = "bf16",
                 llm_kv_dtype: str = "bf16"):
        if not torch.cuda.is_available():
            raise B.IclError("SalmonnRuntime needs a GPU: the HIP path has no CPU fallback")
        B.load_library()
        self.cfg = cfg
        self.lm_cfg = cfg.llama
        self.device = torch.device(device)
        self.kv_dtype = check_kv_dtype(llm_kv_dtype)
        sd = normalize_keys(state_dict) if not consume else state_dict
        self.ws = Workspace(self.device)
        self.whisper = self.beats = self.qformer = self.llama = None
        if "whisper" in parts:
            self.logmel = LogMel(cfg.whisper.n_mels, self.device)
            self.whisper = WhisperEncoderHIP(pack_whisper(sd, cfg.whisper, self.device, consume=consume))
        if "beats" in parts and cfg.beats is not None:
            self.beats = BeatsHIP(pack_beats(sd, cfg.beats, self.device, consume=consume), self.device)
        if "qformer" in parts:
            self.qformer = SpeechQFormerHIP(pack_qformer(sd, cfg.qformer, self.device, consume=consume),
                                            cfg.whisper.d_model, cfg.beats.d_model if self.beats is not None else 0,
                                            cfg.llama.hidden)
        if "llama" in parts:
            self.llama = LlamaHIP(pack_llama(sd, cfg.llama, self.device, consume=consume), self.device,
                                  weight_dtype=llm_weight_dtype)
        self._graphs, self._graph_warm, self._graph_gen = {}, set(), 0

    @property
    def tokens_per_audio(self) -> int:
        return self.qformer.n_windows(1500)

    def encode_speech(self, raw_wav: Optional[torch.Tensor], wav_lens: Optional[Sequence[int]] = None,
                      spectrogram: Optional[torch.Tensor] = None, padded_lens: Optional[Sequence[int]] = None) -> torch.Tensor:
        ws, dev = self.ws, self.device
        if raw_wav is not None:
            raw_wav = raw_wav.to(device=dev, dtype=F32)
            if raw_wav.dim() == 1:
                raw_wav = raw_wav[None]
            raw_wav = raw_wav.contiguous()
            n = raw_wav.shape[0]
            if wav_lens is None:
                wav_lens = [raw_wav.shape[1]] * n
            wav_lens = [int(x) for x in wav_lens]
        else:
            n = spectrogram.shape[0]
        if spectrogram is not None:
            xt = self.logmel.from_spectrogram(ws, spectrogram.to(device=dev, dtype=F32))
        else:
            xt, _ = self.logmel(ws, raw_wav, _i32(wav_lens, dev))
        speech = self.whisper.forward(ws, xt)
        audio = cu = None
        if self.beats is not None and raw_wav is not None:
            padded = [int(x) for x in (padded_lens if padded_lens is not None else wav_lens)]
            audio, cu, _ = self.beats.forward(ws, raw_wav, padded, wav_lens)
        out = self.qformer.forward(ws, speech, n, audio, cu)
        self.last_audio_windows = list(self.qformer.last_windows)
        return out.view(n, max(self.last_audio_windows), self.cfg.llama.hidden)

    def log_mel(self, raw_wav: torch.Tensor, wav_lens: Sequence[int]) -> torch.Tensor:
        raw_wav = raw_wav.to(device=self.device, dtype=F32).contiguous()
        _, spec = self.logmel(self.ws, raw_wav, _i32([int(x) for x in wav_lens], self.device), want_spec=True)
        return spec
```

### include/icl_hip.h

```cpp
#ifndef ICL_HIP_H
#define ICL_HIP_H

#include <stdint.h>

#ifdef __cplusplus
extern "C" {
#endif

#define ICL_ABI_VERSION 6

#define ICL_OK 0
#define ICL_EINVAL (-1)
#define ICL_ELAUNCH (-2)

#define ICL_BF16 0
#define ICL_F32 1

int icl_abi_version(void);
const char* icl_last_error(void);
int icl_device_cu_count(void);

#define ICL_EPI_BIAS 1
#define ICL_EPI_GELU 2
#define ICL_EPI_RESIDUAL 4
#define ICL_EPI_SWIGLU 8

typedef struct icl_gemm_args {
  const void* A;
  const void* W;
  void* C;
  const float* bias;
  const void* R;
  float* workspace;
  int64_t lda, ldw, ldc, ldr;
  int64_t strideA, strideC, strideR;
  int32_t M, N, K;
  int32_t batch;
  int32_t epilogue;
  int32_t out_dtype;
  int32_t res_dtype;
  int32_t split_k;
  int32_t tile;
} icl_gemm_args;

int icl_gemm_bf16(const icl_gemm_args* args, void* stream);
int icl_gemm_rmsnorm_bf16(const icl_gemm_args* args, const float* gamma, float eps, void* xn, int64_t ld_xn, void* stream);
int icl_pack_decode_weights(const void* W, int64_t ldw, int32_t N, int32_t K, void* out, void* stream);
int icl_pack_fp8_weights(const void* W, int64_t ldw, int32_t N, int32_t K, void* q, float* scales, void* w_deq, int64_t ld_deq,
                         void* stream);
int icl_gemm_fp8w(const icl_gemm_args* args, const float* w_scale, void* stream);
int icl_gemm_rmsnorm_fp8w(const icl_gemm_args* args, const float* w_scale, const float* gamma, float eps, void* xn, int64_t ld_xn,
                          void* stream);
int icl_gemm_select_tile(int32_t M, int32_t N, int32_t K, int32_t batch, int32_t split_k);

typedef struct icl_attn_args {
  const void* Q; const void* K; const void* V;
  void* O;
  const int32_t* cu_seqlens;
  const int32_t* kv_lens;
  const float* rel_bias;
  const float* rel_gate;
  int64_t ldq, ldk, ldv, ldo;
  int32_t n_seqs, max_seqlen, n_heads, head_dim;
  int32_t causal, rel_span;
  float scale;
  int32_t reserved;
  int64_t kv_seq_stride, kv_head_stride;
} icl_attn_args;

int icl_attn_fwd_bf16(const icl_attn_args* args, void* stream);

int icl_attn_decode_bf16(const void* Q, int64_t ldq, const void* Kc, const void* Vc, void* O,
                         int64_t ldo, const int32_t* lens, int32_t n_seqs, int32_t n_heads,
                         int32_t head_dim, int32_t max_len, float scale, void* stream);

int icl_attn_decode_rope_bf16(const void* qkv, int64_t ld, int64_t k_off, int64_t v_off, const float* cos, const float* sin,
                              const int32_t* pos, const int32_t* seq_ids, void* kcache, void* vcache, void* O, int64_t ldo,
                              const int32_t* lens, int32_t n_seqs, int32_t n_heads, int32_t head_dim, int32_t max_len,
                              float scale, void* stream);

int icl_layernorm(const void* x, int64_t ldx, const void* res, float alpha, const float* gamma,
                  const float* beta, void* y, int64_t ldy, void* y2, int64_t ldy2, int32_t M,
                  int32_t N, float eps, int32_t in_dtype, int32_t out_dtype, void* stream);
int icl_rmsnorm(const void* x, int64_t ldx, const float* gamma, void* y, int64_t ldy, int32_t M,
                int32_t N, float eps, int32_t in_dtype, int32_t out_dtype, void* stream);

int icl_rope_kv_bf16(void* qkv, int64_t ld, int64_t k_off, int64_t v_off, const float* cos,
                     const float* sin, const int32_t* pos, const int32_t* seq_ids, void* kcache,
                     void* vcache, int32_t M, int32_t n_heads, int32_t head_dim, int32_t max_len,
                     void* stream);

int icl_gemm_rope_kv_bf16(const icl_gemm_args* args, int64_t k_off, int64_t v_off, const float* cos,
                          const float* sin, const int32_t* pos, const int32_t* seq_ids, void* kcache,
                          void* vcache, int32_t n_heads, int32_t head_dim, int32_t max_len, int32_t kv_rows_to_c,
                          void* stream);

int icl_embed_gather_interleave(const int32_t* src_idx, const void* table, const float* speech,
                                float* out, int32_t rows, int32_t H, int32_t vocab,
                                int32_t n_speech_rows, void* stream);

int icl_argmax_eos(const float* logits, int64_t ldl, int32_t B, int32_t V, int32_t eos_id, int32_t eos_id2,
                   int32_t pad_id, int32_t* finished, int32_t* out_tokens, int32_t out_stride,
                   int32_t step, int32_t* next_ids, void* stream);

int icl_argmax_fsm(const float* logits, int64_t ldl, int32_t B, int32_t V, const int32_t* state_off, const int32_t* edge_tok,
                   const int32_t* edge_next, const int32_t* state_dist, int32_t n_states, int32_t n_edges, int32_t* state,
                   int32_t steps_left, int32_t eos_id, int32_t eos_id2, int32_t pad_id, int32_t* finished,
                   int32_t* out_tokens, int32_t out_stride, int32_t step, int32_t* next_ids, float* out_logprob,
                   void* stream);

int icl_sample_eos(const float* logits, int64_t ldl, int32_t B, int32_t V, float* work, int64_t ldw,
                   const int32_t* prev_tokens, int32_t prev_stride, int32_t n_prev, float repetition_penalty,
                   float temperature, int32_t top_k, float top_p, const float* uniforms, int32_t eos_id, int32_t eos_id2,
                   int32_t pad_id, int32_t* finished, int32_t* out_tokens, int32_t out_stride, int32_t step,
                   int32_t* next_ids, int32_t* dbg_ids, float* dbg_probs, int32_t* dbg_count, int32_t dbg_cap,
                   void* stream);

int icl_logmel_whisper(const float* wav, int64_t wav_ld, const int32_t* wav_lens,
                       const double* mel_filters, int32_t n_mel, int32_t n_audio, float* spec,
                       void* xt, int64_t xt_ld, void* workspace, void* stream);
int icl_spec_to_xt(const float* spec, int32_t n_mel, int32_t n_audio, void* xt, int64_t xt_ld,
                   void* stream);

int icl_fbank_kaldi(const float* wav, int64_t wav_ld, const int32_t* wav_lens,
                    const double* mel_banks, int32_t n_audio, int32_t max_frames, float mean,
                    float std, float* fbank, void* stream);

int icl_qformer_window_xattn(const void* q, int64_t ldq, const void* kv, int64_t ldkv,
                             int64_t v_off, void* out, int64_t ldo, int32_t n_audio,
                             int32_t win_per_audio, int32_t win, int32_t rows_per_audio,
                             int32_t n_heads, float scale, void* stream);

int icl_beats_gate(const void* qkv, int64_t ld, const float* grep_w, const float* grep_b,
                   const float* grep_a, float* gate, int32_t M, int32_t n_heads, void* stream);
int icl_axpby_cast(const void* in, int64_t ldi, int32_t in_dtype, const void* add, int64_t lda_,
                   int32_t add_dtype, float alpha, void* out, int64_t ldo, int32_t out_dtype,
                   int32_t M, int32_t N, void* stream);
int icl_lora_down_bf16(void* X, int64_t ldx, int32_t K0, const void* A, int64_t lda_,
                       int32_t r_total, float scale, int32_t M, void* stream);

int icl_beats_patchify(const float* fbank, int32_t max_frames, const int32_t* cu_rows, int32_t n_audio,
                       int32_t total_rows, void* out, void* stream);
int icl_beats_posconv_pack(float* x, const int32_t* cu_rows, const int32_t* valid_rows, int32_t n_audio,
                           int32_t total_rows, int32_t channels, int32_t groups, void* xg, void* stream);
int icl_gather_rows_f32(const float* src, int64_t ld_src, const int32_t* idx, float* out, int64_t ld_out,
                        int32_t rows, int32_t N, void* stream);

int icl_beam_step(const float* logits, int64_t ldl, int32_t rows_per_batch, int32_t B, int32_t V, int32_t num_beams,
                  int32_t max_new_tokens, int32_t step, int32_t eos_id, int32_t eos_id2, float length_penalty,
                  float repetition_penalty, float* run_score,
                  int32_t* run_seq, float* fin_score, int32_t* fin_seq, int32_t* fin_len, int32_t* fin_flag,
                  int32_t* unsat, int32_t* next_ids, int32_t* parent, void* stream);
int icl_kv_copy_spans_bf16(const void* src, void* dst, int64_t src_layer_stride, int64_t src_seq_stride,
                           int64_t src_head_stride, int64_t dst_layer_stride, int64_t dst_seq_stride,
                           int64_t dst_head_stride, const int32_t* src_seq, const int32_t* src_t0,
                           const int32_t* dst_seq, const int32_t* dst_t0, const int32_t* n_t, int32_t n_fixed,
                           int32_t n_rows, int32_t n_layers, int32_t n_heads, int32_t head_dim,
                           int32_t src_n_seqs, int32_t dst_n_seqs, int32_t src_len, int32_t dst_len, void* stream);

int icl_kv_append_fp8(const void* qkv, int64_t ld, int64_t k_off, int64_t v_off, const int32_t* pos, const int32_t* seq_ids,
                      void* kq, void* vq, float* kscale, float* vscale, int32_t M, int32_t n_heads, int32_t head_dim,
                      int32_t max_len, void* stream);
int icl_rope_kv_fp8(void* qkv, int64_t ld, int64_t k_off, int64_t v_off, const float* cos, const float* sin,
                    const int32_t* pos, const int32_t* seq_ids, void* kq, void* vq, float* kscale, float* vscale,
                    int32_t M, int32_t n_heads, int32_t head_dim, int32_t max_len, void* stream);
int icl_attn_decode_bf16_epl16(const void* Q, int64_t ldq, const void* Kc, const void* Vc, void* O, int64_t ldo,
                               const int32_t* lens, int32_t n_seqs, int32_t n_heads, int32_t head_dim, int32_t max_len,
                               float scale, void* stream);
int icl_attn_decode_fp8(const void* Q, int64_t ldq, const void* kq, const void* vq, const float* kscale, const float* vscale,
                        void* O, int64_t ldo, const int32_t* lens, int32_t n_seqs, int32_t n_heads, int32_t head_dim,
                        int32_t max_len, float scale, void* stream);
int icl_attn_decode_rope_fp8(const void* qkv, int64_t ld, int64_t k_off, int64_t v_off, const float* cos, const float* sin,
                             const int32_t* pos, const int32_t* seq_ids, void* kq, void* vq, float* kscale, float* vscale,
                             void* O, int64_t ldo, const int32_t* lens, int32_t n_seqs, int32_t n_heads, int32_t head_dim,
                             int32_t max_len, float scale, void* stream);
int icl_kv_copy_spans_fp8(const void* src, const float* src_scale, void* dst, float* dst_scale, int64_t src_layer_stride,
                          int64_t src_seq_stride, int64_t src_head_stride, int64_t dst_layer_stride, int64_t dst_seq_stride,
                          int64_t dst_head_stride, int64_t src_scale_layer_stride, int64_t src_scale_seq_stride,
                          int64_t src_scale_head_stride, int64_t dst_scale_layer_stride, int64_t dst_scale_seq_stride,
                          int64_t dst_scale_head_stride, const int32_t* src_seq, const int32_t* src_t0, const int32_t* dst_seq,
                          const int32_t* dst_t0, const int32_t* n_t, int32_t n_fixed, int32_t n_rows, int32_t n_layers,
                          int32_t n_heads, int32_t head_dim, int32_t src_n_seqs, int32_t dst_n_seqs, int32_t src_len,
                          int32_t dst_len, void* stream);

int icl_cross_entropy(const float* logits, int64_t ldl, const int32_t* labels, int32_t M, int32_t V,
                      float* row_loss, float* mean_loss, void* stream);

#ifdef __cplusplus
}
#endif
#endif
```

Measured before the change: 142.1.

## Compute only last-token rows in the final prefill layer

In the last Llama prefill layer, K/V are still produced for every row to fill the cache, but Q, attention, the output projection and the MLP run only on each sequence's final row. A new suffix-query causal attention variant reads Q and writes O for just those trailing rows, and a bf16 row-gather kernel is added. This removes most of the last layer's Q projection, attention, O-proj and FFN work during prefill, at the cost of extra small GEMMs and kernel launches and a separate code path that must match the full-layer numerics.

```diff
diff --git a/icl-speech-text-llm_amd/csrc/attn.hip b/icl-speech-text-llm_amd/csrc/attn.hip
--- a/icl-speech-text-llm_amd/csrc/attn.hip
+++ b/icl-speech-text-llm_amd/csrc/attn.hip
@@ -42,8 +42,8 @@
   return __builtin_fmaxf(__builtin_bit_cast(float, lo), __builtin_bit_cast(float, hi));
 }
 
-template <int D, bool CAUSAL, bool BIAS>
-__global__ __launch_bounds__(256, (D == 64 && BIAS) ? 3 : 2) void attn_fwd_kernel(AttnParams p) {
+template <int D, bool CAUSAL, bool BIAS, bool SUFFIX = false>
+__global__ __launch_bounds__(256, (D == 64 && BIAS) ? 3 : 2) void attn_fwd_kernel(AttnParams p, const int* cu_q) {
   constexpr int QB = 1;
   constexpr bool P2 = (D == 128);
   constexpr int BQ = 128 * QB;
@@ -70,10 +70,18 @@
   const int len = p.cu[seq + 1] - row0;
   const int qb = qblk * BQ;
   if (qb >= len) return;
+  int qrow0 = row0, qstart = 0;
+  if constexpr (SUFFIX) {
+    qrow0 = cu_q[seq];
+    const int qlen = cu_q[seq + 1] - qrow0;
+    qstart = max(len - qlen, 0);
+    if (qlen <= 0 || qb + BQ <= qstart) return;
+  }
   int kvlen = len;
   if (p.kv_lens) kvlen = min(max(p.kv_lens[seq], 1), len);
   const int kv_end = CAUSAL ? min(kvlen, qb + BQ) : kvlen;
   const int n_tiles = (kv_end + 63) >> 6;
+  const bool wave_has_q = !SUFFIX || qb + wave * (32 * QB) + 32 * QB > qstart;
 
   int qw[QB], qpos[QB];
   bf16x8 qf[QB][KS];
@@ -84,7 +92,7 @@
     qw[qi] = qb + (wave * QB + qi) * 32;
     qpos[qi] = qw[qi] + ql;
     const int qrow = min(qpos[qi], len - 1);
-    const unsigned short* qp = p.Q + (int64_t)(row0 + qrow) * p.ldq + head * D + hh * 8;
+    const unsigned short* qp = p.Q + (int64_t)(SUFFIX ? qrow0 + max(qrow - qstart, 0) : row0 + qrow) * p.ldq + head * D + hh * 8;
 #pragma unroll
     for (int ks = 0; ks < KS; ++ks) qf[qi][ks] = *(const bf16x8*)(qp + ks * 16);
     gate[qi] = 0.f;
@@ -181,6 +189,7 @@
 #pragma unroll
     for (int qi = 0; qi < QB; ++qi) {
       active[qi] = !MAYMASK || !CAUSAL || (k0 <= qw[qi] + 31);
+      if constexpr (SUFFIX) active[qi] = active[qi] && wave_has_q;
       any_active |= active[qi];
     }
     if (any_active) {
@@ -396,14 +405,14 @@
       const int row = it * RPI + lane / LPR, cc = lane % LPR;
       const int q = qw[row >> 5] + (row & 31);
       const u32x4 v = *(const u32x4*)(stg + row * PITCH + cc * 16);
-      if (q < len) *(u32x4*)(p.O + (int64_t)(row0 + q) * p.ldo + head * D + cc * 8) = v;
+      if (q < len && (!SUFFIX || q >= qstart)) *(u32x4*)(p.O + (int64_t)(SUFFIX ? qrow0 + q - qstart : row0 + q) * p.ldo + head * D + cc * 8) = v;
     }
     return;
   }
 #pragma unroll
   for (int qi = 0; qi < QB; ++qi) {
-    if (qpos[qi] < len) {
-      unsigned short* op = p.O + (int64_t)(row0 + qpos[qi]) * p.ldo + head * D;
+    if (qpos[qi] < len && (!SUFFIX || qpos[qi] >= qstart)) {
+      unsigned short* op = p.O + (int64_t)(SUFFIX ? qrow0 + qpos[qi] - qstart : row0 + qpos[qi]) * p.ldo + head * D;
 #pragma unroll
       for (int d = 0; d < DB; ++d) {
 #pragma unroll
@@ -417,7 +426,6 @@
     }
   }
 }
-
 
 constexpr int IL64_NW = 4;
 template <bool CAUSAL, int NW>
@@ -717,7 +725,7 @@
 }
 
 template <int D>
-int launch_attn(const AttnParams& p, const icl_attn_args* a, hipStream_t stream) {
+int launch_attn(const AttnParams& p, const icl_attn_args* a, const int* cu_q, hipStream_t stream) {
   const int bq = (D == 64 && !a->rel_bias) ? IL64_NW * 64 : 128;
   dim3 grid(((a->max_seqlen + bq - 1) / bq) * a->n_heads * a->n_seqs, 1, 1);
   const bool bias = a->rel_bias != nullptr;
@@ -727,16 +735,21 @@
     ICL_CHECK_LAUNCH("icl_attn_fwd_bf16");
     return ICL_OK;
   }
+  if (cu_q) {
+    if constexpr (D == 128) hipLaunchKernelGGL((attn_fwd_kernel<128, true, false, true>), grid, dim3(256), 0, stream, p, cu_q);
+    ICL_CHECK_LAUNCH("icl_attn_fwd_suffix_bf16");
+    return ICL_OK;
+  }
   if (a->causal) {
     if (bias)
-      hipLaunchKernelGGL((attn_fwd_kernel<D, true, true>), grid, dim3(256), 0, stream, p);
+      hipLaunchKernelGGL((attn_fwd_kernel<D, true, true>), grid, dim3(256), 0, stream, p, nullptr);
     else
-      hipLaunchKernelGGL((attn_fwd_kernel<D, true, false>), grid, dim3(256), 0, stream, p);
+      hipLaunchKernelGGL((attn_fwd_kernel<D, true, false>), grid, dim3(256), 0, stream, p, nullptr);
   } else {
     if (bias)
-      hipLaunchKernelGGL((attn_fwd_kernel<D, false, true>), grid, dim3(256), 0, stream, p);
+      hipLaunchKernelGGL((attn_fwd_kernel<D, false, true>), grid, dim3(256), 0, stream, p, nullptr);
     else
-      hipLaunchKernelGGL((attn_fwd_kernel<D, false, false>), grid, dim3(256), 0, stream, p);
+      hipLaunchKernelGGL((attn_fwd_kernel<D, false, false>), grid, dim3(256), 0, stream, p, nullptr);
   }
   ICL_CHECK_LAUNCH("icl_attn_fwd_bf16");
   return ICL_OK;
@@ -744,7 +757,7 @@
 
 }
 
-extern "C" int icl_attn_fwd_bf16(const icl_attn_args* a, void* stream) {
+static int attn_fwd_impl(const icl_attn_args* a, const int32_t* cu_q, void* stream) {
   ICL_CHECK_ARG(a != nullptr, "icl_attn_fwd_bf16: args is NULL");
   ICL_CHECK_ARG(a->Q && a->K && a->V && a->O && a->cu_seqlens, "icl_attn_fwd_bf16: NULL pointer");
   ICL_CHECK_ARG(a->head_dim == 64 || a->head_dim == 128, "icl_attn_fwd_bf16: head_dim=%d (only 64 and 128)", a->head_dim);
@@ -776,5 +789,14 @@
   const int bq = (a->head_dim == 64 && !a->rel_bias) ? IL64_NW * 64 : 128;
   p.n_qblocks = (a->max_seqlen + bq - 1) / bq;
   p.scale_log2e = a->scale * LOG2E;
-  return a->head_dim == 64 ? launch_attn<64>(p, a, (hipStream_t)stream) : launch_attn<128>(p, a, (hipStream_t)stream);
+  return a->head_dim == 64 ? launch_attn<64>(p, a, cu_q, (hipStream_t)stream) : launch_attn<128>(p, a, cu_q, (hipStream_t)stream);
 }
+
+extern "C" int icl_attn_fwd_bf16(const icl_attn_args* a, void* stream) { return attn_fwd_impl(a, nullptr, stream); }
+
+extern "C" int icl_attn_fwd_suffix_bf16(const icl_attn_args* a, const int32_t* cu_q, void* stream) {
+  ICL_CHECK_ARG(a != nullptr && cu_q != nullptr, "icl_attn_fwd_suffix_bf16: NULL pointer");
+  ICL_CHECK_ARG(a->head_dim == 128 && a->causal && !a->rel_bias && !a->rel_gate && !a->kv_lens,
+                "icl_attn_fwd_suffix_bf16: the suffix-query form is built for head_dim 128, causal, without bias or kv_lens");
+  return attn_fwd_impl(a, cu_q, stream);
+}
diff --git a/icl-speech-text-llm_amd/csrc/beats.hip b/icl-speech-text-llm_amd/csrc/beats.hip
--- a/icl-speech-text-llm_amd/csrc/beats.hip
+++ b/icl-speech-text-llm_amd/csrc/beats.hip
@@ -62,12 +62,12 @@
       u32x4{pack_bf16x2(v0[0], v0[1]), pack_bf16x2(v0[2], v0[3]), pack_bf16x2(v1[0], v1[1]), pack_bf16x2(v1[2], v1[3])};
 }
 
-__global__ __launch_bounds__(256) void gather_rows_kernel(const float* src, int64_t lds_, const int* idx, float* out,
+__global__ __launch_bounds__(256) void gather_rows_kernel(const u32x4* src, int64_t lds_, const int* idx, u32x4* out,
                                                            int64_t ldo, int N) {
   const int64_t r = blockIdx.x;
-  const float* s = src + (int64_t)idx[r] * lds_;
-  float* d = out + r * ldo;
-  for (int c = threadIdx.x * 4; c < N; c += blockDim.x * 4) *(f32x4*)(d + c) = *(const f32x4*)(s + c);
+  const u32x4* s = src + (int64_t)idx[r] * lds_;
+  u32x4* d = out + r * ldo;
+  for (int c = threadIdx.x; c < N; c += blockDim.x) d[c] = s[c];
 }
 
 }
@@ -101,7 +101,19 @@
   ICL_CHECK_ARG(src && idx && out && rows > 0 && N > 0 && N % 4 == 0 && ld_src % 4 == 0 && ld_out % 4 == 0,
                 "icl_gather_rows_f32: bad arguments");
   ICL_CHECK_ARG(((uintptr_t)src & 15) == 0 && ((uintptr_t)out & 15) == 0, "icl_gather_rows_f32: misaligned");
-  hipLaunchKernelGGL(gather_rows_kernel, dim3(rows), dim3(256), 0, (hipStream_t)stream, src, ld_src, idx, out, ld_out, N);
+  hipLaunchKernelGGL(gather_rows_kernel, dim3(rows), dim3(256), 0, (hipStream_t)stream, (const u32x4*)src, ld_src / 4, idx,
+                     (u32x4*)out, ld_out / 4, N / 4);
   ICL_CHECK_LAUNCH("icl_gather_rows_f32");
   return ICL_OK;
 }
+
+extern "C" int icl_gather_rows_bf16(const void* src, int64_t ld_src, const int32_t* idx, void* out, int64_t ld_out,
+                                    int32_t rows, int32_t N, void* stream) {
+  ICL_CHECK_ARG(src && idx && out && rows > 0 && N > 0 && N % 8 == 0 && ld_src % 8 == 0 && ld_out % 8 == 0,
+                "icl_gather_rows_bf16: bad arguments (N and the leading dimensions must be multiples of 8)");
+  ICL_CHECK_ARG(((uintptr_t)src & 15) == 0 && ((uintptr_t)out & 15) == 0, "icl_gather_rows_bf16: misaligned");
+  hipLaunchKernelGGL(gather_rows_kernel, dim3(rows), dim3(256), 0, (hipStream_t)stream, (const u32x4*)src, ld_src / 8, idx,
+                     (u32x4*)out, ld_out / 8, N / 8);
+  ICL_CHECK_LAUNCH("icl_gather_rows_bf16");
+  return ICL_OK;
+}
diff --git a/icl-speech-text-llm_amd/csrc/gemm.hip b/icl-speech-text-llm_amd/csrc/gemm.hip
--- a/icl-speech-text-llm_amd/csrc/gemm.hip
+++ b/icl-speech-text-llm_amd/csrc/gemm.hip
@@ -990,8 +990,10 @@
                                      void* stream) {
   ICL_CHECK_ARG(a != nullptr && cosT && sinT && pos, "icl_gemm_rope_kv_bf16: NULL pointer");
   ICL_CHECK_ARG(head_dim == 128, "icl_gemm_rope_kv_bf16: head_dim=%d (the fused epilogue is built for 128)", head_dim);
-  ICL_CHECK_ARG(n_heads > 0 && k_off == (int64_t)n_heads * 128 && v_off == 2 * k_off && a->N == 3 * k_off && k_off % 256 == 0,
-                "icl_gemm_rope_kv_bf16: need q|k|v blocks of n_heads*128 columns each, a multiple of 256 (N=%d k_off=%lld v_off=%lld)",
+  const int64_t hd = (int64_t)n_heads * 128;
+  ICL_CHECK_ARG(n_heads > 0 && hd % 256 == 0 && (k_off == 0 || k_off == hd) && (v_off == k_off || v_off == k_off + hd) &&
+                    (a->N == v_off || a->N == v_off + hd) && a->N > 0,
+                "icl_gemm_rope_kv_bf16: need q|k|v blocks of n_heads*128 columns each (or empty), a multiple of 256 (N=%d k_off=%lld v_off=%lld)",
                 a->N, (long long)k_off, (long long)v_off);
   ICL_CHECK_ARG(a->batch == 1 && a->out_dtype == ICL_BF16 && (a->epilogue & ~ICL_EPI_BIAS) == 0,
                 "icl_gemm_rope_kv_bf16: batch 1, bf16 output, bias-only epilogue");
diff --git a/icl-speech-text-llm_amd/runtime/binding.py b/icl-speech-text-llm_amd/runtime/binding.py
--- a/icl-speech-text-llm_amd/runtime/binding.py
+++ b/icl-speech-text-llm_amd/runtime/binding.py
@@ -52,6 +52,7 @@
     "icl_gemm_rmsnorm_bf16": (c_int, [POINTER(GemmArgs), c_void_p, c_float, c_void_p, c_int64, c_void_p]),
     "icl_gemm_select_tile": (c_int, [c_int32, c_int32, c_int32, c_int32, c_int32]),
     "icl_attn_fwd_bf16": (c_int, [POINTER(AttnArgs), c_void_p]),
+    "icl_attn_fwd_suffix_bf16": (c_int, [POINTER(AttnArgs), c_void_p, c_void_p]),
     "icl_attn_decode_bf16": (c_int, [c_void_p, c_int64, c_void_p, c_void_p, c_void_p, c_int64, c_void_p,
                                      c_int32, c_int32, c_int32, c_int32, c_float, c_void_p]),
     "icl_attn_decode_rope_bf16": (c_int, [c_void_p, c_int64, c_int64, c_int64, c_void_p, c_void_p, c_void_p, c_void_p, c_void_p,
@@ -114,6 +115,7 @@
     "icl_beats_posconv_pack": (c_int, [c_void_p, c_void_p, c_void_p, c_int32, c_int32, c_int32, c_int32, c_void_p,
                                        c_void_p]),
     "icl_gather_rows_f32": (c_int, [c_void_p, c_int64, c_void_p, c_void_p, c_int64, c_int32, c_int32, c_void_p]),
+    "icl_gather_rows_bf16": (c_int, [c_void_p, c_int64, c_void_p, c_void_p, c_int64, c_int32, c_int32, c_void_p]),
     "icl_cross_entropy": (c_int, [c_void_p, c_int64, c_void_p, c_int32, c_int32, c_void_p, c_void_p, c_void_p]),
 }
 
@@ -300,15 +302,19 @@
     return q, scales, out
 
 
+def rope_epilogue_ok(n_heads: int, head_dim: int, K: int) -> bool:
+    return head_dim == 128 and (n_heads * head_dim) % 256 == 0 and K >= 128
+
+
 def rope_fusable(M: int, n_heads: int, head_dim: int, K: int) -> bool:
     hd = n_heads * head_dim
-    return (head_dim == 128 and hd % 256 == 0 and K >= 128 and
+    return (rope_epilogue_ok(n_heads, head_dim, K) and
             load_library().icl_gemm_select_tile(M, 3 * hd, K, 1, 1) == 3)
 
 
 def attn_fwd(q, k, v, out, cu_seqlens, max_seqlen: int, n_heads: int, head_dim: int, scale: float, *,
-             causal=False, kv_lens=None, rel_bias=None, rel_gate=None, rel_span: int = 0, kv_cache_max_len: int = 0):
-    _require_gpu(q, k, v, out, cu_seqlens, kv_lens, rel_bias, rel_gate)
+             causal=False, kv_lens=None, rel_bias=None, rel_gate=None, rel_span: int = 0, kv_cache_max_len: int = 0, cu_q=None):
+    _require_gpu(q, k, v, out, cu_seqlens, kv_lens, rel_bias, rel_gate, cu_q)
     lib = load_library()
     a = AttnArgs()
     a.Q, a.K, a.V, a.O = q.data_ptr(), k.data_ptr(), v.data_ptr(), out.data_ptr()
@@ -325,6 +331,10 @@
     a.max_seqlen, a.n_heads, a.head_dim = max_seqlen, n_heads, head_dim
     a.causal, a.rel_span, a.scale = int(causal), rel_span, scale
     assert cu_seqlens.dtype == torch.int32
+    if cu_q is not None:
+        assert cu_q.dtype == torch.int32 and cu_q.numel() == cu_seqlens.numel()
+        _check(lib.icl_attn_fwd_suffix_bf16(ctypes.byref(a), cu_q.data_ptr(), _stream()), "icl_attn_fwd_suffix_bf16")
+        return out
     _check(lib.icl_attn_fwd_bf16(ctypes.byref(a), _stream()), "icl_attn_fwd_bf16")
     return out
 
@@ -628,10 +638,12 @@
 
 def gather_rows(src, idx, out, N=None):
     _require_gpu(src, idx, out)
-    assert src.dtype == torch.float32 and out.dtype == torch.float32 and idx.dtype == torch.int32
-    _check(load_library().icl_gather_rows_f32(src.data_ptr(), src.stride(0), idx.data_ptr(), out.data_ptr(),
-                                              out.stride(0), idx.numel(), src.shape[1] if N is None else N,
-                                              _stream()), "icl_gather_rows_f32")
+    assert src.dtype == out.dtype and src.dtype in (torch.float32, torch.bfloat16) and idx.dtype == torch.int32
+    lib = load_library()
+    fn, what = ((lib.icl_gather_rows_f32, "icl_gather_rows_f32") if src.dtype == torch.float32 else
+                (lib.icl_gather_rows_bf16, "icl_gather_rows_bf16"))
+    _check(fn(src.data_ptr(), src.stride(0), idx.data_ptr(), out.data_ptr(), out.stride(0), idx.numel(),
+              src.shape[1] if N is None else N, _stream()), what)
     return out
 
 
diff --git a/icl-speech-text-llm_amd/runtime/engines.py b/icl-speech-text-llm_amd/runtime/engines.py
--- a/icl-speech-text-llm_amd/runtime/engines.py
+++ b/icl-speech-text-llm_amd/runtime/engines.py
@@ -391,6 +391,12 @@
 
     decode_t256 = tuple(x for x in os.environ.get("ICL_DECODE_T256", "qkv,o,gu,down").split(",") if x)
 
+    prefill_last_rows = os.environ.get("ICL_PREFILL_LAST_ROWS", "1") != "0"
+    _last_rows_out: Optional[torch.Tensor] = None
+
+    def want_last_rows(self, out: torch.Tensor) -> None:
+        self._last_rows_out = out
+
     def _t256_split(self, N: int, K: int) -> int:
         return t256_split(N, K, self.n_cu)
 
@@ -496,7 +502,10 @@
                tile=tile_of("down"), N=hd, K=I, w_scale=scale_of("down", 3))
         return False
 
-    def prefill(self, ws: Workspace, h: torch.Tensor, seq_lens: List[int], cache: Optional["KVCache"] = None) -> torch.Tensor:
+    def prefill(self, ws: Workspace, h: torch.Tensor, seq_lens: List[int], cache: Optional["KVCache"] = None,
+                last_rows_only: bool = False, last_out: Optional[torch.Tensor] = None) -> torch.Tensor:
+        if self._last_rows_out is not None:
+            last_rows_only, last_out, self._last_rows_out = True, self._last_rows_out, None
         c = self.w.cfg
         dev = h.device
         M = sum(seq_lens)
@@ -504,6 +513,7 @@
         for s in seq_lens:
             cu_h.append(cu_h[-1] + s)
         assert max(seq_lens) <= c.max_pos
+        assert cache is not None or not last_rows_only, "prefill(last_rows_only=True) needs a KV cache"
         pos = _i32([p for s in seq_lens for p in range(s)], dev)
         sid = _i32([b for b, s in enumerate(seq_lens) for _ in range(s)], dev)
         cu = _i32(cu_h, dev)
@@ -512,13 +522,23 @@
 
         fp8 = cache is not None and cache.dtype == "fp8"
         kv_from_cache = cache is not None and not fp8 and B.rope_fusable(M, H, D, self.w.k_aug)
+        trim = last_rows_only and self.prefill_last_rows and not fp8 and B.rope_epilogue_ok(H, D, self.w.k_aug)
 
         def attn(qkv, att):
             B.attn_fwd(qkv[:, :hd], qkv[:, hd:2 * hd], qkv[:, 2 * hd:], att, cu, maxS, H, D, D ** -0.5, causal=True)
 
+        last_idx = _i32([e - 1 for e in cu_h[1:]], dev) if last_rows_only else None
+
+        def last_rows(src):
+            out = last_out if last_out is not None else ws.get("pfl_h", (len(seq_lens), hd), F32)
+            return B.gather_rows(src, last_idx, out)
+
+        n_layers = len(self.w.layers)
         for i, L in enumerate(self.w.layers):
             kc = cache.k[i] if cache is not None else None
             vc = cache.v[i] if cache is not None else None
+            if trim and i == n_layers - 1:
+                return self._last_layer_rows(ws, L, h, M, seq_lens, pos, sid, cu, kc, vc, cache.max_len, last_idx, last_rows)
             fn = attn
             if fp8:
                 def fn(qkv, att, i=i):
@@ -532,7 +552,37 @@
                     B.attn_fwd(qkv[:, :hd], kc, vc, att, cu, maxS, H, D, D ** -0.5, causal=True, kv_cache_max_len=cache.max_len)
             self._layer(ws, L, h, M, "pf_", fn, pos, sid, kc, vc, cache.max_len if cache is not None else 0,
                         kv_rows_to_c=not kv_from_cache)
-        return h
+        return last_rows(h) if last_rows_only else h
+
+    def _last_layer_rows(self, ws: Workspace, L, h, M: int, seq_lens: List[int], pos, sid, cu, kc, vc, max_len: int,
+                         last_idx, last_rows) -> torch.Tensor:
+        c, w = self.w.cfg, self.w
+        hd, I, D, H = c.hidden, c.ffn, c.head_dim, c.n_heads
+        Bn, dev = len(seq_lens), h.device
+        xn = ws.get("pf_xn", (M, w.k_aug), BF16, zero=True)
+        B.rmsnorm(h, L.rms1, xn, c.rms_eps, N=hd)
+        if L.lora_a is not None:
+            r2 = L.lora_a.shape[0]
+            B.gemm(xn, L.lora_a, xn[:, hd:hd + r2], K=hd, tile=2)
+        rope = (w.rope_cos, w.rope_sin)
+        qkv = ws.get("pf_qkv", (M, 3 * hd), BF16)
+        B.gemm(xn, L.wqkv[hd:], qkv, bias=L.bqkv[hd:] if L.bqkv is not None else None, tile=3,
+               rope=(0, hd, *rope, pos, sid, kc, vc, H, D, max_len, False))
+        hg = last_rows(h)
+        xg = ws.get("pfl_xn", (Bn, w.k_aug), BF16)
+        B.gather_rows(xn, last_idx, xg)
+        q = ws.get("pfl_q", (Bn, hd), BF16)
+        B.gemm(xg, L.wqkv[:hd], q, bias=L.bqkv[:hd] if L.bqkv is not None else None, tile=3,
+               rope=(hd, hd, *rope, _i32([s - 1 for s in seq_lens], dev), None, None, None, H, D, max_len))
+        att = ws.get("pfl_att", (Bn, hd), BF16)
+        B.attn_fwd(q, kc, vc, att, cu, max(seq_lens), H, D, D ** -0.5, causal=True, kv_cache_max_len=max_len,
+                   cu_q=_i32(list(range(Bn + 1)), dev))
+        B.gemm(att, L.wo, hg, residual=hg, tile=3, N=hd, K=hd)
+        B.rmsnorm(hg, L.rms2, xg, c.rms_eps, N=hd)
+        act = ws.get("pfl_act", (Bn, I), BF16)
+        B.gemm(xg, L.wgu, act, swiglu=True, tile=3, N=2 * I, K=hd)
+        B.gemm(act, L.wdown, hg, residual=hg, tile=3, N=hd, K=I)
+        return hg
 
     def logits(self, ws: Workspace, h_rows: torch.Tensor, name: str = "ll_logits", xn_ready: bool = False) -> torch.Tensor:
         c = self.w.cfg
diff --git a/icl-speech-text-llm_amd/runtime/salmonn.py b/icl-speech-text-llm_amd/runtime/salmonn.py
--- a/icl-speech-text-llm_amd/runtime/salmonn.py
+++ b/icl-speech-text-llm_amd/runtime/salmonn.py
@@ -163,22 +163,18 @@
         marks = getattr(self, "phase_marks", None)
         if marks is not None:
             marks["prefill_start"].record()
+        last = ws.get("gen_last", (Bn, c.hidden), F32)
         if Bn <= self.prefill_chunk:
+            self.llama.want_last_rows(last)
             self.llama.prefill(ws, h, lens, cache)
         else:
             r0 = 0
             for b0 in range(0, Bn, self.prefill_chunk):
                 b1 = min(Bn, b0 + self.prefill_chunk)
                 r1 = r0 + sum(lens[b0:b1])
+                self.llama.want_last_rows(last[b0:b1])
                 self.llama.prefill(ws, h[r0:r1], lens[b0:b1], cache.rows(b0, b1))
                 r0 = r1
-        cu_last = []
-        acc = 0
-        for s in lens:
-            acc += s
-            cu_last.append(acc - 1)
-        last = ws.get("gen_last", (Bn, c.hidden), F32)
-        B.gather_rows(h, _i32(cu_last, dev), last)
         logits = self.llama.logits(ws, last, name="gen_logits")
         first = logits.clone() if want_first_logits else None
         trace = ws.get("gen_logits_trace", (max_new_tokens, Bn, c.vocab), F32) if want_step_logits else None
@@ -336,18 +332,14 @@
         assert max_len <= c.max_pos, f"prompt + new tokens ({need}) exceeds max_pos {c.max_pos}"
         whole = self._cache(BK + Bn, max_len)
         cache, pre = whole.rows(0, BK), whole.rows(BK, BK + Bn)
+        last = ws.get("gen_last", (Bn, c.hidden), F32)
         r0 = 0
         for b0 in range(0, Bn, self.prefill_chunk):
             b1 = min(Bn, b0 + self.prefill_chunk)
             r1 = r0 + sum(lens[b0:b1])
+            self.llama.want_last_rows(last[b0:b1])
             self.llama.prefill(ws, h[r0:r1], lens[b0:b1], pre.rows(b0, b1))
             r0 = r1
-        cu_last, acc = [], 0
-        for s in lens:
-            acc += s
-            cu_last.append(acc - 1)
-        last = ws.get("gen_last", (Bn, c.hidden), F32)
-        B.gather_rows(h, _i32(cu_last, dev), last)
         logits = self.llama.logits(ws, last, name="gen_logits")
         first = logits.clone() if want_first_logits else None
         st = B.BeamState(ws.get, Bn, K, T, pad)
diff --git a/include/icl_hip.h b/include/icl_hip.h
--- a/include/icl_hip.h
+++ b/include/icl_hip.h
@@ -69,6 +69,8 @@
 } icl_attn_args;
 
 int icl_attn_fwd_bf16(const icl_attn_args* args, void* stream);
+
+int icl_attn_fwd_suffix_bf16(const icl_attn_args* args, const int32_t* cu_q, void* stream);
 
 int icl_attn_decode_bf16(const void* Q, int64_t ldq, const void* Kc, const void* Vc, void* O,
                          int64_t ldo, const int32_t* lens, int32_t n_seqs, int32_t n_heads,
@@ -145,6 +147,8 @@
                            int32_t total_rows, int32_t channels, int32_t groups, void* xg, void* stream);
 int icl_gather_rows_f32(const float* src, int64_t ld_src, const int32_t* idx, float* out, int64_t ld_out,
                         int32_t rows, int32_t N, void* stream);
+int icl_gather_rows_bf16(const void* src, int64_t ld_src, const int32_t* idx, void* out, int64_t ld_out,
+                         int32_t rows, int32_t N, void* stream);
 
 int icl_beam_step(const float* logits, int64_t ldl, int32_t rows_per_batch, int32_t B, int32_t V, int32_t num_beams,
                   int32_t max_new_tokens, int32_t step, int32_t eos_id, int32_t eos_id2, float length_penalty,
```

New measurement: 143.9, median of 6. 1.01x the previous value.
